# GaryGky/IDEAL-NeRF

Measured on AMD Instinct MI355X. Metric: ray-samples/sec (64+128 pts, 512x512), whole job, higher is better.
Workload: dtype f32

## Files before the change

ideal-nerf_amd/_lib.py:

```python
import ctypes as C
import os

HERE = os.path.dirname(os.path.abspath(__file__))
LIB_PATH = os.environ.get("IDN_LIB") or os.path.join(HERE, "libidealnerf.so")

IDN_PREC_F32, IDN_PREC_BF16X3, IDN_PREC_BF16, IDN_PREC_FP16X3, IDN_PREC_BF16X6 = 0, 1, 2, 3, 4
RAY_FLOATS = 11
MAX_MULTIRES, MAX_MULTIRES_VIEWS = 10, 4
SAMPLE_MAX_REGION = 4096
SCORE_TILE = 32
PROF_KINDS = ("mlp_fwd", "mlp_fwd_save", "delta_chain", "dw_gemm", "dw_gemm_x6", "mlp_fwd_save_x6", "delta_chain_x6")

fp = C.c_void_p


class FaceNerfParams(C.Structure):
    _fields_ = [("pts_w", fp * 8), ("pts_b", fp * 8), ("views_w", fp * 3), ("views_b", fp * 3),
                ("alpha_w", fp), ("alpha_b", fp), ("rgb_w", fp), ("rgb_b", fp),
                ("dim_aud", C.c_int), ("dim_expr", C.c_int), ("dim_latent", C.c_int),
                ("multires_plus1", C.c_int), ("multires_views_plus1", C.c_int)]


class FaceNerfGrads(C.Structure):
    _fields_ = [("pts_w", fp * 8), ("pts_b", fp * 8), ("views_w", fp * 3), ("views_b", fp * 3),
                ("alpha_w", fp), ("alpha_b", fp), ("rgb_w", fp), ("rgb_b", fp)]


class PassBwdExtra(C.Structure):
    _fields_ = [("d_expr", fp), ("d_rays", fp), ("d_views0_bias", fp)]


class CompositeOut(C.Structure):
    _fields_ = [(n, fp) for n in ("rgb_map", "disp_map", "acc_map", "depth_map", "weights", "rgb_fg", "last_weight")]


class RenderArgs(C.Structure):
    _fields_ = [("rays", fp), ("bc_rgb", fp), ("n_rays", C.c_int64), ("n_samples", C.c_int),
                ("n_importance", C.c_int), ("precision", C.c_int),
                ("packed_coarse", fp), ("folded_coarse", fp), ("packed_fine", fp), ("folded_fine", fp),
                ("t_vals", fp), ("t_rand", fp), ("u", fp), ("u_per_ray", C.c_int)] + \
               [(n, fp) for n in ("rgb_map", "disp_map", "acc_map", "depth_map", "last_weight", "rgb_fg",
                                  "rgb0", "disp0", "acc0", "z_std", "last_weight0", "rgb_fg0",
                                  "tap_z_coarse", "tap_raw_coarse", "tap_weights_coarse", "tap_cdf", "tap_inds",
                                  "tap_z_samples", "tap_z_fine", "tap_raw_fine", "tap_weights_fine")] + \
               [("workspace", fp), ("workspace_bytes", C.c_size_t), ("precision_fine_plus1", C.c_int),
                ("lindisp", C.c_int), ("white_bkgd", C.c_int), ("noise_coarse", fp), ("noise_fine", fp), ("fused_march", C.c_int),
                ("rng_mode", C.c_int), ("rng_seed", C.c_uint64), ("rng_ray0", C.c_int64)]


class AudioNetParams(C.Structure):
    _fields_ = [("conv_w", fp * 4), ("conv_b", fp * 4), ("fc_w", fp * 2), ("fc_b", fp * 2), ("dim_aud", C.c_int)]


class AudioNetGrads(C.Structure):
    _fields_ = [("conv_w", fp * 4), ("conv_b", fp * 4), ("fc_w", fp * 2), ("fc_b", fp * 2)]


class Frame(C.Structure):
    _fields_ = [("c2w", C.c_float * 12), ("H", C.c_int), ("W", C.c_int), ("focal", C.c_float), ("cx", C.c_float), ("cy", C.c_float),
                ("near_", C.c_float), ("far_", C.c_float), ("row0", C.c_int), ("nrows", C.c_int), ("rays_out", fp)]


class RenderOpts(C.Structure):
    _fields_ = [("colour_gate", C.c_int), ("gate_counters", fp)]


class CullGridStruct(C.Structure):
    _fields_ = [("bits", fp), ("G", C.c_int), ("lo", C.c_float * 3), ("cell", C.c_float)]


CULL_MAX_OUTPUTS = 12


class CullOutput(C.Structure):
    _fields_ = [("dense", fp), ("live", fp), ("channels", C.c_int), ("fill_background", C.c_int), ("value", C.c_float)]


DW_MAX_PRODUCTS, DW_MAX_TAKES, DW_MAX_COLSUM_TAKES = 16, 4, 2


class DwTake(C.Structure):
    _fields_ = [("row0", C.c_int), ("col0", C.c_int), ("rows", C.c_int), ("cols", C.c_int), ("out", fp), ("ldo", C.c_int)]
# ... 17 lines not shown
    "idealnerf_last_error": (C.c_char_p, []),
    "idealnerf_packed_weight_floats": (C.c_size_t, [C.c_int]),
    "idealnerf_folded_bias_floats": (C.c_size_t, []),
    "idealnerf_pack_weights": (C.c_int, [C.POINTER(FaceNerfParams), C.c_int, fp, fp]),
    "idealnerf_fold_conditioning": (C.c_int, [C.POINTER(FaceNerfParams), fp, fp, fp, fp, fp]),
    "idealnerf_facenerf_fwd": (C.c_int, [fp, fp, C.c_int, fp, C.c_int64, fp, fp]),
    "idealnerf_facenerf_fwd_ch": (C.c_int, [fp, fp, C.c_int, fp, C.c_int, C.c_int, C.c_int64, fp, fp]),
    "idealnerf_params_pts_ch": (C.c_int, [C.POINTER(FaceNerfParams)]),
    "idealnerf_params_views_ch": (C.c_int, [C.POINTER(FaceNerfParams)]),
    "idealnerf_query_rays_fwd": (C.c_int, [fp, fp, C.c_int, fp, fp, C.c_int64, C.c_int, fp, fp]),
    "idealnerf_query_points_fwd": (C.c_int, [fp, fp, C.c_int, fp, fp, C.c_int64, C.c_int, fp, fp]),
    "idealnerf_frame_rays": (C.c_int, [C.POINTER(C.c_float), C.c_int, C.c_int, C.c_float, C.c_float, C.c_float,
                                       C.c_float, C.c_float, C.c_int, C.c_int, fp, fp]),
    "idealnerf_to8b": (C.c_int, [fp, C.c_int64, C.c_int, fp, fp, fp]),
    "idealnerf_compose_to8b": (C.c_int, [fp, fp, fp, C.c_int64, C.c_int, fp, fp, fp, fp]),
    "idealnerf_philox_uniform": (C.c_int, [C.c_uint64, C.c_int, C.c_int64, C.c_int64, C.c_int, fp, fp]),
    "idealnerf_sample_pixels_workspace_bytes": (C.c_size_t, []),
    "idealnerf_sample_pixels": (C.c_int, [fp, C.c_int, C.c_int, C.c_int, C.c_int, C.c_int, C.c_int, C.c_uint64, C.c_uint64,
                                          fp, C.c_size_t, fp, fp]),
    "idealnerf_gather_rays": (C.c_int, [fp, C.c_int64, C.POINTER(C.c_float), C.c_int, C.c_int, C.c_float, C.c_float, C.c_float,
                                        fp, fp, fp, fp, fp, fp, fp, fp]),
    "idealnerf_gather_ray_pairs": (C.c_int, [fp, C.c_int64, C.POINTER(C.c_float), C.POINTER(C.c_float), C.c_int, C.c_int, C.c_float,
                                             C.c_float, C.c_float, fp, fp, fp, fp, fp, fp, fp, fp, fp]),
    "idealnerf_frame_scores_workspace_bytes": (C.c_size_t, [C.c_int, C.c_int]),
    "idealnerf_frame_scores": (C.c_int, [fp, fp, fp, C.c_int, C.c_int, fp, fp, C.c_size_t, fp]),
    "idealnerf_coarse_depths": (C.c_int, [fp, fp, fp, C.c_int, C.c_int64, C.c_int, fp, fp]),
    "idealnerf_composite_fwd": (C.c_int, [fp, fp, fp, fp, fp, C.c_int, C.c_int64, C.c_int, C.POINTER(CompositeOut), fp]),
    "idealnerf_sample_pdf_fwd": (C.c_int, [fp, fp, fp, C.c_int, C.c_int64, C.c_int, C.c_int, fp, fp, fp, fp, fp, fp]),
    "idealnerf_march_fwd": (C.c_int, [fp, fp, fp, fp, fp, C.c_int, fp, C.c_int, C.c_int64, C.c_int, C.c_int,
                                      C.POINTER(CompositeOut), fp, fp, fp, fp, fp, fp]),
    "idealnerf_sample_pdf_bins_fwd": (C.c_int, [fp, fp, fp, C.c_int, C.c_int64, C.c_int, C.c_int, fp, fp, fp, fp]),
    "idealnerf_invert_cdf": (C.c_int, [fp, fp, fp, C.c_int, C.c_int64, C.c_int, C.c_int, fp, fp, fp]),
    "idealnerf_render_workspace_bytes": (C.c_size_t, [C.c_int64, C.c_int, C.c_int]),
    "idealnerf_render_rays_fwd": (C.c_int, [C.POINTER(RenderArgs), fp]),
    "idealnerf_render_frame_workspace_bytes": (C.c_size_t, [C.c_int64, C.c_int, C.c_int]),
    "idealnerf_render_frame_fwd": (C.c_int, [C.POINTER(RenderArgs), C.POINTER(Frame), fp]),
    "idealnerf_render_rays_fwd_opts": (C.c_int, [C.POINTER(RenderArgs), C.POINTER(RenderOpts), fp]),
    "idealnerf_render_frame_fwd_opts": (C.c_int, [C.POINTER(RenderArgs), C.POINTER(Frame), C.POINTER(RenderOpts), fp]),
    "idealnerf_colour_gate_max_dist": (C.c_float, []),
    "idealnerf_audio_net_saved_floats": (C.c_size_t, [C.c_int]),
    "idealnerf_audio_net_fwd": (C.c_int, [C.POINTER(AudioNetParams), fp, C.c_int, fp, fp, fp]),
    "idealnerf_audio_net_bwd": (C.c_int, [C.POINTER(AudioNetParams), C.POINTER(AudioNetGrads), fp, fp, fp, C.c_int, fp]),
    "idealnerf_train_acts_floats": (C.c_size_t, [C.c_int64]),
    "idealnerf_query_rays_train_fwd": (C.c_int, [fp, fp, C.c_int, fp, fp, C.c_int64, C.c_int, fp, fp, fp]),
    "idealnerf_pass_bwd_workspace_bytes": (C.c_size_t, [C.c_int64, C.c_int]),
    "idealnerf_pass_bwd": (C.c_int, [C.POINTER(FaceNerfParams), C.POINTER(FaceNerfGrads), fp, fp, fp, fp, fp, fp, fp,
                                     fp, C.c_int64, C.c_int, fp, fp, fp, fp, fp, fp, fp, C.c_size_t, fp]),
    "idealnerf_pass_bwd_rays": (C.c_int, [C.POINTER(FaceNerfParams), C.POINTER(FaceNerfGrads), fp, fp, fp, fp, fp, fp, fp,
                                          fp, C.c_int64, C.c_int, fp, fp, fp, fp, fp, fp, fp, fp, C.c_size_t, fp]),
    "idealnerf_pass_bwd_cond": (C.c_int, [C.POINTER(FaceNerfParams), fp, fp, fp, fp, fp, fp, fp, fp, C.c_int64, C.c_int, fp, fp, fp,
                                          fp, fp, fp, fp, C.c_size_t, fp]),
    "idealnerf_pass_bwd_ex": (C.c_int, [C.POINTER(FaceNerfParams), C.POINTER(FaceNerfGrads), fp, fp, fp, fp, fp, fp, fp,
                                        fp, C.c_int64, C.c_int, fp, fp, fp, fp, fp, fp, C.POINTER(PassBwdExtra), fp, C.c_size_t, fp]),
    "idealnerf_facenerf_train_fwd": (C.c_int, [fp, fp, C.c_int, fp, C.c_int64, fp, fp, fp]),
    "idealnerf_facenerf_train_fwd_ch": (C.c_int, [fp, fp, C.c_int, fp, C.c_int, C.c_int, C.c_int64, fp, fp, fp]),
    "idealnerf_facenerf_bwd_workspace_bytes": (C.c_size_t, [C.c_int64]),
    "idealnerf_facenerf_bwd": (C.c_int, [C.POINTER(FaceNerfParams), C.POINTER(FaceNerfGrads), fp, fp, fp, fp, C.c_int64, fp,
                                         fp, fp, fp, fp, fp, C.c_size_t, fp]),
    "idealnerf_dw_gemm_workspace_bytes": (C.c_size_t, []),
    "idealnerf_dw_gemm": (C.c_int, [fp, C.c_int, fp, C.c_int, C.c_int64, fp, fp, C.c_int, fp, C.c_size_t, fp]),
    "idealnerf_dw_products_workspace_bytes": (C.c_size_t, []),
    "idealnerf_dw_products": (C.c_int, [C.c_int64, C.c_int, C.c_int, C.POINTER(DwProduct), C.c_int, fp, C.c_size_t, fp]),
    "idealnerf_delta_chain_workspace_bytes": (C.c_size_t, []),
    "idealnerf_delta_chain": (C.c_int, [C.POINTER(FaceNerfParams), C.c_int, fp, C.c_int64, fp, fp, fp, fp, C.c_int,
                                        C.POINTER(C.c_int), fp, C.c_size_t, fp]),
    "idealnerf_composite_bwd": (C.c_int, [fp, fp, fp, fp, C.c_int64, C.c_int, fp, fp, fp, fp, fp, C.c_int, fp, C.c_int, fp, C.c_int, fp]),
    "idealnerf_cull_mark": (C.c_int, [fp, C.c_int64, C.c_float, fp, fp]),
    "idealnerf_cull_cells": (C.c_int, [fp, C.c_int, C.c_int, fp, fp]),
    "idealnerf_cull_classify_workspace_bytes": (C.c_size_t, [C.c_int64]),
    "idealnerf_cull_classify": (C.c_int, [C.POINTER(CullGridStruct), C.POINTER(Frame), C.c_float, C.c_int, fp, fp, fp, C.c_size_t, fp]),
    "idealnerf_cull_gather": (C.c_int, [fp, C.c_int64, C.POINTER(Frame), fp, fp, fp, fp]),
    "idealnerf_cull_scatter": (C.c_int, [fp, C.c_int64, C.c_int64, fp, C.POINTER(CullOutput), C.c_int, fp]),
    "idealnerf_profile_begin": (None, []),
    "idealnerf_profile_end": (C.c_int, [C.POINTER(C.c_double), C.POINTER(C.c_int64), C.POINTER(C.c_int64)]),
    "idealnerf_profile_end_kinds": (C.c_int, [C.POINTER(C.c_double), C.POINTER(C.c_int64), C.POINTER(C.c_int64)]),
}

_lib = None


class IdealNerfError(RuntimeError):
    pass


def load():
    global _lib
    if _lib is not None:
        return _lib
    if not os.path.exists(LIB_PATH):
        raise IdealNerfError(
            f"{LIB_PATH} is missing: build the HIP extension first "
            "(python ideal-nerf_amd/build.py, or __graft_entry__.build()). There is no fallback path.")
    lib = C.CDLL(LIB_PATH)
    for name, (res, args) in PROTOTYPES.items():
        fn = getattr(lib, name)
        fn.restype = res
        fn.argtypes = args
    if lib.idealnerf_version() != ABI_VERSION:
        raise IdealNerfError(f"{LIB_PATH} has ABI version {lib.idealnerf_version()}, this package binds version {ABI_VERSION}: rebuild it")
    _lib = lib
    return lib


def check(rc):
    if rc != 0:
        msg = load().idealnerf_last_error()
        raise IdealNerfError(f"libidealnerf error {rc}: {msg.decode() if msg else '?'}")
```

ideal-nerf_amd/csrc/capi.hip:

```cpp
#include "idn_internal.h"
#include <cstdarg>
#include <cstdio>

namespace idn {

static thread_local char g_err[512] = "";

int fail(int code, const char* fmt, ...) {
    va_list ap;
    va_start(ap, fmt);
    vsnprintf(g_err, sizeof(g_err), fmt, ap);
    va_end(ap);
    return code;
}

static int check_precision(int precision) {
    if (precision == IDN_PREC_F32 || precision == IDN_PREC_BF16X3 || precision == IDN_PREC_BF16 || precision == IDN_PREC_FP16X3 ||
        precision == IDN_PREC_BF16X6)
        return IDN_OK;
    return fail(IDN_EUNSUPPORTED, "precision %d is unknown (IDN_PREC_F32, IDN_PREC_BF16X3, IDN_PREC_BF16, IDN_PREC_FP16X3, IDN_PREC_BF16X6)", precision);
}
static int check_precision_train(int precision) {
    if (precision == IDN_PREC_F32 || precision == IDN_PREC_BF16X6) return IDN_OK;
    return fail(IDN_EUNSUPPORTED, "the training path runs fp32-grade arithmetic only: IDN_PREC_F32 or IDN_PREC_BF16X6 (got %d)", precision);
// ... 310 lines not shown
    if (!packed || !folded || !rays || !z || !raw || !acts) return fail(IDN_EINVAL, "NULL pointer");
    const int64_t p_pad = (n_rays * n_samples + 127) / 128 * 128;
    return launch_mlp(precision, mlp_saving(mlp_rays(packed, folded, rays, z, n_rays, n_samples, raw), acts, p_pad), (hipStream_t)stream,
                      MlpGate{});
}

size_t idealnerf_pass_bwd_workspace_bytes(int64_t n_rays, int n_samples) {
    if (n_rays <= 0 || n_samples <= 0) return 0;
    return bwd_workspace_bytes(n_rays * n_samples);
}

static int check_grads(const idn_facenerf_grads* grads) {
    if (!grads) return fail(IDN_EINVAL, "grads is NULL");
    for (int i = 0; i < 8; ++i)
        if (!grads->pts_w[i] || !grads->pts_b[i]) return fail(IDN_EINVAL, "grad pts_linears.%d is NULL", i);
    for (int i = 0; i < 3; ++i)
        if (!grads->views_w[i] || !grads->views_b[i]) return fail(IDN_EINVAL, "grad views_linears.%d is NULL", i);
    if (!grads->alpha_w || !grads->alpha_b || !grads->rgb_w || !grads->rgb_b) return fail(IDN_EINVAL, "grad head is NULL");
    return IDN_OK;
}

static int pass_bwd_any(const PassBwd& b, void* stream) {
    const idn_facenerf_params* p = b.p;
    const BwdCond& c = b.cond;
    const bool frozen = !b.grads;
    if (int e = check_params(p)) return e;
    if (!frozen)
        if (int e = check_grads(b.grads)) return e;
    if ((p->dim_aud > 0) != (c.aud != nullptr) || (p->dim_expr > 0) != (c.expr != nullptr) ||
        (p->dim_latent > 0) != (c.latent != nullptr))
        return fail(IDN_EINVAL, "conditioning pointers do not match the widths");
    if (c.d_expr && (p->dim_expr == 0 || !c.expr)) return fail(IDN_EINVAL, "d_expr for a network without an expression");
    if (frozen && b.d_rays) return fail(IDN_EUNSUPPORTED, "the conditioning-only backward (grads NULL) returns no ray gradient");
    if (!frozen && c.d_vb) return fail(IDN_EINVAL, "d_views0_bias is the frozen plan's: with grads it is grads->views_b[0]");
    const bool want_cond = c.d_aud || c.d_latent || c.d_expr;
    if (frozen && c.d_vb && !want_cond) return fail(IDN_EINVAL, "d_views0_bias needs d_aud, d_latent or d_expr (with none the pass is not run)");
    if (b.n_rays < 0) return fail(IDN_EINVAL, "n_rays < 0");
    if (b.n_rays == 0 || (frozen && !want_cond)) return IDN_OK;
    if (!b.acts || !b.raw || !b.z || !b.rays || !b.bc) return fail(IDN_EINVAL, "NULL pointer");
    return launch_pass_bwd(b, (hipStream_t)stream);
}
static int pass_bwd_trained(const PassBwd& b, void* stream) {
    if (int e = check_params(b.p)) return e;
    if (!b.grads) return check_grads(b.grads);
    return pass_bwd_any(b, stream);
}

int idealnerf_pass_bwd(const idn_facenerf_params* p, const idn_facenerf_grads* grads, const float* aud,
                       const float* expr, const float* latent, const float* acts, const float* raw, const float* z,
                       const float* rays, const float* bc_rgb, int64_t n_rays, int n_samples, const float* g_rgb_map,
                       const float* g_rgb_fg, const float* g_last_weight, const float* g_acc, float* d_aud,
                       float* d_latent, void* workspace, size_t workspace_bytes, void* stream) {
    PassBwd b = {};
    b.p = p; b.grads = grads;
    b.cond.aud = aud; b.cond.expr = expr; b.cond.latent = latent; b.cond.d_aud = d_aud; b.cond.d_latent = d_latent;
    b.acts = acts; b.raw = raw; b.z = z; b.rays = rays; b.bc = bc_rgb; b.n_rays = n_rays; b.S = n_samples;
    b.g_rgb = g_rgb_map; b.g_fg = g_rgb_fg; b.g_lw = g_last_weight; b.g_acc = g_acc; b.ws = workspace; b.ws_bytes = workspace_bytes;
    return pass_bwd_trained(b, stream);
}

int idealnerf_pass_bwd_rays(const idn_facenerf_params* p, const idn_facenerf_grads* grads, const float* aud,
                            const float* expr, const float* latent, const float* acts, const float* raw, const float* z,
                            const float* rays, const float* bc_rgb, int64_t n_rays, int n_samples, const float* g_rgb_map,
                            const float* g_rgb_fg, const float* g_last_weight, const float* g_acc, float* d_aud,
                            float* d_latent, float* d_rays, void* workspace, size_t workspace_bytes, void* stream) {
    PassBwd b = {};
    b.p = p; b.grads = grads;
    b.cond.aud = aud; b.cond.expr = expr; b.cond.latent = latent; b.cond.d_aud = d_aud; b.cond.d_latent = d_latent;
    b.acts = acts; b.raw = raw; b.z = z; b.rays = rays; b.bc = bc_rgb; b.n_rays = n_rays; b.S = n_samples;
    b.g_rgb = g_rgb_map; b.g_fg = g_rgb_fg; b.g_lw = g_last_weight; b.g_acc = g_acc; b.ws = workspace; b.ws_bytes = workspace_bytes;
    b.d_rays = d_rays;
    return pass_bwd_trained(b, stream);
}

int idealnerf_pass_bwd_cond(const idn_facenerf_params* p, const float* aud, const float* expr, const float* latent,
                            const float* acts, const float* raw, const float* z, const float* rays, const float* bc_rgb,
                            int64_t n_rays, int n_samples, const float* g_rgb_map, const float* g_rgb_fg,
                            const float* g_last_weight, const float* g_acc, float* d_aud, float* d_latent, void* workspace,
                            size_t workspace_bytes, void* stream) {
    PassBwd b = {};
    b.p = p;
    b.cond.aud = aud; b.cond.expr = expr; b.cond.latent = latent; b.cond.d_aud = d_aud; b.cond.d_latent = d_latent;
    b.acts = acts; b.raw = raw; b.z = z; b.rays = rays; b.bc = bc_rgb; b.n_rays = n_rays; b.S = n_samples;
    b.g_rgb = g_rgb_map; b.g_fg = g_rgb_fg; b.g_lw = g_last_weight; b.g_acc = g_acc; b.ws = workspace; b.ws_bytes = workspace_bytes;
    return pass_bwd_any(b, stream);
}

int idealnerf_pass_bwd_ex(const idn_facenerf_params* p, const idn_facenerf_grads* grads, const float* aud,
                          const float* expr, const float* latent, const float* acts, const float* raw, const float* z,
                          const float* rays, const float* bc_rgb, int64_t n_rays, int n_samples, const float* g_rgb_map,
                          const float* g_rgb_fg, const float* g_last_weight, const float* g_acc, float* d_aud,
                          float* d_latent, const idn_pass_bwd_extra* extra, void* workspace, size_t workspace_bytes,
                          void* stream) {
    PassBwd b = {};
    b.p = p; b.grads = grads;
    b.cond.aud = aud; b.cond.expr = expr; b.cond.latent = latent; b.cond.d_aud = d_aud; b.cond.d_latent = d_latent;
    if (extra) b.cond.d_expr = extra->d_expr, b.cond.d_vb = extra->d_views0_bias, b.d_rays = extra->d_rays;
    b.acts = acts; b.raw = raw; b.z = z; b.rays = rays; b.bc = bc_rgb; b.n_rays = n_rays; b.S = n_samples;
    b.g_rgb = g_rgb_map; b.g_fg = g_rgb_fg; b.g_lw = g_last_weight; b.g_acc = g_acc; b.ws = workspace; b.ws_bytes = workspace_bytes;
    return pass_bwd_any(b, stream);
}

int idealnerf_facenerf_train_fwd(const float* packed, const float* folded, int precision, const float* x, int64_t n,
                                 float* out, float* acts, void* stream) {
    return idealnerf_facenerf_train_fwd_ch(packed, folded, precision, x, IDN_PTS_CH, IDN_VIEWS_CH, n, out, acts, stream);
}
int idealnerf_facenerf_train_fwd_ch(const float* packed, const float* folded, int precision, const float* x, int pts_ch,
                                    int views_ch, int64_t n, float* out, float* acts, void* stream) {
    if (int e = check_precision_train(precision)) return e;
    if (int e = check_widths(pts_ch, views_ch)) return e;
    if (n < 0) return fail(IDN_EINVAL, "n < 0");
    if (n == 0) return IDN_OK;
    if (!packed || !folded || !x || !out || !acts) return fail(IDN_EINVAL, "NULL pointer");
    if (n > 0x7fffffffLL) return fail(IDN_EUNSUPPORTED, "n %lld exceeds 2^31-1 per launch", (long long)n);
    const int64_t p_pad = (n + 127) / 128 * 128;
    return launch_mlp(precision, mlp_saving(mlp_rows(packed, folded, x, pts_ch, views_ch, n, out), acts, p_pad), (hipStream_t)stream,
                      MlpGate{});
}

size_t idealnerf_facenerf_bwd_workspace_bytes(int64_t n) {
    if (n <= 0) return 0;
    return bwd_workspace_bytes(n);
}

int idealnerf_facenerf_bwd(const idn_facenerf_params* p, const idn_facenerf_grads* grads, const float* aud, const float* expr,
                           const float* latent, const float* acts, int64_t n, const float* g_out, float* d_x, float* d_aud,
                           float* d_expr, float* d_latent, void* workspace, size_t workspace_bytes, void* stream) {
    if (int e = check_params(p)) return e;
    if (int e = check_grads(grads)) return e;
    if ((p->dim_aud > 0) != (aud != nullptr) || (p->dim_expr > 0) != (expr != nullptr) ||
        (p->dim_latent > 0) != (latent != nullptr))
        return fail(IDN_EINVAL, "conditioning pointers do not match the widths");
    if (n < 0) return fail(IDN_EINVAL, "n < 0");
    if (n == 0) return IDN_OK;
    if (!acts || !g_out) return fail(IDN_EINVAL, "NULL pointer");
    const BwdCond cond = {aud, expr, latent, d_aud, d_expr, d_latent, nullptr};
    return launch_facenerf_bwd(*p, *grads, cond, acts, n, g_out, d_x, workspace, workspace_bytes, (hipStream_t)stream);
}

size_t idealnerf_dw_gemm_workspace_bytes(void) { return dw_gemm_workspace_bytes(); }

int idealnerf_dw_gemm(const float* delta, int ld_delta, const float* acts, int ld_acts, int64_t rows, float* dW, float* db,
                      int pipe, void* workspace, size_t workspace_bytes, void* stream) {
    if (!delta || !acts || !dW) return fail(IDN_EINVAL, "NULL pointer");
    return launch_dw_gemm(delta, ld_delta, acts, ld_acts, rows, dW, db, pipe, workspace, workspace_bytes, (hipStream_t)stream);
}

size_t idealnerf_dw_products_workspace_bytes(void) { return dw_products_workspace_bytes(); }

int idealnerf_dw_products(int64_t rows, int pipe, int x6_items, idn_dw_product* products, int n, void* workspace,
                          size_t workspace_bytes, void* stream) {
    return launch_dw_products(rows, pipe, x6_items, products, n, workspace, workspace_bytes, (hipStream_t)stream);
}

size_t idealnerf_delta_chain_workspace_bytes(void) { return delta_chain_workspace_bytes(); }

int idealnerf_delta_chain(const idn_facenerf_params* p, int pipe, const float* acts, int64_t p_pad, const float* d_rgb,
                          float* dv0, float* dv21, float* da, int max_blocks, int* blocks_out, void* workspace,
                          size_t workspace_bytes, void* stream) {
    if (int e = check_params(p)) return e;
    return launch_delta_chain_alone(*p, pipe, acts, p_pad, d_rgb, dv0, dv21, da, max_blocks, blocks_out, workspace,
                                    workspace_bytes, (hipStream_t)stream);
}

int idealnerf_composite_bwd(const float* raw, const float* z, const float* rays, const float* bc_rgb, int64_t n_rays,
                            int n_samples, const float* g_rgb_map, const float* g_rgb_fg, const float* g_last_weight,
                            const float* g_acc, float* d_rgb, int ld_rgb, float* d_sig, int ld_sig, float* d_norm, int ld_norm,
                            void* stream) {
    if (n_rays < 0) return fail(IDN_EINVAL, "composite_bwd: n_rays < 0");
    if (n_rays == 0) return IDN_OK;
    if (!raw || !z || !rays || !bc_rgb || !d_rgb || !d_sig) return fail(IDN_EINVAL, "composite_bwd: NULL pointer");
    if ((uintptr_t)raw & 15) return fail(IDN_EINVAL, "composite_bwd: raw is not 16-byte aligned");
    if (ld_rgb < 3 || ld_sig < 1 || (d_norm && ld_norm < 1))
        return fail(IDN_EINVAL, "composite_bwd: row pitch %d / %d / %d below 3 / 1 / 1", ld_rgb, ld_sig, ld_norm);
    if (n_rays > 0x7fffffffLL) return fail(IDN_EUNSUPPORTED, "composite_bwd: n_rays %lld exceeds 2^31-1 per launch", (long long)n_rays);
    const CompBwdArgs a{reinterpret_cast<const float4*>(raw), z, rays, bc_rgb, g_rgb_map, g_rgb_fg, g_last_weight, g_acc,
                        d_rgb, ld_rgb, d_sig, ld_sig, (long)n_rays, n_samples, d_norm, ld_norm};
    return launch_composite_bwd(a, (hipStream_t)stream);
}

void idealnerf_profile_begin(void) {
    g_prof_n = 0;
    g_prof_on = true;
}

int idealnerf_profile_end_kinds(double* total_ms, int64_t* launches, int64_t* points) {
    g_prof_on = false;
    double ms[IDN_PROF_KINDS] = {0};
    int64_t n[IDN_PROF_KINDS] = {0}, pts[IDN_PROF_KINDS] = {0};
    for (int i = 0; i < g_prof_n; ++i) {
        IDN_HIP_CHECK(hipEventSynchronize(g_prof_ev[i][1]));
        float t = 0;
        IDN_HIP_CHECK(hipEventElapsedTime(&t, g_prof_ev[i][0], g_prof_ev[i][1]));
        const int k = g_prof_kind[i];
        ms[k] += t;
        n[k] += 1;
        pts[k] += g_prof_points[i];
    }
    for (int k = 0; k < IDN_PROF_KINDS; ++k) {
        if (total_ms) total_ms[k] = ms[k];
        if (launches) launches[k] = n[k];
        if (points) points[k] = pts[k];
    }
    return IDN_OK;
}
// ... 256 lines not shown
```

ideal-nerf_amd/csrc/dw_gemm.h:

```cpp
#pragma once
#include "mlp_common.h"

namespace idn {

__device__ __forceinline__ f32x16 mfma32(float a, float b, f32x16 c) { return __builtin_amdgcn_mfma_f32_32x32x2f32(a, b, c, 0, 0, 0); }
__device__ __forceinline__ int d_row(int r, int hh) { return (r & 3) + 8 * (r >> 2) + 4 * hh; }

struct TNArgs {
    const float* A; int lda;
    const float* B; int ldb;
    float* part;
    int N, K;
    long P;
    int chunks_per_split;
    float* cpart;
    int b_split, b_off0, b_off1;
};
constexpr int kMaxTnBatch = 12;
struct TNBatch {
    TNArgs it[kMaxTnBatch];
    int n, splits;
};
constexpr int kMaxReduceItems = 32;
struct ReduceItem {
    const float* part;
    float* out;
    int splits, N, K, ldo, rows, cols;
    int block_end;
};
struct ReduceBatch {
    ReduceItem it[kMaxReduceItems];
    int n;
};

inline size_t al256(size_t x) { return (x + 255) & ~(size_t)255; }
enum { kPipeX6 = IDN_DW_PIPE_BF16X6, kPipeF32 = IDN_DW_PIPE_F32 };

struct DwPassProduct { int N, K; bool colsum; int pipes; };
constexpr int kOnX6 = 1 << kPipeX6, kOnF32 = 1 << kPipeF32, kOnBoth = kOnX6 | kOnF32;
constexpr DwPassProduct kTrunk = {256, 256, true, kOnBoth};
constexpr DwPassProduct kPassProducts[] = {
    {64, 128, true, kOnBoth},
    {256, 256, true, kOnX6}, {128, 128, true, kOnF32}, {128, 128, true, kOnF32},
    kTrunk, {128, 64, false, kOnBoth},
    kTrunk, kTrunk, kTrunk, {256, 64, false, kOnBoth}, kTrunk, kTrunk, kTrunk, kTrunk,
    {256, 64, true, kOnBoth},
};
constexpr size_t pass_sum(int pipe, int what) {
    size_t n = 0;
    for (const DwPassProduct& t : kPassProducts)
        if (t.pipes >> pipe & 1) n += what == 0 ? (t.N == 256 && t.K == 256) : what == 1 ? (size_t)t.N * t.K : t.colsum ? t.N : 0;
    return n;
}
constexpr int kX6ItemsPerPass = (int)pass_sum(kPipeX6, 0);
static_assert(kX6ItemsPerPass == 9 && kX6ItemsPerPass <= kMaxTnBatch, "one x6 batch per pass");

constexpr int kMaxSplits = 256;
constexpr int kColsumBlocks = 256;
constexpr int kGemmsPerPass = 16;
constexpr size_t kPartFloatsPerSplit = 9 * 65536 + 6 * 16384 + 4 * 8192;
constexpr size_t kPartPoolFloats = (size_t)kMaxSplits * kPartFloatsPerSplit, kCpartPoolFloats = (size_t)kColsumBlocks * 256 * kGemmsPerPass;
static_assert(pass_sum(kPipeX6, 1) <= kPartFloatsPerSplit && pass_sum(kPipeF32, 1) <= kPartFloatsPerSplit, "a pass's partial blocks fit");
static_assert(kMaxSplits * pass_sum(kPipeX6, 2) <= kCpartPoolFloats && kMaxSplits * pass_sum(kPipeF32, 2) <= kCpartPoolFloats, "a pass's column sums fit");

struct DwProduct { const float *part, *cpart; int splits, N, K, chunks_per_split; };

struct DwPass {
    DwPass(float* part, size_t part_floats, float* cpart, size_t cpart_floats, int64_t P, int pipe, int x6_items, hipStream_t s)
        : part_next(part), part_left(part_floats), cpart_next(cpart), cpart_left(cpart_floats), P(P), pipe(pipe), x6_items(x6_items), s(s) {}
    int product(const float* A, int lda, int N, const float* B, int ldb, int K, bool want_colsum, DwProduct* h, const float* B2 = nullptr);
    int take(const DwProduct& h, int row0, int col0, int rows, int cols, float* out, int ldo);
    int take_colsum(const DwProduct& h, int col0, int cols, float* out);
    int finish();

private:
    float* part_next; size_t part_left;
    float* cpart_next; size_t cpart_left;
    int64_t P;
    int pipe, x6_items;
    hipStream_t s;
    TNBatch x6{{}, 0, 0};
    ReduceBatch red{{}, 0};
    int red_blocks = 0;
};

}
```

ideal-nerf_amd/csrc/dw_gemm.hip:

```cpp
#include "dw_gemm.h"
#include "mlp_x6.h"

namespace idn {

template <int N>
struct LdsVec;
template <>
struct LdsVec<4> {
    f32x4 v;
    template <int OFF>
    __device__ __forceinline__ void issue(uint32_t addr) { asm volatile("ds_read_b128 %0, %1 offset:%2" : "=v"(v) : "v"(addr), "n"(OFF) : "memory"); }
    __device__ __forceinline__ float get(int j) const { return v[j]; }
};
template <>
struct LdsVec<2> {
    typedef float f32x2 __attribute__((ext_vector_type(2)));
    f32x2 v;
    template <int OFF>
    __device__ __forceinline__ void issue(uint32_t addr) { asm volatile("ds_read_b64 %0, %1 offset:%2" : "=v"(v) : "v"(addr), "n"(OFF) : "memory"); }
    __device__ __forceinline__ float get(int j) const { return v[j]; }
};
template <>
struct LdsVec<1> {
    float v;
    template <int OFF>
    __device__ __forceinline__ void issue(uint32_t addr) { asm volatile("ds_read_b32 %0, %1 offset:%2" : "=v"(v) : "v"(addr), "n"(OFF) : "memory"); }
    __device__ __forceinline__ float get(int) const { return v; }
};
template <int OFF>
__device__ __forceinline__ void lds_read_f32(float& dst, uint32_t addr) {
    asm volatile("ds_read_b32 %0, %1 offset:%2" : "=v"(dst) : "v"(addr), "n"(OFF) : "memory");
}
__device__ __forceinline__ float landed(float& v) {
    asm volatile("" : "+v"(v));
    return v;
}
template <int NEWER, class VA, class VB>
__device__ __forceinline__ void lds_retire(VA& a, VB& b) {
    if constexpr (NEWER == 0) asm volatile("s_waitcnt lgkmcnt(0)" : "+v"(a.v), "+v"(b.v)::"memory");
    else asm volatile("s_waitcnt lgkmcnt(2)" : "+v"(a.v), "+v"(b.v)::"memory");
}

constexpr int kTnRows = 16, kTnBufs = 3;
constexpr int kTnNarrowBufs = 3;
constexpr int kTnRows4x1 = 32, kTnRowsThin = 64;
constexpr int kTnNarrowSplits = 256;

template <int NTW, int KTW, int NB = kTnBufs, int R = kTnRows>
__global__ __launch_bounds__(256) void gemm_tn_kernel(TNArgs g) {
    static_assert(R % 16 == 0, "chunks are multiples of 16 points");
    constexpr int NPA = NTW * R / 16, NPB = KTW * R / 16;
    static_assert(NB >= 3 && (NB - 2) * (NPA + NPB) <= 63, "vmcnt is a 6-bit field");
    constexpr int BN = 64 * NTW, BK = 64 * KTW;
    constexpr int kTileFloats = R * (BN + BK);
    constexpr int kSteps = R / 2;
    constexpr int NP = NPA + NPB;
    static_assert(NP <= kSteps, "at most one piece per step");
    extern __shared__ __attribute__((aligned(16))) float tn_smem[];
    const int tid = threadIdx.x, lane = tid & 63;
    const int w = __builtin_amdgcn_readfirstlane(tid >> 6);
    const int i = lane & 31, hh = lane >> 5;
    const int wr = w >> 1, wc = w & 1;
    const int n0 = blockIdx.x * BN, k0 = blockIdx.y * BK;
    const int split = blockIdx.z;
    f32x16 acc[NTW][KTW];
#pragma unroll
    for (int a = 0; a < NTW; ++a)
#pragma unroll
        for (int b = 0; b < KTW; ++b)
            for (int r = 0; r < 16; ++r) acc[a][b][r] = 0.f;

    const long c_begin = (long)split * g.chunks_per_split;
    long c_end = c_begin + g.chunks_per_split;
    const long c_total = g.P / R;
    if (c_end > c_total) c_end = c_total;
    const bool colsum_block = g.cpart != nullptr && blockIdx.y == 0;
    const bool do_colsum = colsum_block && tid < BN;
    const int ccol = tid < BN ? tid : 0;
    float csum = 0.0f;

    constexpr int kRowsPerPieceA = 256 / BN > 0 ? 256 / BN : 1, kRowsPerPieceB = 256 / BK > 0 ? 256 / BK : 1;
    const __amdgpu_buffer_rsrc_t rsrcA = __builtin_amdgcn_make_buffer_rsrc(const_cast<float*>(g.A + n0 + c_begin * R * (long)g.lda), 0, 0xfffffffc, 0x00020000);
    const __amdgpu_buffer_rsrc_t rsrcB = __builtin_amdgcn_make_buffer_rsrc(const_cast<float*>(g.B + k0 + c_begin * R * (long)g.ldb), 0, 0xfffffffc, 0x00020000);
    const uint32_t voffA = ((lane / (BN / 4)) * g.lda + (lane % (BN / 4)) * 4) * 4;
    const uint32_t voffB = ((lane / (BK / 4)) * g.ldb + (lane % (BK / 4)) * 4) * 4;
    const uint32_t rowA = g.lda * 4, rowB = g.ldb * 4;
    auto piece_a = [&](long c, int buf, int ja) {
        const int pc = NPA * w + ja;
        __builtin_amdgcn_raw_ptr_buffer_load_lds(rsrcA, (__attribute__((address_space(3))) void*)(tn_smem + buf * kTileFloats + pc * 256), 16, voffA,
                                                 (uint32_t)(((c - c_begin) * R + pc * kRowsPerPieceA) * rowA), 0, 0);
    };
    auto piece_b = [&](long c, int buf, int jb) {
        const int pc = NPB * w + jb;
        __builtin_amdgcn_raw_ptr_buffer_load_lds(rsrcB, (__attribute__((address_space(3))) void*)(tn_smem + buf * kTileFloats + R * BN + pc * 256), 16, voffB,
                                                 (uint32_t)(((c - c_begin) * R + pc * kRowsPerPieceB) * rowB), 0, 0);
    };
    auto piece = [&](long c, int buf, int j) {
        if (j < NPA) piece_a(c, buf, j);
        else if (j < NP) piece_b(c, buf, j - NPA);
    };
    const uint32_t smem0 = (uint32_t)(uintptr_t)(__attribute__((address_space(3))) float*)tn_smem;
    const uint32_t a_addr0 = smem0 + (hh * BN + NTW * (32 * wr + i)) * 4;
    const uint32_t b_addr0 = smem0 + (R * BN + hh * BK + KTW * (32 * wc + i)) * 4;
    for (int ahead = 0; ahead < NB - 1; ++ahead)
        for (int j = 0; j < NP; ++j) piece(c_begin + ahead < c_end ? c_begin + ahead : c_end - 1, ahead, j);
    int buf = 0;
    for (long c = c_begin; c < c_end; ++c) {
        asm volatile("s_waitcnt vmcnt(%0)" ::"n"((NB - 2) * NP) : "memory");
        __builtin_amdgcn_s_barrier();
        asm volatile("" ::: "memory");
        const int buf2 = buf >= 1 ? buf - 1 : NB - 1;
        const long cnext = c + NB - 1 < c_end ? c + NB - 1 : c_end - 1;
        float cs[16];
        auto cs_issue = [&](int batch) {
            const uint32_t caddr = smem0 + buf * (kTileFloats * 4) + ccol * 4 + batch * (16 * BN * 4);
            static_for<16>([&](auto Row) {
                lds_read_f32<decltype(Row)::value * BN * 4>(cs[decltype(Row)::value], caddr);
            });
        };
        static_assert(R / 16 <= kSteps / 4, "one batch of column reads per iteration of the first half loop");
        if (colsum_block) cs_issue(0);
        LdsVec<NTW> a0v, a1v;
        LdsVec<KTW> b0v, b1v;
        constexpr int kStepA = 2 * BN * 4, kStepB = 2 * BK * 4;
        uint32_t pa = a_addr0 + buf * (kTileFloats * 4), pb = b_addr0 + buf * (kTileFloats * 4);
        a0v.template issue<0>(pa);
        b0v.template issue<0>(pb);
        static_assert(NPA <= kSteps / 2 && NPB <= kSteps / 2, "pieces of one matrix fit one half of a chunk");
        constexpr int M = NTW * KTW;
        if constexpr (M >= 4) {
            auto step = [&](LdsVec<NTW>& ca, LdsVec<KTW>& cb, auto&& side0, auto&& side1, auto&& side2) {
                lds_retire<0>(ca, cb);
                static_for<M>([&](auto M_) {
                    constexpr int m = decltype(M_)::value, x = m / KTW, y = m % KTW;
                    acc[x][y] = mfma32(ca.get(x), cb.get(y), acc[x][y]);
                    if constexpr (m < 3) {
                        __builtin_amdgcn_sched_barrier(0);
                        if constexpr (m == 0) side0();
                        if constexpr (m == 1) side1();
                        if constexpr (m == 2) side2();
                        __builtin_amdgcn_sched_barrier(0);
                    }
                });
            };
#pragma unroll 1
            for (int it = 0; it < kSteps / 4; ++it) {
                step(a0v, b0v,
                     [&]() { a1v.template issue<kStepA>(pa); b1v.template issue<kStepB>(pb); },
                     [&]() { if (2 * it < NPA) piece_a(cnext, buf2, 2 * it); },
                     [&]() {
                         if (colsum_block && it < R / 16) {
                             static_for<16>([&](auto Row) { csum += landed(cs[decltype(Row)::value]); });
                         }
                         pa += 2 * kStepA;
                         pb += 2 * kStepB;
                     });
                step(a1v, b1v,
                     [&]() { a0v.template issue<0>(pa); b0v.template issue<0>(pb); },
                     [&]() { if (2 * it + 1 < NPA) piece_a(cnext, buf2, 2 * it + 1); },
                     [&]() { if (colsum_block && it + 1 < R / 16) cs_issue(it + 1); });
// ... 19 lines not shown
            LdsVec<KTW> b2v, b3v;
            a1v.template issue<kStepA>(pa);
            b1v.template issue<kStepB>(pb);
            auto quad = [&](LdsVec<NTW>& c0a, LdsVec<KTW>& c0b, LdsVec<NTW>& c1a, LdsVec<KTW>& c1b, LdsVec<NTW>& n0a, LdsVec<KTW>& n0b,
                            LdsVec<NTW>& n1a, LdsVec<KTW>& n1b, bool last, auto&& side_c, auto&& side_d) {
                lds_retire<0>(c0a, c0b);
                lds_retire<0>(c1a, c1b);
                const uint32_t na = last ? pa : pa + 2 * kStepA, nb = last ? pb : pb + 2 * kStepB;
                auto mf = [&](LdsVec<NTW>& ca, LdsVec<KTW>& cb, auto M_) {
                    constexpr int m = decltype(M_)::value, x = m / KTW, y = m % KTW;
                    acc[x][y] = mfma32(ca.get(x), cb.get(y), acc[x][y]);
                    __builtin_amdgcn_sched_barrier(0);
                };
                mf(c0a, c0b, ic<0>{});
                n0a.template issue<0>(na);
                n0b.template issue<0>(nb);
                __builtin_amdgcn_sched_barrier(0);
                mf(c0a, c0b, ic<1>{});
                n1a.template issue<kStepA>(na);
                n1b.template issue<kStepB>(nb);
                __builtin_amdgcn_sched_barrier(0);
                mf(c1a, c1b, ic<0>{});
                side_c();
                __builtin_amdgcn_sched_barrier(0);
                mf(c1a, c1b, ic<1>{});
                side_d();
                pa = na;
                pb = nb;
                __builtin_amdgcn_sched_barrier(0);
            };
#pragma unroll 1
            for (int it = 0; it < kSteps / 8; ++it) {
                quad(a0v, b0v, a1v, b1v, a2v, b2v, a3v, b3v, false,
                     [&]() { if (2 * it < NPA) piece_a(cnext, buf2, 2 * it); },
                     [&]() {
                         if (colsum_block && it < R / 16) {
                             static_for<16>([&](auto Row) { csum += landed(cs[decltype(Row)::value]); });
                         }
                     });
                quad(a2v, b2v, a3v, b3v, a0v, b0v, a1v, b1v, false,
                     [&]() { if (2 * it + 1 < NPA) piece_a(cnext, buf2, 2 * it + 1); },
                     [&]() { if (colsum_block && it + 1 < R / 16) cs_issue(it + 1); });
            }
#pragma unroll 1
            for (int it = 0; it < kSteps / 8; ++it) {
                quad(a0v, b0v, a1v, b1v, a2v, b2v, a3v, b3v, false,
                     [&]() { if (2 * it < NPB) piece_b(cnext, buf2, 2 * it); }, [&]() {});
                quad(a2v, b2v, a3v, b3v, a0v, b0v, a1v, b1v, it == kSteps / 8 - 1,
                     [&]() { if (2 * it + 1 < NPB) piece_b(cnext, buf2, 2 * it + 1); }, [&]() {});
            }
            lds_retire<0>(a1v, b1v);
        }
        lds_retire<0>(a0v, b0v);
        buf = buf + 1 == NB ? 0 : buf + 1;
    }
    asm volatile("s_waitcnt vmcnt(0)" ::: "memory");
    if (do_colsum) g.cpart[(long)split * g.N + n0 + tid] = csum;
    float* out = g.part + (long)split * g.N * g.K;
#pragma unroll
    for (int x = 0; x < NTW; ++x)
#pragma unroll
        for (int r = 0; r < 16; ++r) {
            const int n = n0 + NTW * (32 * wr + d_row(r, hh)) + x;
            float* dst = out + (long)n * g.K + k0 + KTW * (32 * wc + i);
            if constexpr (KTW == 4) {
                *reinterpret_cast<f32x4*>(dst) = f32x4{acc[x][0][r], acc[x][1][r], acc[x][2][r], acc[x][3][r]};
            } else {
#pragma unroll
                for (int y = 0; y < KTW; ++y) dst[y] = acc[x][y][r];
            }
        }
}

typedef unsigned tn_u32x4 __attribute__((ext_vector_type(4)));
typedef int tn_i32x4 __attribute__((ext_vector_type(4)));
__device__ __forceinline__ void split3(float x0, float x1, unsigned& p1, unsigned& p2, unsigned& p3) {
    float w1, w2, w3;
    x6::split3(x0, x1, w1, w2, w3);
    p1 = __float_as_uint(w1), p2 = __float_as_uint(w2), p3 = __float_as_uint(w3);
}
constexpr int kX6BufBytes = 2 * 8 * 3 * kFragBytes;
constexpr int kX6Lds = 2 * kX6BufBytes;

struct X6Frag {
    f32x4 v;
    template <int OFF>
    __device__ __forceinline__ void issue(uint32_t addr) { asm volatile("ds_read_b128 %0, %1 offset:%2" : "=v"(v) : "v"(addr), "n"(OFF) : "memory"); }
};
template <int N>
__device__ __forceinline__ void x6_retire(X6Frag (&f)[3]) {
    static_assert(N <= 15, "lgkmcnt is a 4-bit field");
    asm volatile("s_waitcnt lgkmcnt(%3)" : "+v"(f[0].v), "+v"(f[1].v), "+v"(f[2].v) : "n"(N) : "memory");
}

__device__ __forceinline__ void gemm_tn_x6_item(const TNArgs& g, const int split, char* x6_smem) {
    const int tid = threadIdx.x, lane = tid & 63;
    const int w = __builtin_amdgcn_readfirstlane(tid >> 6);
    const int i = lane & 31, hh = lane >> 5;
    const int wr = w >> 1, wc = w & 1;
    f32x16 acc[4][4];
#pragma unroll
    for (int a = 0; a < 4; ++a)
#pragma unroll
        for (int b = 0; b < 4; ++b)
            for (int r = 0; r < 16; ++r) acc[a][b][r] = 0.f;

    const long c_begin = (long)split * g.chunks_per_split;
    long c_end = c_begin + g.chunks_per_split;
    const long c_total = g.P / kTnRows;
    if (c_end > c_total) c_end = c_total;
    const int n_chunks = (int)(c_end - c_begin);
    auto make_rsrc = [](const float* ptr) {
        const uint64_t a64 = (uint64_t)(uintptr_t)ptr;
        return tn_i32x4{(int)(uint32_t)a64, (int)((uint32_t)(a64 >> 32) & 0xffffu), (int)0xfffffffcu, 0x00020000};
    };
    const tn_i32x4 rsrcA = make_rsrc(g.A + c_begin * kTnRows * (long)g.lda);
    const tn_i32x4 rsrcB = make_rsrc(g.B + c_begin * kTnRows * (long)g.ldb);
    const int voff = tid * 4;
    const int voffB = g.b_split ? (tid < 128 ? g.b_off0 : g.b_off1) + (tid & 127) * 4 : voff;
    const int rowA = g.lda * 4, rowB = g.ldb * 4;
    float ra[kTnRows], rb[kTnRows];
#pragma unroll
    for (int p = 0; p < kTnRows; ++p) ra[p] = rb[p] = 0.f;
    auto load_row_at = [&](float& dst, const tn_i32x4& rsrc, int soff, int vo) {
        asm volatile("buffer_load_dword %0, %1, %2, %3 offen" : "+v"(dst) : "v"(vo), "s"(rsrc), "s"(soff) : "memory");
    };
    auto load_row = [&](float& dst, const tn_i32x4& rsrc, int soff) { load_row_at(dst, rsrc, soff, voff); };
    auto load_chunk = [&](int rc) {
        const int base = (rc < n_chunks ? rc : n_chunks - 1) * kTnRows;
#pragma unroll
        for (int p = 0; p < kTnRows; ++p) load_row(ra[p], rsrcA, (base + p) * rowA);
#pragma unroll
        for (int p = 0; p < kTnRows; ++p) load_row_at(rb[p], rsrcB, (base + p) * rowB, voffB);
    };
    char* const my_slot = x6_smem + (tid >> 5) * (3 * kFragBytes) + (tid & 31) * 16;
    auto split_store = [&](int buf, int X, const float (&r)[kTnRows]) {
        unsigned pw[3][8];
#pragma unroll
        for (int j = 0; j < 8; ++j) split3(r[2 * j], r[2 * j + 1], pw[0][j], pw[1][j], pw[2][j]);
        char* dst = my_slot + buf * kX6BufBytes + X * (8 * 3 * kFragBytes);
#pragma unroll
        for (int q = 0; q < 3; ++q)
#pragma unroll
            for (int h2 = 0; h2 < 2; ++h2)
                *reinterpret_cast<tn_u32x4*>(dst + q * kFragBytes + h2 * 512) =
                    tn_u32x4{pw[q][4 * h2], pw[q][4 * h2 + 1], pw[q][4 * h2 + 2], pw[q][4 * h2 + 3]};
    };
    const bool do_colsum = g.cpart != nullptr;
    float csum = 0.0f, csum1 = 0.0f;
    auto colsum = [&]() {
        float s0 = (ra[0] + ra[1]) + (ra[2] + ra[3]), s1 = (ra[4] + ra[5]) + (ra[6] + ra[7]);
        float s2 = (ra[8] + ra[9]) + (ra[10] + ra[11]), s3 = (ra[12] + ra[13]) + (ra[14] + ra[15]);
        csum += (s0 + s1) + (s2 + s3);
    };
    const uint32_t smem0 = (uint32_t)(uintptr_t)(__attribute__((address_space(3))) char*)x6_smem;
    const uint32_t a_base = smem0 + (4 * wr) * (3 * kFragBytes) + lane * 16;
    const uint32_t b_base = smem0 + (8 + 4 * wc) * (3 * kFragBytes) + lane * 16;

    load_chunk(0);
#pragma unroll
    for (int p = 0; p < kTnRows; ++p) asm volatile("s_waitcnt vmcnt(0)" : "+v"(ra[p]), "+v"(rb[p])::"memory");
    colsum();
    split_store(0, 0, ra);
    split_store(0, 1, rb);
    load_chunk(1);
    asm volatile("s_waitcnt lgkmcnt(0)" ::: "memory");
    __builtin_amdgcn_s_barrier();
    asm volatile("" ::: "memory");

    X6Frag fa[4][3], fb[4][3];
    auto issue_first_row = [&](uint32_t pa, uint32_t pb) {
        static_for<3>([&](auto Q) { fa[0][decltype(Q)::value].template issue<decltype(Q)::value * kFragBytes>(pa); });
        static_for<2>([&](auto Y) {
            static_for<3>([&](auto Q) {
                fb[decltype(Y)::value][decltype(Q)::value].template issue<(decltype(Y)::value * 3 + decltype(Q)::value) * kFragBytes>(pb);
            });
        });
    };
    issue_first_row(a_base, b_base);
#pragma unroll 1
    for (int rc = 0; rc < n_chunks; ++rc) {
        const int buf = rc & 1;
        const uint32_t pa = a_base + buf * kX6BufBytes, pb = b_base + buf * kX6BufBytes;
        static_for<2>([&](auto Y) {
            static_for<3>([&](auto Q) {
                fb[decltype(Y)::value + 2][decltype(Q)::value].template issue<((decltype(Y)::value + 2) * 3 + decltype(Q)::value) * kFragBytes>(pb);
            });
        });
        static_for<3>([&](auto X) {
            static_for<3>([&](auto Q) {
                fa[decltype(X)::value + 1][decltype(Q)::value].template issue<((decltype(X)::value + 1) * 3 + decltype(Q)::value) * kFragBytes>(pa);
            });
        });
        auto mm2 = [&](int x, int y0, int y1) {
#define X6_TERM(QA, QB)                                                   \
    acc[x][y0] = x6::mfma_bf(fa[x][QA].v, fb[y0][QB].v, acc[x][y0]);        \
    acc[x][y1] = x6::mfma_bf(fa[x][QA].v, fb[y1][QB].v, acc[x][y1]);
            X6_TERM(0, 0) X6_TERM(0, 1) X6_TERM(1, 0) X6_TERM(1, 1) X6_TERM(0, 2) X6_TERM(2, 0)
#undef X6_TERM
        };
        x6_retire<15>(fa[0]);
        x6_retire<15>(fb[0]);
        x6_retire<15>(fb[1]);
        mm2(0, 0, 1);
        x6_retire<9>(fb[2]);
        x6_retire<9>(fb[3]);
        mm2(0, 2, 3);
        x6_retire<0>(fa[1]);
        x6_retire<0>(fa[2]);
        x6_retire<0>(fa[3]);
        const unsigned live_mask = rc + 1 < n_chunks ? 0xffffffffu : 0u;
        const int nbase = (rc + 2 < n_chunks ? rc + 2 : n_chunks - 1) * kTnRows;
        char* const dst = my_slot + (buf ^ 1) * kX6BufBytes;
        unsigned pw[2][3][8];
        float t0 = 0.f, t1 = 0.f;
        auto slice = [&](auto X_, auto S_) {
            constexpr int X = decltype(X_)::value, sl = decltype(S_)::value;
            float (&r)[kTnRows] = *(X ? &rb : &ra);
            auto store = [&](auto Q_, auto H_) {
                constexpr int q = decltype(Q_)::value, h2 = decltype(H_)::value;
                *reinterpret_cast<tn_u32x4*>(dst + X * (8 * 3 * kFragBytes) + q * kFragBytes + h2 * 512) =
                    tn_u32x4{pw[X][q][4 * h2], pw[X][q][4 * h2 + 1], pw[X][q][4 * h2 + 2], pw[X][q][4 * h2 + 3]};
            };
            if constexpr (sl < 24) {
                constexpr int j = sl / 3, ph = sl % 3;
                if constexpr (ph == 0) {
                    asm volatile("s_waitcnt vmcnt(30)" : "+v"(r[2 * j]), "+v"(r[2 * j + 1])::"memory");
                    const unsigned p1 = x6::cvt_pk_bf16(r[2 * j], r[2 * j + 1]);
                    pw[X][0][j] = p1;
                    t0 = r[2 * j] - __uint_as_float(p1 << 16);
                    t1 = r[2 * j + 1] - __uint_as_float(p1 & 0xffff0000u);
                    if constexpr (X == 0) {
                        csum += __uint_as_float(__float_as_uint(r[2 * j]) & live_mask);
                        csum1 += __uint_as_float(__float_as_uint(r[2 * j + 1]) & live_mask);
                        asm volatile("" : "+v"(csum), "+v"(csum1));
                    }
                } else if constexpr (ph == 1) {
                    const unsigned p2 = x6::cvt_pk_bf16(t0, t1);
                    pw[X][1][j] = p2;
                    t0 = t0 - __uint_as_float(p2 << 16);
                    t1 = t1 - __uint_as_float(p2 & 0xffff0000u);
                    pw[X][2][j] = x6::cvt_pk_bf16(t0, t1);
                } else {
                    load_row_at(r[2 * j], X ? rsrcB : rsrcA, (nbase + 2 * j) * (X ? rowB : rowA), X ? voffB : voff);
                    load_row_at(r[2 * j + 1], X ? rsrcB : rsrcA, (nbase + 2 * j + 1) * (X ? rowB : rowA), X ? voffB : voff);
                    if constexpr (j >= 3 && j < 6) store(ic<j - 3>{}, ic<0>{});
                    if constexpr (j == 7) store(ic<0>{}, ic<1>{});
                }
            } else if constexpr (sl == 24) {
                store(ic<1>{}, ic<1>{});
            } else if constexpr (sl == 25) {
                store(ic<2>{}, ic<1>{});
            }
        };
        __builtin_amdgcn_sched_barrier(0);
        static_for<72>([&](auto K_) {
            constexpr int k = decltype(K_)::value;
            constexpr int x = 1 + k / 24, kk = k % 24, y = 2 * (kk / 12) + (kk % 2), t = (kk % 12) / 2;
            constexpr int qa = t == 2 || t == 3 ? 1 : (t == 5 ? 2 : 0);
            constexpr int qb = t == 1 || t == 3 ? 1 : (t == 4 ? 2 : 0);
            acc[x][y] = x6::mfma_bf(fa[x][qa].v, fb[y][qb].v, acc[x][y]);
            constexpr int kX1 = 26;
            if constexpr (k < kX1) slice(ic<0>{}, ic<k>{});
            else slice(ic<1>{}, ic<k - kX1>{});
            if constexpr (k == 59) {
                asm volatile("s_waitcnt lgkmcnt(0)" ::: "memory");
                __builtin_amdgcn_s_barrier();
                asm volatile("" ::: "memory");
                issue_first_row(a_base + (buf ^ 1) * kX6BufBytes, b_base + (buf ^ 1) * kX6BufBytes);
            }
            __builtin_amdgcn_sched_barrier(0);
        });
    }
    x6_retire<0>(fa[0]);
    x6_retire<0>(fb[0]);
    x6_retire<0>(fb[1]);
#pragma unroll
    for (int p = 0; p < kTnRows; ++p) asm volatile("s_waitcnt vmcnt(0)" : "+v"(ra[p]), "+v"(rb[p])::"memory");
    if (do_colsum) g.cpart[(long)split * g.N + tid] = csum + csum1;
    float* out = g.part + (long)split * g.N * g.K;
#pragma unroll
    for (int x = 0; x < 4; ++x)
#pragma unroll
        for (int y = 0; y < 4; ++y)
#pragma unroll
            for (int r = 0; r < 16; ++r)
                out[(long)(32 * (4 * wr + x) + d_row(r, hh)) * g.K + 32 * (4 * wc + y) + i] = acc[x][y][r];
}
__global__ __launch_bounds__(256) void gemm_tn_x6_kernel(TNBatch b) {
    extern __shared__ __attribute__((aligned(16))) char x6_smem[];
    const int item = __builtin_amdgcn_readfirstlane((int)blockIdx.z / b.splits);
    const int split = __builtin_amdgcn_readfirstlane((int)blockIdx.z - item * b.splits);
    gemm_tn_x6_item(b.it[item], split, x6_smem);
}

__global__ __launch_bounds__(256) void reduce_batch_kernel(ReduceBatch b) {
    __shared__ double red[4][64];
    int i = 0;
    while (i + 1 < b.n && (int)blockIdx.x >= b.it[i].block_end) ++i;
    const ReduceItem& t = b.it[i];
    const int block0 = i ? b.it[i - 1].block_end : 0;
    const int o = threadIdx.x & 63, q = threadIdx.x >> 6;
    const int idx = ((int)blockIdx.x - block0) * 64 + o;
    const bool live = idx < t.rows * t.cols;
    const int n = live ? idx / t.cols : 0, k = live ? idx % t.cols : 0;
    double s = 0.0;
    if (live) {
        const float* src = t.part + (long)n * t.K + k;
        const long stride = (long)t.N * t.K;
#pragma unroll 8
        for (int sp = q; sp < t.splits; sp += 4) s += (double)src[sp * stride];
    }
    red[q][o] = s;
    __syncthreads();
    if (q == 0 && live) t.out[(long)n * t.ldo + k] = (float)(((red[0][o] + red[1][o]) + red[2][o]) + red[3][o]);
}

template <int NTW, int KTW, int NB, int R = kTnRows>
static int launch_tn(const TNArgs& g, int splits, hipStream_t s) {
    constexpr size_t lds = (size_t)NB * R * (size_t)(64 * NTW + 64 * KTW) * 4;
    static_assert(lds <= 160 * 1024, "the chunk ring must fit a CU's LDS");
    static LaunchSetup setup;
    int num_cu = 0;
    if (int e = setup.get([]() -> int {
            IDN_HIP_CHECK(hipFuncSetAttribute(reinterpret_cast<const void*>(&gemm_tn_kernel<NTW, KTW, NB, R>),
                                              hipFuncAttributeMaxDynamicSharedMemorySize, (int)lds));
            return IDN_OK;
        }, &num_cu))
        return e;
    hipLaunchKernelGGL((gemm_tn_kernel<NTW, KTW, NB, R>), dim3(g.N / (64 * NTW), g.K / (64 * KTW), splits), dim3(256), lds, s, g);
    IDN_HIP_CHECK(hipGetLastError());
    return IDN_OK;
}
struct DwShape { int N, K, rows_per_chunk, max_splits; int (*launch)(const TNArgs&, int, hipStream_t); };
constexpr DwShape kX6Shape = {256, 256, kTnRows, kMaxSplits, nullptr};
constexpr DwShape kF32Shapes[] = {
    {256, 256, kTnRows, kMaxSplits, &launch_tn<4, 4, kTnBufs>},
    {256, 64, kTnRows4x1, kTnNarrowSplits, &launch_tn<4, 1, kTnNarrowBufs, kTnRows4x1>},
    {128, 256, kTnRows, kMaxSplits, &launch_tn<2, 4, kTnBufs>},
    {128, 64, kTnRowsThin, kTnNarrowSplits, &launch_tn<2, 1, kTnNarrowBufs, kTnRowsThin>},
    {128, 128, kTnRows, kMaxSplits, &launch_tn<2, 2, kTnBufs>},
    {64, 128, kTnRowsThin, kTnNarrowSplits, &launch_tn<1, 2, kTnNarrowBufs, kTnRowsThin>},
};
static_assert(kTnNarrowSplits <= kMaxSplits, "the pools hold kMaxSplits splits of every product of a pass (dw_gemm.h)");

static int x6_setup(int* cus) {
    static LaunchSetup st;
    return st.get([]() -> int {
        IDN_HIP_CHECK(hipFuncSetAttribute(reinterpret_cast<const void*>(&gemm_tn_x6_kernel), hipFuncAttributeMaxDynamicSharedMemorySize, kX6Lds));
        return IDN_OK;
    }, cus);
}

int DwPass::product(const float* A, int lda, int N, const float* B, int ldb, int K, bool want_colsum, DwProduct* h, const float* B2) {
    const DwShape* sh = nullptr;
    if (N == 256 && K == 256 && pipe == kPipeX6) sh = &kX6Shape;
    else
        for (const DwShape& t : kF32Shapes)
            if (t.N == N && t.K == K) sh = &t;
    if (!sh) return fail(IDN_EUNSUPPORTED, "gemm_tn: no instantiation for %d x %d", N, K);
    const bool queued = sh->launch == nullptr;
    if (B2 && !queued) return fail(IDN_EINVAL, "gemm_tn: a split B needs the 256 x 256 bf16-piece kernel");
    if (P % sh->rows_per_chunk) return fail(IDN_EINVAL, "gemm_tn: %lld rows are not a multiple of the %d-row chunk", (long long)P, sh->rows_per_chunk);
    const long chunks = P / sh->rows_per_chunk;
    int splits = sh->max_splits;
    if (queued) {
        if (x6.n >= x6_items || x6.n >= kMaxTnBatch) return fail(IDN_EINVAL, "gemm_tn: more 256 x 256 products than the pass declared (%d)", x6_items);
        int cus = 0;
        if (int e = x6_setup(&cus)) return e;
        splits = 2 * cus / x6_items;
        if (splits > kMaxSplits) splits = kMaxSplits;
    }
    if (splits > chunks) splits = (int)chunks;
    if (splits < 1) splits = 1;
    const int cps = (int)((chunks + splits - 1) / splits);
    splits = (int)((chunks + cps - 1) / cps);
    const size_t part_floats = (size_t)splits * N * K, cpart_floats = want_colsum ? (size_t)splits * N : 0;
    if (part_floats > part_left || cpart_floats > cpart_left)
        return fail(IDN_EWORKSPACE, "gemm_tn: the partial blocks of %d x %d in %d splits do not fit the pool", N, K, splits);
    TNArgs g{A, lda, B, ldb, part_next, N, K, (long)P, cps, want_colsum ? cpart_next : nullptr, 0, 0, 0};
    if (B2) {
        const float* base = B < B2 ? B : B2;
        const int64_t o0 = (int64_t)(B - base) * 4, o1 = (int64_t)(B2 - base) * 4;
        if (o0 >= (int64_t)1 << 31 || o1 >= (int64_t)1 << 31) return fail(IDN_EUNSUPPORTED, "gemm_tn: split B matrices more than 2 GiB apart");
        g.B = base, g.b_split = 1;
        g.b_off0 = (int)o0, g.b_off1 = (int)o1;
    }
    if (queued) {
        x6.splits = splits;
        x6.it[x6.n++] = g;
    } else {
        ProfScope prof(s, P, IDN_PROF_DW_GEMM);
        if (int e = sh->launch(g, splits, s)) return e;
    }
    *h = DwProduct{g.part, g.cpart, splits, N, K, cps};
    part_next += part_floats, part_left -= part_floats;
    cpart_next += cpart_floats, cpart_left -= cpart_floats;
    return IDN_OK;
}

int DwPass::take(const DwProduct& h, int row0, int col0, int rows, int cols, float* out, int ldo) {
    if (red.n >= kMaxReduceItems) return fail(IDN_EUNSUPPORTED, "reduce queue full");
    red_blocks += (rows * cols + 63) / 64;
    red.it[red.n++] = ReduceItem{h.part + (size_t)row0 * h.K + col0, out, h.splits, h.N, h.K, ldo, rows, cols, red_blocks};
    return IDN_OK;
}
int DwPass::take_colsum(const DwProduct& h, int col0, int cols, float* out) {
    if (!h.cpart) return fail(IDN_EINVAL, "gemm_tn: the product kept no column sums");
    return take(DwProduct{h.cpart, nullptr, h.splits, 1, h.N, h.chunks_per_split}, 0, col0, 1, cols, out, cols);
}

int DwPass::finish() {
    if (x6.n) {
        ProfScope prof(s, P * x6.n, IDN_PROF_DW_GEMM_X6);
        hipLaunchKernelGGL(gemm_tn_x6_kernel, dim3(1, 1, x6.splits * x6.n), dim3(256), kX6Lds, s, x6);
    }
    IDN_HIP_CHECK(hipGetLastError());
    if (red.n) hipLaunchKernelGGL(reduce_batch_kernel, dim3(red_blocks), dim3(256), 0, s, red);
    IDN_HIP_CHECK(hipGetLastError());
    return IDN_OK;
}

size_t dw_gemm_workspace_bytes() { return al256((size_t)kMaxSplits * 65536 * 4) + al256((size_t)kColsumBlocks * 256 * 4); }
int launch_dw_gemm(const float* delta, int ld_delta, const float* acts, int ld_acts, int64_t rows, float* dW, float* db, int pipe,
                   void* ws, size_t ws_bytes, hipStream_t s) {
    if (rows <= 0 || rows % 128) return fail(IDN_EINVAL, "dw_gemm: rows %lld is not a positive multiple of 128", (long long)rows);
    if (ld_delta < 256 || ld_acts < 256) return fail(IDN_EINVAL, "dw_gemm: row pitch < 256");
    const int x6_items = pipe == IDN_DW_PIPE_BF16X6_PASS ? kX6ItemsPerPass : 1;
    if (pipe == IDN_DW_PIPE_BF16X6_PASS) pipe = IDN_DW_PIPE_BF16X6;
    if (pipe != IDN_DW_PIPE_BF16X6 && pipe != IDN_DW_PIPE_F32) return fail(IDN_EINVAL, "dw_gemm: pipe %d", pipe);
    if (!ws || ws_bytes < dw_gemm_workspace_bytes()) return fail(IDN_EWORKSPACE, "dw_gemm workspace %zu < %zu", ws_bytes, dw_gemm_workspace_bytes());
    float* part = reinterpret_cast<float*>(ws);
    float* cpart = reinterpret_cast<float*>(reinterpret_cast<char*>(ws) + al256((size_t)kMaxSplits * 65536 * 4));
    DwPass q(part, (size_t)kMaxSplits * 65536, cpart, (size_t)kColsumBlocks * 256, rows, pipe, x6_items, s);
    DwProduct h;
    if (int e = q.product(delta, ld_delta, 256, acts, ld_acts, 256, db != nullptr, &h)) return e;
    int e = db ? q.take_colsum(h, 0, 256, db) : IDN_OK;
    if (!e) e = q.take(h, 0, 0, 256, 256, dW, 256);
    return e ? e : q.finish();
}

size_t dw_products_workspace_bytes() { return al256(kPartPoolFloats * 4) + al256(kCpartPoolFloats * 4); }
int launch_dw_products(int64_t rows, int pipe, int x6_items, idn_dw_product* pr, int n, void* ws, size_t ws_bytes, hipStream_t s) {
    if (!pr) return fail(IDN_EINVAL, "dw_products: NULL pointer");
    if (n < 1 || n > IDN_DW_MAX_PRODUCTS) return fail(IDN_EINVAL, "dw_products: %d products outside [1, %d]", n, IDN_DW_MAX_PRODUCTS);
    if (pipe != kPipeX6 && pipe != kPipeF32) return fail(IDN_EINVAL, "dw_products: pipe %d", pipe);
    if (rows <= 0 || rows % 128) return fail(IDN_EINVAL, "dw_products: rows %lld is not a positive multiple of 128", (long long)rows);
    if (rows > (int64_t)1 << 24) return fail(IDN_EUNSUPPORTED, "dw_products: rows %lld exceed 2^24", (long long)rows);
    if (pipe == kPipeX6 && (x6_items < 1 || x6_items > kMaxTnBatch))
        return fail(IDN_EINVAL, "dw_products: x6_items %d outside [1, %d]", x6_items, kMaxTnBatch);
    int n_x6 = 0, n_red = 0;
    size_t part_per_split = 0, cpart_per_split = 0;
    for (int i = 0; i < n; ++i) {
        const idn_dw_product& t = pr[i];
        if (!t.delta || !t.acts) return fail(IDN_EINVAL, "dw_products: product %d: NULL pointer", i);
        const bool x6 = t.N == 256 && t.K == 256 && pipe == kPipeX6;
        bool known = x6;
        for (const DwShape& sh : kF32Shapes) known = known || (sh.N == t.N && sh.K == t.K);
        if (!known) return fail(IDN_EUNSUPPORTED, "dw_products: product %d: no instantiation for %d x %d", i, t.N, t.K);
        const int b_cols = t.acts2 ? 128 : t.K;
        if (t.ld_delta < t.N || t.ld_acts < b_cols) return fail(IDN_EINVAL, "dw_products: product %d: row pitch %d / %d < %d / %d", i, t.ld_delta, t.ld_acts, t.N, b_cols);
        if (t.ld_delta % 4 || t.ld_acts % 4 || ((uintptr_t)t.delta | (uintptr_t)t.acts | (uintptr_t)t.acts2) % 16)
            return fail(IDN_EINVAL, "dw_products: product %d: operands are not 16-byte aligned row by row", i);
        if (t.acts2 && !x6) return fail(IDN_EINVAL, "dw_products: product %d: a split B needs the 256 x 256 bf16-piece kernel", i);
        if (t.acts2) {
            const uintptr_t lo = (uintptr_t)(t.acts < t.acts2 ? t.acts : t.acts2), hi = (uintptr_t)(t.acts < t.acts2 ? t.acts2 : t.acts);
            if (hi - lo >= (uintptr_t)1 << 31) return fail(IDN_EUNSUPPORTED, "dw_products: product %d: split B matrices more than 2 GiB apart", i);
        }
        if (x6 && ++n_x6 > x6_items) return fail(IDN_EINVAL, "dw_products: more 256 x 256 products than x6_items (%d)", x6_items);
        if (t.n_takes < 0 || t.n_takes > IDN_DW_MAX_TAKES || t.n_colsum_takes < 0 || t.n_colsum_takes > IDN_DW_MAX_COLSUM_TAKES)
            return fail(IDN_EINVAL, "dw_products: product %d: %d takes / %d column-sum takes", i, t.n_takes, t.n_colsum_takes);
        if (t.n_colsum_takes && !t.want_colsum) return fail(IDN_EINVAL, "dw_products: product %d kept no column sums", i);
        if ((n_red += t.n_takes + t.n_colsum_takes) > kMaxReduceItems)
            return fail(IDN_EINVAL, "dw_products: more than %d takes in one pass", kMaxReduceItems);
        for (int j = 0; j < t.n_takes; ++j) {
            const idn_dw_take& k = t.takes[j];
            if (!k.out) return fail(IDN_EINVAL, "dw_products: product %d take %d: NULL pointer", i, j);
            if (k.row0 < 0 || k.col0 < 0 || k.rows < 1 || k.cols < 1 || k.row0 + k.rows > t.N || k.col0 + k.cols > t.K || k.ldo < k.cols)
                return fail(IDN_EINVAL, "dw_products: product %d take %d leaves the %d x %d block (or its pitch is short)", i, j, t.N, t.K);
        }
        for (int j = 0; j < t.n_colsum_takes; ++j) {
            const idn_dw_colsum_take& k = t.colsum_takes[j];
            if (!k.out) return fail(IDN_EINVAL, "dw_products: product %d column-sum take %d: NULL pointer", i, j);
            if (k.col0 < 0 || k.cols < 1 || k.col0 + k.cols > t.N)
                return fail(IDN_EINVAL, "dw_products: product %d column-sum take %d leaves the %d columns", i, j, t.N);
        }
        part_per_split += (size_t)t.N * t.K;
        cpart_per_split += t.want_colsum ? t.N : 0;
    }
    if (part_per_split > kPartFloatsPerSplit || cpart_per_split * kMaxSplits > kCpartPoolFloats)
        return fail(IDN_EWORKSPACE, "dw_products: the list's partial blocks do not fit the pools of a pass");
    if (!ws || ws_bytes < dw_products_workspace_bytes())
        return fail(IDN_EWORKSPACE, "dw_products workspace %zu < %zu", ws_bytes, dw_products_workspace_bytes());
    float* part = reinterpret_cast<float*>(ws);
    float* cpart = reinterpret_cast<float*>(reinterpret_cast<char*>(ws) + al256(kPartPoolFloats * 4));
    DwPass q(part, kPartPoolFloats, cpart, kCpartPoolFloats, rows, pipe, x6_items, s);
    for (int i = 0; i < n; ++i) {
        idn_dw_product& t = pr[i];
        DwProduct h;
        if (int e = q.product(t.delta, t.ld_delta, t.N, t.acts, t.ld_acts, t.K, t.want_colsum != 0, &h, t.acts2)) return e;
        for (int j = 0; j < t.n_colsum_takes; ++j)
            if (int e = q.take_colsum(h, t.colsum_takes[j].col0, t.colsum_takes[j].cols, t.colsum_takes[j].out)) return e;
        for (int j = 0; j < t.n_takes; ++j) {
            const idn_dw_take& k = t.takes[j];
            if (int e = q.take(h, k.row0, k.col0, k.rows, k.cols, k.out, k.ldo)) return e;
        }
        t.splits = h.splits, t.chunks_per_split = h.chunks_per_split;
    }
    return q.finish();
}

}
```

ideal-nerf_amd/csrc/idn_internal.h:

```cpp
#pragma once
#include <hip/hip_runtime.h>
#include <mutex>
#include <type_traits>
#include <stdint.h>
#include <stddef.h>
#include "../../include/idealnerf.h"

namespace idn {

__host__ __device__ inline int pts_ch_of(const idn_facenerf_params& p) {
    return p.multires_plus1 ? 6 * p.multires_plus1 - 3 : IDN_PTS_CH;
}
__host__ __device__ inline int views_ch_of(const idn_facenerf_params& p) {
    return p.multires_views_plus1 ? 6 * p.multires_views_plus1 - 3 : IDN_VIEWS_CH;
}
inline bool widths_ok(int pts_ch, int views_ch) {
    return pts_ch >= 3 && pts_ch <= IDN_PTS_CH && pts_ch % 6 == 3 && views_ch >= 3 && views_ch <= IDN_VIEWS_CH && views_ch % 6 == 3;
}

constexpr int kFragBytes = 1024;
constexpr int kFragFloats = 256;
constexpr int kSliceFrags = 64;
constexpr int kRingSlots = 2;
constexpr int kRingFrags = kRingSlots * kSliceFrags;
// ... 185 lines not shown
                       float cx, float cy, const unsigned char* image, const unsigned char* background, const float* target_table,
                       const float* background_table, float* batch_rays, float* batch_rays2, float* target_s, float* bc_rgb,
                       hipStream_t s);
int launch_cull_mark(const float* raw, int64_t n, float sigma_min, unsigned char* corners, hipStream_t s);
int launch_cull_cells(const unsigned char* corners, int G, int dilate, unsigned* bits, hipStream_t s);
size_t cull_classify_workspace_bytes(int64_t npix);
int launch_cull_classify(const idn_cull_grid& grid, const idn_frame& frame, float dz, int K, long long* sel, int* n_live, void* ws,
                         hipStream_t s);
int launch_cull_gather(const long long* sel, int64_t n, const idn_frame& frame, const float* bc, float* rays, float* bc_live,
                       hipStream_t s);
int launch_cull_scatter(const long long* sel, int64_t n_live, int64_t npix, const float* bc, const idn_cull_output* outs, int n_outs,
                        hipStream_t s);
size_t frame_scores_workspace_bytes(int H, int W);
int launch_frame_scores(const float* pred, const unsigned char* truth, const unsigned char* regions, int H, int W, double* out,
                        double* partial, hipStream_t s);
int launch_coarse_depths(const float* rays, const float* t_vals, const float* t_rand, int64_t n_rays, int S,
                         int lindisp, float* z, hipStream_t s, Draws draws = Draws{0, 0, 0});
int launch_composite(const float* raw, const float* z, const float* rays, const float* bc, int64_t n_rays, int S,
                     const float* noise, int white_bkgd, const idn_composite_out& out, hipStream_t s);
int launch_march(const float* raw, const float* z, const float* rays, const float* bc, const float* noise, int white_bkgd,
                 const idn_composite_out& out, const float* u, int u_per_ray, int64_t n_rays, int S, int Ni,
                 float* z_samples, int64_t* inds, float* cdf_out, float* z_fine, float* z_std, hipStream_t s,
                 Draws draws = Draws{0, 0, 0});
int launch_render_fused(int arrangement, const float* packed_c, const float* folded_c, const float* packed_f, const float* folded_f,
                        const float* rays, const float* bc, const float* z_c, float* z_f, const float* u, int u_per_ray, int64_t n_rays,
                        int white_bkgd, const idn_composite_out& co, const idn_composite_out& fo, float* z_std, float* tap_raw_c,
                        float* tap_raw_f, float* tap_z_fine, int64_t* tap_inds, float* tap_z_samples, float* tap_cdf, hipStream_t s,
                        Draws draws = Draws{0, 0, 0});
int launch_sample_pdf(const float* z, const float* weights, const float* cdf_in, const float* bins_in,
                      const float* u, int u_per_ray, int64_t n_rays, int S, int Ni, float* z_samples,
                      int64_t* inds, float* cdf_out, float* z_fine, float* z_std, hipStream_t s);

constexpr int kBwdStages = 11;
constexpr int kBwdNT[kBwdStages] = {4, 4, 4, 8, 8, 8, 8, 8, 8, 8, 8};
constexpr int kBwdKG[kBwdStages] = {2, 16, 16, 18, 32, 32, 32, 32, 32, 32, 32};
constexpr int kBwdHeadFrags = 280, kBwdTrunk0 = 384;
constexpr int bwd_f0(int s) {
    if (s >= 4) return kBwdTrunk0 + 256 * (s - 4);
    int f = 0;
    for (int i = 0; i < s; ++i) f += kBwdNT[i] * kBwdKG[i];
    return f;
}
static_assert(bwd_f0(3) + kBwdNT[3] * kBwdKG[3] == kBwdHeadFrags, "head stages");
constexpr int kBwdStreamFrags = kBwdTrunk0 + 7 * 256;
static_assert(kBwdStreamFrags % kSliceFrags == 0 && kBwdTrunk0 % kRingFrags == 0, "ring phase of the trunk stages");
constexpr int kBwdNumSlices = kBwdStreamFrags / kSliceFrags;

int launch_pack_f32_bwd(const idn_facenerf_params& p, float* packed_bwd, hipStream_t s);
int launch_delta_chain(const float* packed_bwd, const float* acts, int64_t p_pad, const float* d_rgb, float* dv0,
                       float* dv2, float* dv1, float* const da[8], hipStream_t s, int max_grid = 0,
                       int* grid_out = nullptr);
size_t bwd_stream_floats_x6();
int launch_pack_bf16x6_bwd(const idn_facenerf_params& p, float* packed_bwd, hipStream_t s);
int launch_delta_chain_x6(const float* packed_bwd, const float* acts, int64_t p_pad, const float* d_rgb, float* dv0,
                          float* dv2, float* dv1, float* const da[8], hipStream_t s, int max_grid = 0,
                          int* grid_out = nullptr);
size_t delta_chain_workspace_bytes();
int launch_delta_chain_alone(const idn_facenerf_params& p, int pipe, const float* acts, int64_t p_pad, const float* d_rgb,
                             float* dv0, float* dv21, float* da, int max_blocks, int* blocks_out, void* ws, size_t ws_bytes,
                             hipStream_t s);

size_t dw_gemm_workspace_bytes();
int launch_dw_gemm(const float* delta, int ld_delta, const float* acts, int ld_acts, int64_t rows, float* dW, float* db, int pipe,
                   void* ws, size_t ws_bytes, hipStream_t s);
size_t dw_products_workspace_bytes();
int launch_dw_products(int64_t rows, int pipe, int x6_items, idn_dw_product* products, int n, void* ws, size_t ws_bytes, hipStream_t s);

size_t bwd_workspace_bytes(int64_t n_points);
struct BwdCond {
    const float *aud, *expr, *latent;
    float *d_aud, *d_expr, *d_latent;
    float* d_vb;
};
struct PassBwd {
    const idn_facenerf_params* p;
    const idn_facenerf_grads* grads;
    BwdCond cond;
    const float *acts, *raw, *z, *rays, *bc;
    int64_t n_rays;
    int S;
    const float *g_rgb, *g_fg, *g_lw, *g_acc;
    float* d_rays;
    void* ws;
    size_t ws_bytes;
};
int launch_pass_bwd(const PassBwd& b, hipStream_t s);
struct CompBwdArgs {
    const float4* raw; const float* z; const float* rays; const float* bc;
    const float* g_rgb;
    const float* g_fg;
    const float* g_lw;
    const float* g_acc;
    float* d_rgb; int ld_rgb;
    float* d_sig; int ld_sig;
    long n_rays; int S;
    float* d_norm; int ld_norm;
};
int launch_composite_bwd(const CompBwdArgs& a, hipStream_t s);
int launch_ray_grad(const float* d_x, int pts_ch, int views_ch, const float* rays, const float* z, int64_t n_rays, int S,
                    float* d_rays, hipStream_t s);
int launch_facenerf_bwd(const idn_facenerf_params& p, const idn_facenerf_grads& gr, const BwdCond& cond, const float* acts,
                        int64_t n, const float* g_out, float* d_x, void* ws, size_t ws_bytes, hipStream_t s);

}
```

ideal-nerf_amd/csrc/mlp_f32_bwd.hip:

```cpp
#include "mlp_x6.h"

namespace idn {

__device__ __forceinline__ f32x16 mfma_b(float a, float b, f32x16 c) {
    return __builtin_amdgcn_mfma_f32_32x32x2f32(a, b, c, 0, 0, 0);
}

struct BwdPackStage {
    const float* w;
    const float* extra;
    int ld, col0, rows, cols, extra_at;
};
struct BwdPackDesc {
    BwdPackStage st[kBwdStages];
};
__global__ void pack_f32_bwd_kernel(BwdPackDesc d, float4* out) {
    const int gid = blockIdx.x * blockDim.x + threadIdx.x;
    if (gid >= kBwdStreamFrags * 64) return;
    const int f = gid >> 6, lane = gid & 63;
    float v[4] = {0.f, 0.f, 0.f, 0.f};
    int s = -1;
    for (int i = 0; i < kBwdStages; ++i)
        if (f >= bwd_f0(i) && f < bwd_f0(i) + kBwdNT[i] * kBwdKG[i]) s = i;
    if (s >= 0) {
// ... 367 lines not shown
        }
        a[0] = n[0];
        a[1] = n[1];
        a[2] = n[2];
    });
    if constexpr (!LAST && (F0 + kX6KFrags * NP) % kX6SliceFrags != 0) retire3<0>(a);
    pref[0] = a[0];
    pref[1] = a[1];
    pref[2] = a[2];
}

template <int KS>
struct MaskStoreSide {
    f32x16* O;
    const uint32_t* mk;
    float* row;
    template <int T>
    __device__ __forceinline__ void apply(ic<T>) const {
        const uint32_t w = mk[T >> 1];
        static_for<16>([&](auto R) {
            constexpr int r = decltype(R)::value, i = 16 * (T & 1) + r;
            const int off = (int)(w << i) >> 31;
            O[T][r] = __uint_as_float(__float_as_uint(O[T][r]) & ~(uint32_t)off);
        });
    }
    template <int T, int Q0>
    __device__ __forceinline__ void store2(ic<T>, ic<Q0>) const {
        static_for<2>([&](auto I) {
            constexpr int q = Q0 + decltype(I)::value;
            *reinterpret_cast<f32x4*>(row + 32 * T + 8 * q) = f32x4{O[T][4 * q], O[T][4 * q + 1], O[T][4 * q + 2], O[T][4 * q + 3]};
        });
    }
    template <int T>
    __device__ __forceinline__ void whole(ic<T>) const {
        apply(ic<T>{});
        store2(ic<T>{}, ic<0>{});
        store2(ic<T>{}, ic<2>{});
    }
    template <int T, int Q>
    __device__ __forceinline__ void store1(ic<T>, ic<Q>) const {
        *reinterpret_cast<f32x4*>(row + 32 * T + 8 * Q) = f32x4{O[T][4 * Q], O[T][4 * Q + 1], O[T][4 * Q + 2], O[T][4 * Q + 3]};
    }
    template <int T, int S>
    __device__ __forceinline__ void operator()(ic<T>, ic<S>) const {
        if constexpr (KS == 16 && T > 0) {
            if constexpr (S == 7) apply(ic<T - 1>{});
            if constexpr (S >= 8 && S < 16 && (S & 1) == 0) store1(ic<T - 1>{}, ic<(S - 8) / 2>{});
        }
    }
};

constexpr int kDelta6Lds = kX6RingFrags * kFragBytes;

__global__ __launch_bounds__(256, 1) void delta_chain_x6_kernel(DeltaArgs a) {
    extern __shared__ __attribute__((aligned(16))) char smem[];
    char* ring = smem;
    const int tid = threadIdx.x, lane = tid & 63;
    const int wave = __builtin_amdgcn_readfirstlane(tid >> 6);
    const int m = lane & 31, h = lane >> 5;

    WStream6 ws;
    ws.init(a.wstream, kBwd6NumSlices, ring, tid, wave);
    FragReader fr;
    fr.addr0 = (uint32_t)(uintptr_t)(__attribute__((address_space(3))) char*)ring + lane * 16;
    fr.addr1 = fr.addr0 + 64 * kFragBytes;
    const long ntiles = a.p_pad >> 7;
    f32x4 pref[3] = {{0.f, 0.f, 0.f, 0.f}, {0.f, 0.f, 0.f, 0.f}, {0.f, 0.f, 0.f, 0.f}};

    for (long tile = blockIdx.x; tile < ntiles; tile += gridDim.x) {
        const long P = tile * 128 + wave * 32 + m;
        const f32x4 drgb = *reinterpret_cast<const f32x4*>(a.d_rgb + P * 64);
        const float dsig = a.dv0[P * 256 + kSigmaChannel];
        f32x4 in_rgb[3], in_sig[3];
        {
            const f32x4 z4 = {0.f, 0.f, 0.f, 0.f};
            float r[3][2], g[3];
            split3(h ? 0.0f : drgb[0], h ? 0.0f : drgb[1], r[0][0], r[1][0], r[2][0]);
            split3(h ? 0.0f : drgb[2], 0.0f, r[0][1], r[1][1], r[2][1]);
            float unused0, unused1, unused2;
            (void)unused0; (void)unused1; (void)unused2;
            split3(h ? 0.0f : dsig, 0.0f, g[0], g[1], g[2]);
            static_for<3>([&](auto Q) {
                constexpr int q = decltype(Q)::value;
                in_rgb[q] = z4;
                in_rgb[q][0] = r[q][0];
                in_rgb[q][1] = r[q][1];
                in_sig[q] = z4;
                in_sig[q][0] = g[q];
            });
        }

        settle(in_rgb);
        settle(in_sig);
        PTile6 Pt[8];
        f32x16 O[8];
        typedef uint32_t u32x4 __attribute__((ext_vector_type(4)));
        const u32x4* mbase = reinterpret_cast<const u32x4*>(a.acts + (size_t)kActCols * a.p_pad);
        auto mask_load = [&](int id) { return mbase[mask_index(id, a.p_pad, tile * 4 + wave, lane)]; };
        u32x4 mask_nxt = mask_load(10);
        auto tiles = [&](auto Q, auto S_) {
            constexpr int q = decltype(Q)::value, s = decltype(S_)::value;
            return Pt[s >> 1].p[q][s & 1];
        };
        auto stage_run = [&](auto F0c, auto NTc, auto KSc, auto LASTc, auto LDc, auto YOUNGERc, auto&& bget, int next_id, float* dst) __attribute__((always_inline)) {
            constexpr int NT = decltype(NTc)::value, LD = decltype(LDc)::value;
            const u32x4 mv = mask_nxt;
            const uint32_t mk[4] = {mv.x, mv.y, mv.z, mv.w};
            if (next_id >= 0) mask_nxt = mask_load(next_id);
            const MaskStoreSide<decltype(KSc)::value> side{O, mk, dst + P * LD + 4 * h};
            constexpr bool trunk = decltype(F0c)::value >= bwd6_f0(4);
            run_stage6<decltype(F0c)::value, NT, decltype(KSc)::value, decltype(LASTc)::value != 0, decltype(YOUNGERc)::value, (trunk ? 4 : 0)>(O, bget, ws, fr, pref, side);
            if constexpr (trunk) side.whole(ic<NT - 1>{});
            else static_for<NT>([&](auto T) { side.whole(T); });
            static_for<NT>([&](auto T) { convert_tile<false>(O[decltype(T)::value], Pt[decltype(T)::value]); });
        };
        stage_run(ic<bwd6_f0(0)>{}, ic<4>{}, ic<1>{}, ic<0>{}, ic<256>{}, ic<0>{}, [&](auto Q, auto) { return in_rgb[decltype(Q)::value]; }, 9, a.dv2);
        stage_run(ic<bwd6_f0(1)>{}, ic<4>{}, ic<8>{}, ic<0>{}, ic<256>{}, ic<0>{}, tiles, 8, a.dv1);
        stage_run(ic<bwd6_f0(2)>{}, ic<4>{}, ic<8>{}, ic<0>{}, ic<256>{}, ic<0>{}, tiles, 7, a.dv0);
        stage_run(ic<bwd6_f0(3)>{}, ic<8>{}, ic<9>{}, ic<1>{}, ic<256>{}, ic<0>{},
                  [&](auto Q, auto S_) {
                      constexpr int q = decltype(Q)::value, s = decltype(S_)::value;
                      if constexpr (s < 8) return Pt[s >> 1].p[q][s & 1];
                      else return in_sig[q];
                  },
                  6, a.da[7]);
        finish_pass6<kX6KFrags * (kBwdHeadFrags / 2), bwd6_f0(4)>(ws);
        stage_run(ic<bwd6_f0(4)>{}, ic<8>{}, ic<16>{}, ic<0>{}, ic<256>{}, ic<0>{}, tiles, 5, a.da[6]);
#pragma unroll 1
        for (int L = 6; L >= 2; --L)
            stage_run(ic<bwd6_f0(5)>{}, ic<8>{}, ic<16>{}, ic<0>{}, ic<256>{}, ic<8>{}, tiles, L - 2, a.da[L - 1]);
        stage_run(ic<bwd6_f0(10)>{}, ic<8>{}, ic<16>{}, ic<1>{}, ic<256>{}, ic<8>{}, tiles, -1, a.da[0]);
    }
    __builtin_amdgcn_s_waitcnt(0);
    __syncthreads();
}

}

int launch_delta_chain_x6(const float* packed_bwd, const float* acts, int64_t p_pad, const float* d_rgb, float* dv0,
                          float* dv2, float* dv1, float* const da[8], hipStream_t s, int max_grid, int* grid_out) {
    if (p_pad <= 0) return IDN_OK;
    if (p_pad % 128) return fail(IDN_EINVAL, "delta chain: p_pad %lld is not a multiple of 128", (long long)p_pad);
    static LaunchSetup setup;
    int num_cu = 0;
    if (int e = setup.get([]() -> int {
            IDN_HIP_CHECK(hipFuncSetAttribute(reinterpret_cast<const void*>(&x6::delta_chain_x6_kernel),
                                              hipFuncAttributeMaxDynamicSharedMemorySize, x6::kDelta6Lds));
            return IDN_OK;
        }, &num_cu))
        return e;
    const int64_t ntiles = p_pad / 128;
    const int grid = chain_grid(ntiles, num_cu, max_grid);
    DeltaArgs a{packed_bwd, acts, (long)p_pad, d_rgb, dv0, dv2, dv1, {}};
    for (int l = 0; l < 8; ++l) a.da[l] = da[l];
    ProfScope prof(s, p_pad, IDN_PROF_DELTA_CHAIN_X6);
    hipLaunchKernelGGL(x6::delta_chain_x6_kernel, dim3(grid), dim3(256), x6::kDelta6Lds, s, a);
    IDN_HIP_CHECK(hipGetLastError());
    if (grid_out) *grid_out = grid;
    return IDN_OK;
}

size_t delta_chain_workspace_bytes() { return bwd_stream_floats_x6() * sizeof(float); }

int launch_delta_chain_alone(const idn_facenerf_params& p, int pipe, const float* acts, int64_t p_pad, const float* d_rgb,
                             float* dv0, float* dv21, float* da, int max_blocks, int* blocks_out, void* ws, size_t ws_bytes,
                             hipStream_t s) {
    if (!acts || !d_rgb || !dv0 || !dv21 || !da) return fail(IDN_EINVAL, "delta_chain: NULL pointer");
    if (p_pad <= 0 || p_pad % 128) return fail(IDN_EINVAL, "delta_chain: p_pad %lld is not a positive multiple of 128", (long long)p_pad);
    if (p_pad > (int64_t)1 << 24) return fail(IDN_EUNSUPPORTED, "delta_chain: p_pad %lld exceeds 2^24", (long long)p_pad);
    if (pipe != IDN_DW_PIPE_BF16X6 && pipe != IDN_DW_PIPE_F32) return fail(IDN_EINVAL, "delta_chain: pipe %d", pipe);
    if (max_blocks < 0) return fail(IDN_EINVAL, "delta_chain: max_blocks %d < 0", max_blocks);
    for (const void* q : {(const void*)acts, (const void*)d_rgb, (const void*)dv0, (const void*)dv21, (const void*)da, (const void*)ws})
        if ((uintptr_t)q & 15) return fail(IDN_EINVAL, "delta_chain: operands are not 16-byte aligned");
    if (!ws || ws_bytes < delta_chain_workspace_bytes())
        return fail(IDN_EWORKSPACE, "delta_chain workspace %zu < %zu", ws_bytes, delta_chain_workspace_bytes());
    float* wbwd = static_cast<float*>(ws);
    float* dal[8];
    for (int l = 0; l < 8; ++l) dal[l] = da + (size_t)l * (size_t)p_pad * 256;
    int grid = 0;
    if (pipe == IDN_DW_PIPE_BF16X6) {
        if (int e = launch_pack_bf16x6_bwd(p, wbwd, s)) return e;
        if (int e = launch_delta_chain_x6(wbwd, acts, p_pad, d_rgb, dv0, dv21, dv21 + 128, dal, s, max_blocks, &grid)) return e;
    } else {
        if (int e = launch_pack_f32_bwd(p, wbwd, s)) return e;
        if (int e = launch_delta_chain(wbwd, acts, p_pad, d_rgb, dv0, dv21, dv21 + 128, dal, s, max_blocks, &grid)) return e;
    }
    if (blocks_out) *blocks_out = grid;
    return IDN_OK;
}

}
```

ideal-nerf_amd/csrc/train.hip:

```cpp
#include "dw_gemm.h"
#include "march.h"
#include <cstdlib>

namespace idn {

__device__ __forceinline__ double shfl_up_dd(double v, int delta) {
    int lo = __double2loint(v), hi = __double2hiint(v);
    lo = __shfl_up(lo, delta, 64);
    hi = __shfl_up(hi, delta, 64);
    return __hiloint2double(hi, lo);
}
__device__ __forceinline__ double shfl_down_dd(double v, int delta) {
    int lo = __double2loint(v), hi = __double2hiint(v);
    lo = __shfl_down(lo, delta, 64);
    hi = __shfl_down(hi, delta, 64);
    return __hiloint2double(hi, lo);
}
__device__ __forceinline__ double shfl_xor_dd(double v, int mask) {
    int lo = __double2loint(v), hi = __double2hiint(v);
    lo = __shfl_xor(lo, mask, 64);
    hi = __shfl_xor(hi, mask, 64);
    return __hiloint2double(hi, lo);
}

// ... 147 lines not shown
        const int c = rel >> 6, lane = rel & 63;
        if (c >= C) return;
        double s = 0.0;
        for (int n = lane; n < IDN_W; n += 64)
            s += (double)d.p.pts_w[0][(long)n * ld0 + PC + c] * (double)d.db0[n] +
                 (double)d.p.pts_w[5][(long)n * ld5 + PC + c] * (double)d.db5[n];
#pragma unroll
        for (int m = 32; m >= 1; m >>= 1) s += shfl_xor_dd(s, m);
        const int e = c - d.p.dim_aud;
        const bool want_expr = d.d_expr != nullptr && e >= 0 && e < d.p.dim_expr;
        double sv = 0.0;
        if (want_expr) {
            for (int n = lane; n < IDN_W / 2; n += 64)
                sv += (double)d.p.views_w[0][(long)n * ldv + IDN_W + VC + e] * (double)d.dbv[n];
#pragma unroll
            for (int m = 32; m >= 1; m >>= 1) sv += shfl_xor_dd(sv, m);
        }
        if (lane != 0) return;
        if (c < d.p.dim_aud) {
            if (d.d_aud) d.d_aud[c] += (float)s;
        } else if (c >= d.p.dim_aud + d.p.dim_expr) {
            if (d.d_latent) d.d_latent[c - d.p.dim_aud - d.p.dim_expr] += (float)s;
        } else if (want_expr) {
            d.d_expr[e] += (float)((s + sv) / 3.0);
        }
    }
}

__global__ __launch_bounds__(256) void colsum_rows_kernel(const float* m0, const float* m1, long rows, long rows_per_block, double* part) {
    const float* m = blockIdx.y ? m1 : m0;
    const long r0 = (long)blockIdx.x * rows_per_block;
    const long r1 = r0 + rows_per_block < rows ? r0 + rows_per_block : rows;
    const float* col = m + threadIdx.x;
    double acc = 0.0;
    long r = r0;
    for (; r + 8 <= r1; r += 8) {
        float v[8];
#pragma unroll
        for (int i = 0; i < 8; ++i) v[i] = col[(r + i) * 256];
#pragma unroll
        for (int i = 0; i < 8; ++i) acc += (double)v[i];
    }
    for (; r < r1; ++r) acc += (double)col[r * 256];
    part[((long)blockIdx.x * 2 + blockIdx.y) * 256 + threadIdx.x] = acc;
}
__global__ __launch_bounds__(256) void colsum_finish_kernel(const double* part, int blocks, float* out) {
    double acc = 0.0;
    for (int b = 0; b < blocks; ++b) acc += part[((long)b * 2 + blockIdx.x) * 256 + threadIdx.x];
    out[blockIdx.x * 256 + threadIdx.x] = (float)acc;
}
constexpr int kCondColsumBlocks = 512;
static_assert(512 + (size_t)kCondColsumBlocks * 512 * 2 <= kCpartPoolFloats, "the conditioning-only column sums fit the cpart pool");

struct BwdWs {
    float *dA[8], *dV[2], *dV0, *dRGB, *part, *cpart, *wbwd;
    size_t bytes;
};
static BwdWs carve_bwd(char* base, int64_t p_pad) {
    BwdWs w;
    size_t off = 0;
    auto take = [&](size_t floats) {
        float* p = reinterpret_cast<float*>(base + off);
        off += al256(floats * 4);
        return p;
    };
    for (int l = 0; l < 8; ++l) w.dA[l] = take((size_t)p_pad * 256);
    w.dV[0] = take((size_t)p_pad * 256);
    w.dV[1] = w.dV[0] + 128;
    w.dV0 = take((size_t)p_pad * 256);
    w.dRGB = take((size_t)p_pad * 64);
    w.part = take(kPartPoolFloats);
    w.cpart = take(kCpartPoolFloats);
    w.wbwd = take(bwd_stream_floats_x6());
    w.bytes = off;
    return w;
}

size_t bwd_workspace_bytes(int64_t n_points) {
    const int64_t p_pad = (n_points + 127) / 128 * 128;
    return carve_bwd(nullptr, p_pad).bytes;
}

static int backward_pipe() {
    static const int v = [] {
        const char* e = getenv("IDN_BACKWARD_PIPE");
        return (e && e[0] == 'f' && e[1] == '3' && e[2] == '2' && e[3] == 0) ? kPipeF32 : kPipeX6;
    }();
    return v;
}

static int bwd_tail(const idn_facenerf_params& p, const idn_facenerf_grads* grads, const BwdCond& cond, const float* acts, int64_t P,
                    int64_t Pp, const BwdWs& w, hipStream_t s) {
    const int C = p.dim_aud + p.dim_expr + p.dim_latent;
    const int PC = pts_ch_of(p), VC = views_ch_of(p);
    const int ld0 = PC + C, ld5 = PC + C + IDN_W, ldv = IDN_W + VC + p.dim_expr;
    auto act = [&](int i) { return acts + (size_t)act_off(i) * Pp; };
    auto a_l = [&](int l) { return act(kActA1 + l - 1); };
    auto v_l = [&](int l) { return act(kActV1 + l - 1); };
#define TRY(x) do { if (int e_ = (x)) return e_; } while (0)
    const int pipe = backward_pipe();
    if (pipe == kPipeX6) {
        TRY(launch_pack_bf16x6_bwd(p, w.wbwd, s));
        TRY(launch_delta_chain_x6(w.wbwd, acts, Pp, w.dRGB, w.dV0, w.dV[0], w.dV[1], w.dA, s));
    } else {
        TRY(launch_pack_f32_bwd(p, w.wbwd, s));
        TRY(launch_delta_chain(w.wbwd, acts, Pp, w.dRGB, w.dV0, w.dV[0], w.dV[1], w.dA, s));
    }
    if (!grads) {
        const bool want_dbv = cond.d_expr != nullptr || cond.d_vb != nullptr;
        if (C == 0 && !want_dbv) return IDN_OK;
        float* db = w.cpart;
        double* part = reinterpret_cast<double*>(w.cpart + 512);
        const int64_t chunks = Pp / 128;
        const int64_t rows_per_block = (chunks + kCondColsumBlocks - 1) / kCondColsumBlocks * 128;
        if (C > 0) {
            const int blocks = (int)((Pp + rows_per_block - 1) / rows_per_block);
            hipLaunchKernelGGL(colsum_rows_kernel, dim3(blocks, 2), dim3(256), 0, s, (const float*)w.dA[0], (const float*)w.dA[5], (long)Pp,
                               (long)rows_per_block, part);
            IDN_HIP_CHECK(hipGetLastError());
            hipLaunchKernelGGL(colsum_finish_kernel, dim3(2), dim3(256), 0, s, (const double*)part, blocks, db);
            IDN_HIP_CHECK(hipGetLastError());
        }
        float* dbv = cond.d_vb ? cond.d_vb : w.part;
        if (want_dbv) {
            const int blocks = (int)((P + rows_per_block - 1) / rows_per_block);
            hipLaunchKernelGGL(colsum_rows_kernel, dim3(blocks, 1), dim3(128), 0, s, (const float*)w.dV0, (const float*)w.dV0, (long)P,
                               (long)rows_per_block, part);
            IDN_HIP_CHECK(hipGetLastError());
            hipLaunchKernelGGL(colsum_finish_kernel, dim3(1), dim3(128), 0, s, (const double*)part, blocks, dbv);
            IDN_HIP_CHECK(hipGetLastError());
        }
        if (C == 0) return IDN_OK;
        FoldBwdArgs f{p, cond.aud, cond.expr, cond.latent, db, db + 256, dbv, nullptr, nullptr, nullptr, cond.d_aud, cond.d_latent, cond.d_expr};
        hipLaunchKernelGGL(fold_bwd_kernel<true>, dim3((C * 64 + 255) / 256), dim3(256), 0, s, f);
        IDN_HIP_CHECK(hipGetLastError());
        return IDN_OK;
    }
    const idn_facenerf_grads& gr = *grads;
    DwPass q(w.part, kPartPoolFloats, w.cpart, kCpartPoolFloats, Pp, pipe, kX6ItemsPerPass, s);
    DwProduct h;
    TRY(q.product(w.dRGB, 64, 64, v_l(3), 128, 128, true, &h));
    TRY(q.take_colsum(h, 0, 3, gr.rgb_b));
    TRY(q.take(h, 0, 0, 3, 128, gr.rgb_w, 128));
    if (pipe == kPipeX6) {
        TRY(q.product(w.dV[0], 256, 256, v_l(2), 128, 256, true, &h, v_l(1)));
        TRY(q.take_colsum(h, 0, 128, gr.views_b[2]));
        TRY(q.take_colsum(h, 128, 128, gr.views_b[1]));
        TRY(q.take(h, 0, 0, 128, 128, gr.views_w[2], 128));
        TRY(q.take(h, 128, 128, 128, 128, gr.views_w[1], 128));
    } else {
        for (int l = 2; l >= 1; --l) {
            TRY(q.product(w.dV[2 - l], 256, 128, v_l(l), 128, 128, true, &h));
            TRY(q.take_colsum(h, 0, 128, gr.views_b[l]));
            TRY(q.take(h, 0, 0, 128, 128, gr.views_w[l], 128));
        }
    }
    TRY(q.product(w.dV0, 256, 256, a_l(8), 256, 256, true, &h));
    TRY(q.take_colsum(h, 0, 128, gr.views_b[0]));
    TRY(q.take_colsum(h, kSigmaChannel, 1, gr.alpha_b));
    TRY(q.take(h, 0, 0, 128, 256, gr.views_w[0], ldv));
    TRY(q.take(h, kSigmaChannel, 0, 1, 256, gr.alpha_w, 256));
    TRY(q.product(w.dV0, 256, 128, act(kActDir), 64, 64, false, &h));
    TRY(q.take(h, 0, 0, 128, VC, gr.views_w[0] + IDN_W, ldv));
    for (int l = 7; l >= 1; --l) {
        TRY(q.product(w.dA[l], 256, 256, a_l(l), 256, 256, true, &h));
        TRY(q.take_colsum(h, 0, 256, gr.pts_b[l]));
        TRY(q.take(h, 0, 0, 256, 256, l == 5 ? gr.pts_w[5] + PC + C : gr.pts_w[l], l == 5 ? ld5 : 256));
        if (l == 5) {
            TRY(q.product(w.dA[5], 256, 256, act(kActX0), 64, 64, false, &h));
            TRY(q.take(h, 0, 0, 256, PC, gr.pts_w[5], ld5));
        }
    }
    TRY(q.product(w.dA[0], 256, 256, act(kActX0), 64, 64, true, &h));
    TRY(q.take_colsum(h, 0, 256, gr.pts_b[0]));
    TRY(q.take(h, 0, 0, 256, PC, gr.pts_w[0], ld0));
    TRY(q.finish());
#undef TRY
    {
        FoldBwdArgs f{p, cond.aud, cond.expr, cond.latent, gr.pts_b[0], gr.pts_b[5], gr.views_b[0], gr.pts_w[0], gr.pts_w[5],
                      gr.views_w[0], cond.d_aud, cond.d_latent, cond.d_expr};
        const int total = IDN_W * C + (IDN_W / 2) * p.dim_expr + C * 64;
        if (total > 0) {
            hipLaunchKernelGGL(fold_bwd_kernel<false>, dim3((total + 255) / 256), dim3(256), 0, s, f);
            IDN_HIP_CHECK(hipGetLastError());
        }
    }
    return IDN_OK;
}

static int launch_dx(const idn_facenerf_params& p, const BwdWs& w, int64_t n, int64_t Pp, float* d_x, hipStream_t s);

template <bool kNorm>
static void launch_composite_bwd_spl(const CompBwdArgs& a, hipStream_t s) {
    const dim3 grid((unsigned)((a.n_rays + 3) / 4)), block(256);
    switch ((a.S + 63) / 64) {
        case 1: hipLaunchKernelGGL((composite_bwd_kernel<1, kNorm>), grid, block, 0, s, a); break;
        case 2: hipLaunchKernelGGL((composite_bwd_kernel<2, kNorm>), grid, block, 0, s, a); break;
        case 3: hipLaunchKernelGGL((composite_bwd_kernel<3, kNorm>), grid, block, 0, s, a); break;
        case 4: hipLaunchKernelGGL((composite_bwd_kernel<4, kNorm>), grid, block, 0, s, a); break;
        case 5: hipLaunchKernelGGL((composite_bwd_kernel<5, kNorm>), grid, block, 0, s, a); break;
        case 6: hipLaunchKernelGGL((composite_bwd_kernel<6, kNorm>), grid, block, 0, s, a); break;
        case 7: hipLaunchKernelGGL((composite_bwd_kernel<7, kNorm>), grid, block, 0, s, a); break;
        default: hipLaunchKernelGGL((composite_bwd_kernel<8, kNorm>), grid, block, 0, s, a); break;
    }
}

int launch_composite_bwd(const CompBwdArgs& a, hipStream_t s) {
    if (a.S < 2 || a.S > 64 * kMaxSpl) return fail(IDN_EUNSUPPORTED, "composite_bwd: n_samples %d outside [2, %d]", a.S, 64 * kMaxSpl);
    if (a.d_norm) launch_composite_bwd_spl<true>(a, s);
    else launch_composite_bwd_spl<false>(a, s);
    IDN_HIP_CHECK(hipGetLastError());
    return IDN_OK;
}

int launch_pass_bwd(const PassBwd& b, hipStream_t s) {
    const idn_facenerf_params& p = *b.p;
    const int64_t n_rays = b.n_rays; const int S = b.S;
    float* const d_rays = b.d_rays;
    const int64_t P = n_rays * S;
    const int64_t Pp = (P + 127) / 128 * 128;
    if (S < 2 || S > 64 * kMaxSpl) return fail(IDN_EUNSUPPORTED, "pass_bwd: n_samples %d outside [2, %d]", S, 64 * kMaxSpl);
    const BwdWs w = carve_bwd(reinterpret_cast<char*>(b.ws), Pp);
    if (!b.ws || b.ws_bytes < w.bytes) return fail(IDN_EWORKSPACE, "backward workspace %zu < %zu", b.ws_bytes, w.bytes);

    IDN_HIP_CHECK(hipMemsetAsync(w.dRGB, 0, (size_t)Pp * 64 * 4, s));
    if (Pp > P) IDN_HIP_CHECK(hipMemsetAsync(w.dV0 + (size_t)P * 256, 0, (size_t)(Pp - P) * 256 * 4, s));
    {
        CompBwdArgs a{reinterpret_cast<const float4*>(b.raw), b.z, b.rays, b.bc, b.g_rgb, b.g_fg, b.g_lw, b.g_acc,
                      w.dRGB, 64, w.dV0 + kSigmaChannel, 256, (long)n_rays, S, d_rays ? d_rays + 6 : nullptr, IDN_RAY_FLOATS};
        if (int e = launch_composite_bwd(a, s)) return e;
    }
    if (int e = bwd_tail(p, b.grads, b.cond, b.acts, P, Pp, w, s)) return e;
    if (d_rays) {
        float* d_x = w.dA[1];
        static_assert(IDN_PTS_CH + IDN_VIEWS_CH <= 256, "the input-row gradient fits a delta matrix");
        if (int e = launch_dx(p, w, P, Pp, d_x, s)) return e;
        return launch_ray_grad(d_x, pts_ch_of(p), views_ch_of(p), b.rays, b.z, n_rays, S, d_rays, s);
    }
    return IDN_OK;
}

__global__ __launch_bounds__(256) void head_seed_kernel(const float* g_out, long n, long p_pad, float* d_rgb, float* dv0) {
    const long idx = (long)blockIdx.x * 256 + threadIdx.x;
    const long p = idx >> 4;
    const int q = (int)(idx & 15);
    if (p >= p_pad) return;
    f32x4 v = {0.f, 0.f, 0.f, 0.f};
    if (q == 0 && p < n) v = f32x4{g_out[p * 4 + 0], g_out[p * 4 + 1], g_out[p * 4 + 2], 0.f};
    *reinterpret_cast<f32x4*>(d_rgb + p * 64 + 4 * q) = v;
    if (q == 0) dv0[p * 256 + kSigmaChannel] = p < n ? g_out[p * 4 + 3] : 0.f;
}

constexpr int kDxFrags = 2 * 64 + 16;
constexpr int kDxLds = kDxFrags * kFragBytes;
constexpr int kDxWaves = 16;
static_assert(kDxLds <= 160 * 1024, "the fragments must fit a CU's LDS");
struct DxArgs {
    const float* w0; int ld0;
    const float* w5; int ld5;
    const float* wv; int ldv;
    const float* dA0; const float* dA5; const float* dV0;
    long n, p_pad;
    float* d_x;
    int pts_ch, views_ch;
};
__global__ __launch_bounds__(64 * kDxWaves, 1) void dx_kernel(DxArgs a) {
    extern __shared__ __attribute__((aligned(16))) f32x4 dx_frag[];
    const int tid = threadIdx.x, lane = tid & 63;
    const int wave = __builtin_amdgcn_readfirstlane(tid >> 6);
    const int j = lane & 31, hh = lane >> 5;
    for (int e = tid; e < kDxFrags * 64; e += 64 * kDxWaves) {
        const int f = e >> 6, i = e & 31, h = (e >> 5) & 1;
        float v[4];
        for (int t = 0; t < 4; ++t) {
            if (f < 128) {
                const int g = f >> 1, col = 32 * (f & 1) + i, k = 8 * g + 4 * h + t;
                const float* row = k < IDN_W ? a.w0 + (long)k * a.ld0 : a.w5 + (long)(k - IDN_W) * a.ld5;
                v[t] = col < a.pts_ch ? row[col] : 0.f;
            } else {
                const int k = 8 * (f - 128) + 4 * h + t;
                v[t] = i < a.views_ch ? a.wv[(long)k * a.ldv + IDN_W + i] : 0.f;
            }
        }
        dx_frag[e] = f32x4{v[0], v[1], v[2], v[3]};
    }
// ... 86 lines not shown
```

ideal-nerf_amd/ops.py:

```python
import contextlib
import ctypes as C
import os
from typing import Dict, Optional

import torch

from . import _lib
from ._lib import IDN_PREC_F32, RAY_FLOATS, IdealNerfError, check

PTS_CH, VIEWS_CH, W_HID = 63, 27, 256


def embed_channels(multires: int, views: bool = False) -> int:
    limit = _lib.MAX_MULTIRES_VIEWS if views else _lib.MAX_MULTIRES
    name = "multires_views" if views else "multires"
    if not 0 <= int(multires) <= limit:
        raise NotImplementedError(f"{name}={multires}: libidealnerf is compiled for {name} in 0..{limit} "
                                  f"({3 + 6 * limit} input channels at the most)")
    return 3 + 6 * int(multires)


def check_input_channels(input_ch: int, input_ch_views: int):
    for ch, name, flag, limit in ((input_ch, "input_ch", "multires", _lib.MAX_MULTIRES),
                                  (input_ch_views, "input_ch_views", "multires_views", _lib.MAX_MULTIRES_VIEWS)):
# ... 146 lines not shown
        out = torch.empty((n, 4), dtype=torch.float32, device=x.device)
        acts = torch.empty(lib.idealnerf_train_acts_floats(n), dtype=torch.float32, device=x.device)
        check(lib.idealnerf_facenerf_train_fwd_ch(_ptr(packed, "packed"), _ptr(folded, "folded"), precision, _ptr(x, "x"),
                                                  pts_ch, views_ch, n, out.data_ptr(), acts.data_ptr(), L.stream))
    return out, acts


def grads_struct(grads: Dict[str, torch.Tensor]):
    g = _lib.FaceNerfGrads()
    for i in range(8):
        g.pts_w[i] = grads[f"pts_linears.{i}.weight"].data_ptr()
        g.pts_b[i] = grads[f"pts_linears.{i}.bias"].data_ptr()
    for i in range(3):
        g.views_w[i] = grads[f"views_linears.{i}.weight"].data_ptr()
        g.views_b[i] = grads[f"views_linears.{i}.bias"].data_ptr()
    g.alpha_w, g.alpha_b = grads["alpha_linear.weight"].data_ptr(), grads["alpha_linear.bias"].data_ptr()
    g.rgb_w, g.rgb_b = grads["rgb_linear.weight"].data_ptr(), grads["rgb_linear.bias"].data_ptr()
    return g


def facenerf_bwd(p, grads, aud, expr, latent, acts, g_out, d_x=None, d_aud=None, d_expr=None, d_latent=None):
    lib = _lib.load()
    _shape(g_out, "g_out", None, 4)
    n = g_out.shape[0]
    _shape(acts, "acts", lib.idealnerf_train_acts_floats(n))
    _shape(d_x, "d_x", n, sum(widths(p)))
    for t, name, dim in ((aud, "aud", p.dim_aud), (expr, "expr", p.dim_expr), (latent, "latent", p.dim_latent),
                         (d_aud, "d_aud", p.dim_aud), (d_expr, "d_expr", p.dim_expr), (d_latent, "d_latent", p.dim_latent)):
        _shape(t, name, dim)
    for k, t in grads.items():
        _ptr(t, f"grad {k}")
    with _Launch(aud, expr, latent, acts, g_out, d_x, d_aud, d_expr, d_latent, *grads.values()) as L:
        ptrs = [_ptr(t, name) for t, name in ((aud, "aud"), (expr, "expr"), (latent, "latent"), (acts, "acts"))]
        ptrs += [n, _ptr(g_out, "g_out")]
        ptrs += [_ptr(t, name) for t, name in ((d_x, "d_x"), (d_aud, "d_aud"), (d_expr, "d_expr"), (d_latent, "d_latent"))]
        ws = _workspace(lib.idealnerf_facenerf_bwd_workspace_bytes(n), g_out.device, L.stream)
        check(lib.idealnerf_facenerf_bwd(C.byref(p), C.byref(grads_struct(grads)), *ptrs, ws.data_ptr(), ws.numel(), L.stream))
    return grads


def query_rays_train_fwd(packed, folded, rays, z, precision=_lib.IDN_PREC_BF16X6):
    lib = _lib.load()
    _shape(z, "z", None, None)
    n, S = z.shape
    _shape(rays, "rays", n, RAY_FLOATS)
    with _Launch(packed, folded, rays, z) as L:
        raw = torch.empty((n, S, 4), dtype=torch.float32, device=z.device)
        acts = torch.empty(lib.idealnerf_train_acts_floats(n * S), dtype=torch.float32, device=z.device)
        check(lib.idealnerf_query_rays_train_fwd(_ptr(packed, "packed"), _ptr(folded, "folded"), precision, _ptr(rays, "rays"),
                                                 _ptr(z, "z"), n, S, raw.data_ptr(), acts.data_ptr(), L.stream))
    return raw, acts


def _pass_bwd(p, grads, aud, expr, latent, acts, raw, z, rays, bc, g_rgb, g_fg, g_lw, g_acc, d_aud, d_latent, d_views0_bias=None,
              d_rays=None, with_rays=False, d_expr=None, ex=False):
    lib = _lib.load()
    if grads is None:
        grads = {}
    n, S = z.shape
    for t, name, shape in ((raw, "raw", (n, S, 4)), (rays, "rays", (n, RAY_FLOATS)), (bc, "bc_rgb", (n, 3)),
                           (g_rgb, "g_rgb_map", (n, 3)), (g_fg, "g_rgb_fg", (n, 3)), (g_lw, "g_last_weight", (n,)),
                           (g_acc, "g_acc", (n,)), (d_rays, "d_rays", (n, RAY_FLOATS)), (d_expr, "d_expr", (p.dim_expr,))):
        _shape(t, name, *shape)
    tensors = (aud, expr, latent, acts, raw, z, rays, bc, g_rgb, g_fg, g_lw, g_acc, d_aud, d_latent)
    with _Launch(*tensors, d_rays, d_expr, d_views0_bias if ex else None, *grads.values()) as L:
        ws = _workspace(lib.idealnerf_pass_bwd_workspace_bytes(n, S), z.device, L.stream)
        ptrs = [_ptr(t) for t in tensors]
        if ex:
            _shape(d_views0_bias, "d_views0_bias", W_HID // 2)
            extra = _lib.PassBwdExtra(_ptr(d_expr, "d_expr"), _ptr(d_rays, "d_rays"), _ptr(d_views0_bias, "d_views0_bias"))
            check(lib.idealnerf_pass_bwd_ex(C.byref(p), C.byref(grads_struct(grads)) if grads else None, *ptrs[:8], n, S, *ptrs[8:],
                                            C.byref(extra), ws.data_ptr(), ws.numel(), L.stream))
        elif with_rays:
            check(lib.idealnerf_pass_bwd_rays(C.byref(p), C.byref(grads_struct(grads)), *ptrs[:8], n, S, *ptrs[8:], _ptr(d_rays, "d_rays"),
                                              ws.data_ptr(), ws.numel(), L.stream))
        elif grads:
            check(lib.idealnerf_pass_bwd(C.byref(p), C.byref(grads_struct(grads)), *ptrs[:8], n, S, *ptrs[8:], ws.data_ptr(), ws.numel(), L.stream))
        else:
            check(lib.idealnerf_pass_bwd_cond(C.byref(p), *ptrs[:8], n, S, *ptrs[8:], ws.data_ptr(), ws.numel(), L.stream))
    return grads


def pass_bwd(p, grads, aud, expr, latent, acts, raw, z, rays, bc, g_rgb, g_fg, g_lw, g_acc, d_aud, d_latent):
    return _pass_bwd(p, grads, aud, expr, latent, acts, raw, z, rays, bc, g_rgb, g_fg, g_lw, g_acc, d_aud, d_latent)


def pass_bwd_rays(p, grads, aud, expr, latent, acts, raw, z, rays, bc, g_rgb, g_fg, g_lw, g_acc, d_aud, d_latent, d_rays):
    return _pass_bwd(p, grads, aud, expr, latent, acts, raw, z, rays, bc, g_rgb, g_fg, g_lw, g_acc, d_aud, d_latent,
                     d_rays=d_rays, with_rays=True)


def pass_bwd_cond(p, aud, expr, latent, acts, raw, z, rays, bc, g_rgb, g_fg, g_lw, g_acc, d_aud, d_latent, d_views0_bias=None):
    if d_views0_bias is not None and d_aud is None and d_latent is None:
        raise IdealNerfError("pass_bwd_cond: d_views0_bias needs d_aud or d_latent (with neither the pass is not run)")
    _pass_bwd(p, None, aud, expr, latent, acts, raw, z, rays, bc, g_rgb, g_fg, g_lw, g_acc, d_aud, d_latent, d_views0_bias,
              ex=d_views0_bias is not None)


def pass_bwd_ex(p, grads, aud, expr, latent, acts, raw, z, rays, bc, g_rgb, g_fg, g_lw, g_acc, d_aud, d_latent, d_expr=None,
                d_rays=None, d_views0_bias=None):
    return _pass_bwd(p, grads, aud, expr, latent, acts, raw, z, rays, bc, g_rgb, g_fg, g_lw, g_acc, d_aud, d_latent,
                     d_views0_bias=d_views0_bias, d_rays=d_rays, d_expr=d_expr, ex=True)


def query_rays_fwd(packed, folded, rays, z, precision=IDN_PREC_F32) -> torch.Tensor:
    lib = _lib.load()
    _shape(z, "z", None, None)
    n, S = z.shape
    _shape(rays, "rays", n, RAY_FLOATS)
    _net_buffers(lib, packed, folded, precision)
    with _Launch(packed, folded, rays, z) as L:
        raw = torch.empty((n, S, 4), dtype=torch.float32, device=z.device)
        check(lib.idealnerf_query_rays_fwd(_ptr(packed, "packed"), _ptr(folded, "folded"), precision, _ptr(rays, "rays"),
                                           _ptr(z, "z"), n, S, raw.data_ptr(), L.stream))
    return raw


def query_points_fwd(packed, folded, pts, viewdirs, precision=IDN_PREC_F32) -> torch.Tensor:
    lib = _lib.load()
    _shape(pts, "pts", None, None, 3)
    n, S, _ = pts.shape
    _shape(viewdirs, "viewdirs", n, 3)
    _net_buffers(lib, packed, folded, precision)
    with _Launch(packed, folded, pts, viewdirs) as L:
        raw = torch.empty((n, S, 4), dtype=torch.float32, device=pts.device)
        check(lib.idealnerf_query_points_fwd(_ptr(packed, "packed"), _ptr(folded, "folded"), precision, _ptr(pts, "pts"),
                                             _ptr(viewdirs, "viewdirs"), n, S, raw.data_ptr(), L.stream))
    return raw


def frame_rays(c2w, H, W, focal, near, far, row0=0, nrows=None, cx=None, cy=None, device="cuda") -> torch.Tensor:
    lib = _lib.load()
    nrows = H - row0 if nrows is None else nrows
    if not (0 <= row0 and 0 <= nrows and row0 + nrows <= H and W > 0):
        raise IdealNerfError(f"rows [{row0}, {row0 + nrows}) are outside a {H}x{W} frame")
    if tuple(c2w.shape[-2:]) not in ((3, 4), (4, 4)) or c2w.dim() != 2:
        raise IdealNerfError(f"c2w must be [3, 4] or [4, 4], got {list(c2w.shape)}")
# ... 135 lines not shown
    _shape(bins, "bins", None, None)
    n, nb = bins.shape
    _shape(weights, "weights", n, nb - 1)
    per_ray = _u_shape(u, n)
    ni = u.shape[-1]
    dev = bins.device
    with _Launch(bins, weights, u) as L:
        o = dict(z_samples=torch.empty((n, ni), dtype=torch.float32, device=dev),
                 inds=torch.empty((n, ni), dtype=torch.int64, device=dev),
                 cdf=torch.empty((n, nb), dtype=torch.float32, device=dev))
        check(lib.idealnerf_sample_pdf_bins_fwd(_ptr(bins, "bins"), _ptr(weights, "weights"), _ptr(u, "u"), per_ray, n,
                                                nb, ni, o["z_samples"].data_ptr(), o["inds"].data_ptr(),
                                                o["cdf"].data_ptr(), L.stream))
    return o


def invert_cdf(cdf, bins, u):
    lib = _lib.load()
    _shape(cdf, "cdf", None, None)
    n, nb = cdf.shape
    _shape(bins, "bins", n, nb)
    per_ray = _u_shape(u, n)
    ni = u.shape[-1]
    with _Launch(cdf, bins, u) as L:
        zs = torch.empty((n, ni), dtype=torch.float32, device=cdf.device)
        inds = torch.empty((n, ni), dtype=torch.int64, device=cdf.device)
        check(lib.idealnerf_invert_cdf(_ptr(cdf, "cdf"), _ptr(bins, "bins"), _ptr(u, "u"), per_ray, n, nb, ni,
                                       zs.data_ptr(), inds.data_ptr(), L.stream))
    return zs, inds


def dw_gemm(delta, acts, pipe=0, with_bias=True):
    lib = _lib.load()
    _shape(delta, "delta", None, None)
    rows = delta.shape[0]
    _shape(acts, "acts", rows, None)
    with _Launch(delta, acts) as L:
        dW = torch.empty((256, 256), dtype=torch.float32, device=delta.device)
        db = torch.empty(256, dtype=torch.float32, device=delta.device) if with_bias else None
        nbytes = lib.idealnerf_dw_gemm_workspace_bytes()
        ws = _workspace(nbytes, delta.device, L.stream)
        check(lib.idealnerf_dw_gemm(_ptr(delta, "delta"), delta.shape[1], _ptr(acts, "acts"), acts.shape[1], rows, dW.data_ptr(),
                                    None if db is None else db.data_ptr(), int(pipe), ws.data_ptr(), ws.numel(), L.stream))
    return dW, db


DW_SHAPES = ((256, 256), (256, 64), (128, 256), (128, 64), (128, 128), (64, 128))
DW_MAX_X6_ITEMS, DW_MAX_REDUCE_ITEMS = 12, 32


_dw_products_ws = {}


def dw_products(rows, products, pipe=0, x6_items=1):
    lib = _lib.load()
    E = IdealNerfError
    if not 1 <= len(products) <= _lib.DW_MAX_PRODUCTS:
        raise E(f"dw_products: {len(products)} products outside [1, {_lib.DW_MAX_PRODUCTS}]")
    if pipe not in (0, 1):
        raise E(f"dw_products: pipe {pipe}")
    if rows <= 0 or rows % 128:
        raise E(f"dw_products: rows {rows} is not a positive multiple of 128")
    if pipe == 0 and not 1 <= x6_items <= DW_MAX_X6_ITEMS:
        raise E(f"dw_products: x6_items {x6_items} outside [1, {DW_MAX_X6_ITEMS}]")
    n_x6 = n_red = 0
    tensors = []
    for i, t in enumerate(products):
        N, K = int(t["N"]), int(t["K"])
        if (N, K) not in DW_SHAPES:
            raise E(f"dw_products: product {i}: no instantiation for {N} x {K}")
        _shape(t["delta"], f"product {i}: delta", rows, None)
        _shape(t["acts"], f"product {i}: acts", rows, None)
        b_cols = K if t.get("acts2") is None else 128
        if t["delta"].shape[1] < N or t["acts"].shape[1] < b_cols:
            raise E(f"dw_products: product {i}: row pitch {t['delta'].shape[1]} / {t['acts'].shape[1]} < {N} / {b_cols}")
        d0 = int(t.get("delta_col0", 0))
        if d0 < 0 or d0 % 4 or d0 + N > t["delta"].shape[1]:
            raise E(f"dw_products: product {i}: delta columns {d0} .. {d0 + N} of {t['delta'].shape[1]}")
        x6 = pipe == 0 and (N, K) == (256, 256)
        if t.get("acts2") is not None:
            if not x6:
                raise E(f"dw_products: product {i}: a split B needs the 256 x 256 bf16-piece kernel")
            _shape(t["acts2"], f"product {i}: acts2", rows, t["acts"].shape[1])
        n_x6 += x6
        if n_x6 > x6_items:
            raise E(f"dw_products: more 256 x 256 products than x6_items ({x6_items})")
        takes, ctakes = t.get("takes", ()), t.get("colsum_takes", ())
        if len(takes) > _lib.DW_MAX_TAKES or len(ctakes) > _lib.DW_MAX_COLSUM_TAKES:
            raise E(f"dw_products: product {i}: {len(takes)} takes / {len(ctakes)} column-sum takes")
        if ctakes and not t.get("colsum"):
            raise E(f"dw_products: product {i} kept no column sums")
        n_red += len(takes) + len(ctakes)
        if n_red > DW_MAX_REDUCE_ITEMS:
            raise E(f"dw_products: more than {DW_MAX_REDUCE_ITEMS} takes in one pass")
        for j, (row0, col0, nr, nc, out, o_r, o_c) in enumerate(takes):
            if min(row0, col0) < 0 or min(nr, nc) < 1 or row0 + nr > N or col0 + nc > K:
                raise E(f"dw_products: product {i} take {j} leaves the {N} x {K} block")
            _shape(out, f"product {i} take {j}: out", None, None)
            if min(o_r, o_c) < 0 or o_r + nr > out.shape[0] or o_c + nc > out.shape[1]:
                raise E(f"dw_products: product {i} take {j} does not fit out {list(out.shape)}")
            tensors.append(out)
        for j, (col0, nc, out, o0) in enumerate(ctakes):
            if col0 < 0 or nc < 1 or col0 + nc > N:
                raise E(f"dw_products: product {i} column-sum take {j} leaves the {N} columns")
            _shape(out, f"product {i} column-sum take {j}: out", None)
            if o0 < 0 or o0 + nc > out.shape[0]:
                raise E(f"dw_products: product {i} column-sum take {j} does not fit out {list(out.shape)}")
            tensors.append(out)
        tensors += [t["delta"], t["acts"], t.get("acts2")]
    with _Launch(*tensors) as L:
        recs = (_lib.DwProduct * len(products))()
        for r, t in zip(recs, products):
            r.delta, r.ld_delta, r.N = _ptr(t["delta"], "delta") + 4 * int(t.get("delta_col0", 0)), t["delta"].shape[1], int(t["N"])
            r.acts, r.ld_acts, r.K = _ptr(t["acts"], "acts"), t["acts"].shape[1], int(t["K"])
            r.acts2, r.want_colsum = _ptr(t.get("acts2"), "acts2"), int(bool(t.get("colsum")))
            takes, ctakes = t.get("takes", ()), t.get("colsum_takes", ())
            r.n_takes, r.n_colsum_takes = len(takes), len(ctakes)
            for k, (row0, col0, nr, nc, out, o_r, o_c) in zip(r.takes, takes):
                k.row0, k.col0, k.rows, k.cols, k.ldo = row0, col0, nr, nc, out.shape[1]
                k.out = _ptr(out, "out") + 4 * (o_r * out.shape[1] + o_c)
            for k, (col0, nc, out, o0) in zip(r.colsum_takes, ctakes):
                k.col0, k.cols, k.out = col0, nc, _ptr(out, "out") + 4 * o0
        nbytes = lib.idealnerf_dw_products_workspace_bytes()
        key = (str(L.device), int(L.stream))
        ws = _dw_products_ws.get(key)
        if ws is None:
            ws = _dw_products_ws[key] = torch.zeros(nbytes, dtype=torch.uint8, device=L.device)
        check(lib.idealnerf_dw_products(rows, int(pipe), int(x6_items), recs, len(products), ws.data_ptr(), ws.numel(), L.stream))
        return [(r.splits, r.chunks_per_split) for r in recs]


_delta_chain_ws = {}


def delta_chain(p, pipe, acts, d_rgb, dv0, max_blocks=0, dv21=None, da=None):
    lib = _lib.load()
    E = IdealNerfError
    if not isinstance(p, _lib.FaceNerfParams):
        raise E("delta_chain: p must be a params_struct")
    if pipe not in (0, 1):
        raise E(f"delta_chain: pipe {pipe}")
    if isinstance(max_blocks, bool) or not isinstance(max_blocks, int) or max_blocks < 0:
        raise E(f"delta_chain: max_blocks {max_blocks} < 0")
    _shape(dv0, "dv0", None, 256)
    p_pad = dv0.shape[0]
    if p_pad <= 0 or p_pad % 128 or p_pad > 1 << 24:
        raise E(f"delta_chain: p_pad {p_pad} is not a positive multiple of 128 up to 2^24")
    _shape(acts, "acts", lib.idealnerf_train_acts_floats(p_pad))
    _shape(d_rgb, "d_rgb", p_pad, 64)
    _shape(dv21, "dv21", p_pad, 256)
    _shape(da, "da", 8, p_pad, 256)
    for t, name in ((acts, "acts"), (d_rgb, "d_rgb"), (dv0, "dv0"), (dv21, "dv21"), (da, "da")):
        if t is not None and t.dtype != torch.float32:
            raise E(f"{name} must be {torch.float32} (got {t.dtype})")
    with _Launch(acts, d_rgb, dv0, dv21, da) as L:
        ptrs = [_ptr(t, name) for t, name in ((acts, "acts"), (d_rgb, "d_rgb"), (dv0, "dv0"))]
        if dv21 is None:
            dv21 = torch.empty((p_pad, 256), dtype=torch.float32, device=L.device)
        if da is None:
            da = torch.empty((8, p_pad, 256), dtype=torch.float32, device=L.device)
        ptrs += [_ptr(dv21, "dv21"), _ptr(da, "da")]
        if any(q % 16 for q in ptrs):
            raise E("delta_chain: operands are not 16-byte aligned")
        key = str(L.device)
        ws = _delta_chain_ws.get(key)
        if ws is None:
            ws = _delta_chain_ws[key] = torch.zeros(lib.idealnerf_delta_chain_workspace_bytes(), dtype=torch.uint8, device=L.device)
        blocks = C.c_int(0)
        check(lib.idealnerf_delta_chain(C.byref(p), int(pipe), ptrs[0], p_pad, ptrs[1], ptrs[2], ptrs[3], ptrs[4], int(max_blocks),
                                        C.byref(blocks), ws.data_ptr(), ws.numel(), L.stream))
    return dv21, da, blocks.value


def composite_bwd(raw, z, rays, bc, g_rgb=None, g_fg=None, g_lw=None, g_acc=None, d_rgb=None, d_sig=None, sig_col=0, d_norm=None,
                  norm_col=0):
    lib = _lib.load()
    E = IdealNerfError
    if z is None:
        raise E("composite_bwd: z is None")
    _shape(z, "z", None, None)
    n, S = z.shape
# ... 453 lines not shown
```

include/idealnerf.h:

```cpp
#ifndef IDEALNERF_H
#define IDEALNERF_H

#include <stddef.h>
#include <stdint.h>

#ifdef __cplusplus
extern "C" {
#endif

#define IDN_OK 0
#define IDN_EINVAL (-1)
#define IDN_EUNSUPPORTED (-2)
#define IDN_EHIP (-3)
#define IDN_EWORKSPACE (-4)

#define IDN_W 256
#define IDN_D 8
#define IDN_PTS_CH 63
#define IDN_VIEWS_CH 27
#define IDN_MAX_MULTIRES 10
#define IDN_MAX_MULTIRES_VIEWS 4
#define IDN_RAY_FLOATS 11

#define IDN_PREC_F32 0
// ... 159 lines not shown
float idealnerf_colour_gate_max_dist(void);


size_t idealnerf_train_acts_floats(int64_t n_points);

int idealnerf_query_rays_train_fwd(const float* packed, const float* folded, int precision, const float* rays,
                                   const float* z, int64_t n_rays, int n_samples, float* raw, float* acts,
                                   void* stream);

typedef struct idn_facenerf_grads {
    float* pts_w[8];
    float* pts_b[8];
    float* views_w[3];
    float* views_b[3];
    float* alpha_w;
    float* alpha_b;
    float* rgb_w;
    float* rgb_b;
} idn_facenerf_grads;

size_t idealnerf_pass_bwd_workspace_bytes(int64_t n_rays, int n_samples);

int idealnerf_pass_bwd(const idn_facenerf_params* p, const idn_facenerf_grads* grads, const float* aud,
                       const float* expr, const float* latent, const float* acts, const float* raw, const float* z,
                       const float* rays, const float* bc_rgb, int64_t n_rays, int n_samples, const float* g_rgb_map,
                       const float* g_rgb_fg, const float* g_last_weight, const float* g_acc, float* d_aud,
                       float* d_latent, void* workspace, size_t workspace_bytes, void* stream);

int idealnerf_pass_bwd_rays(const idn_facenerf_params* p, const idn_facenerf_grads* grads, const float* aud,
                            const float* expr, const float* latent, const float* acts, const float* raw, const float* z,
                            const float* rays, const float* bc_rgb, int64_t n_rays, int n_samples, const float* g_rgb_map,
                            const float* g_rgb_fg, const float* g_last_weight, const float* g_acc, float* d_aud,
                            float* d_latent, float* d_rays, void* workspace, size_t workspace_bytes, void* stream);

int idealnerf_pass_bwd_cond(const idn_facenerf_params* p, const float* aud, const float* expr, const float* latent,
                            const float* acts, const float* raw, const float* z, const float* rays, const float* bc_rgb,
                            int64_t n_rays, int n_samples, const float* g_rgb_map, const float* g_rgb_fg,
                            const float* g_last_weight, const float* g_acc, float* d_aud, float* d_latent, void* workspace,
                            size_t workspace_bytes, void* stream);

typedef struct idn_pass_bwd_extra {
    float* d_expr;
    float* d_rays;
    float* d_views0_bias;
} idn_pass_bwd_extra;

int idealnerf_pass_bwd_ex(const idn_facenerf_params* p, const idn_facenerf_grads* grads, const float* aud,
                          const float* expr, const float* latent, const float* acts, const float* raw, const float* z,
                          const float* rays, const float* bc_rgb, int64_t n_rays, int n_samples, const float* g_rgb_map,
                          const float* g_rgb_fg, const float* g_last_weight, const float* g_acc, float* d_aud,
                          float* d_latent, const idn_pass_bwd_extra* extra, void* workspace, size_t workspace_bytes,
                          void* stream);

int idealnerf_facenerf_train_fwd(const float* packed, const float* folded, int precision, const float* x, int64_t n,
                                 float* out, float* acts, void* stream);
int idealnerf_facenerf_train_fwd_ch(const float* packed, const float* folded, int precision, const float* x, int pts_ch,
                                    int views_ch, int64_t n, float* out, float* acts, void* stream);

size_t idealnerf_facenerf_bwd_workspace_bytes(int64_t n);

int idealnerf_facenerf_bwd(const idn_facenerf_params* p, const idn_facenerf_grads* grads, const float* aud, const float* expr,
                           const float* latent, const float* acts, int64_t n, const float* g_out, float* d_x, float* d_aud,
                           float* d_expr, float* d_latent, void* workspace, size_t workspace_bytes, void* stream);

#define IDN_DW_PIPE_BF16X6 0
#define IDN_DW_PIPE_F32 1
#define IDN_DW_PIPE_BF16X6_PASS 2
size_t idealnerf_dw_gemm_workspace_bytes(void);
int idealnerf_dw_gemm(const float* delta, int ld_delta, const float* acts, int ld_acts, int64_t rows, float* dW, float* db,
                      int pipe, void* workspace, size_t workspace_bytes, void* stream);

#define IDN_DW_MAX_PRODUCTS 16
#define IDN_DW_MAX_TAKES 4
#define IDN_DW_MAX_COLSUM_TAKES 2
typedef struct idn_dw_take {
    int row0, col0, rows, cols;
    float* out;
    int ldo;
} idn_dw_take;
typedef struct idn_dw_colsum_take {
    int col0, cols;
    float* out;
} idn_dw_colsum_take;
typedef struct idn_dw_product {
    const float* delta;
    int ld_delta, N;
    const float* acts;
    int ld_acts, K;
    const float* acts2;
    int want_colsum;
    int n_takes;
    idn_dw_take takes[IDN_DW_MAX_TAKES];
    int n_colsum_takes;
    idn_dw_colsum_take colsum_takes[IDN_DW_MAX_COLSUM_TAKES];
    int splits, chunks_per_split;
} idn_dw_product;
size_t idealnerf_dw_products_workspace_bytes(void);
int idealnerf_dw_products(int64_t rows, int pipe, int x6_items, idn_dw_product* products, int n, void* workspace,
                          size_t workspace_bytes, void* stream);

size_t idealnerf_delta_chain_workspace_bytes(void);
int idealnerf_delta_chain(const idn_facenerf_params* p, int pipe, const float* acts, int64_t p_pad, const float* d_rgb,
                          float* dv0, float* dv21, float* da, int max_blocks, int* blocks_out, void* workspace,
                          size_t workspace_bytes, void* stream);

int idealnerf_composite_bwd(const float* raw, const float* z, const float* rays, const float* bc_rgb, int64_t n_rays,
                            int n_samples, const float* g_rgb_map, const float* g_rgb_fg, const float* g_last_weight,
                            const float* g_acc, float* d_rgb, int ld_rgb, float* d_sig, int ld_sig, float* d_norm, int ld_norm,
                            void* stream);

typedef struct idn_audio_net_params {
    const float* conv_w[4];
    const float* conv_b[4];
    const float* fc_w[2];
    const float* fc_b[2];
    int dim_aud;
} idn_audio_net_params;
typedef struct idn_audio_net_grads {
    float* conv_w[4];
    float* conv_b[4];
    float* fc_w[2];
    float* fc_b[2];
} idn_audio_net_grads;
size_t idealnerf_audio_net_saved_floats(int n_windows);
int idealnerf_audio_net_fwd(const idn_audio_net_params* p, const float* windows, int n_windows, float* out, float* saved,
                            void* stream);
int idealnerf_audio_net_bwd(const idn_audio_net_params* p, const idn_audio_net_grads* grads, const float* windows,
                            const float* saved, const float* d_out, int n_windows, void* stream);

int idealnerf_to8b(const float* rgb, int64_t n_pixels, int swap_rb, uint8_t* out, int* nonfinite_flag, void* stream);

int idealnerf_compose_to8b(const float* rgb_head, const float* last_weight, const float* rgb_fg, int64_t n_pixels,
                           int swap_rb, uint8_t* out, uint8_t* fg_out, int* nonfinite_flag, void* stream);

int idealnerf_cull_mark(const float* raw, int64_t n, float sigma_min, uint8_t* corners, void* stream);
int idealnerf_cull_cells(const uint8_t* corners, int G, int dilate, uint32_t* bits, void* stream);

typedef struct idn_cull_grid {
    const uint32_t* bits;
    int G;
    float lo[3];
    float cell;
} idn_cull_grid;
size_t idealnerf_cull_classify_workspace_bytes(int64_t n_pixels);
int idealnerf_cull_classify(const idn_cull_grid* grid, const idn_frame* frame, float dz, int K, int64_t* sel, int32_t* n_live,
                            void* workspace, size_t workspace_bytes, void* stream);
int idealnerf_cull_gather(const int64_t* sel, int64_t n, const idn_frame* frame, const float* bc, float* rays, float* bc_live,
                          void* stream);
#define IDN_CULL_MAX_OUTPUTS 12
typedef struct idn_cull_output {
    float* dense;
    const float* live;
// ... 25 lines not shown
```

Before: 132.7 million.

## Skip dead point chunks in backward weight-gradient GEMMs via a live-chunk list

Adds a live-chunk pass that scans the output-colour and first-layer deltas. It builds a compact list of 16-point chunks whose gradients are nonzero. The weight-gradient GEMM kernels (the TN kernel and the x6 variant) gain a gathered mode that walks only the listed chunks, prefetching list entries with scalar loads, and splits that are left empty write zero partials. It is on by default in the pass backward path, with an option to turn it off and to expose chunk counters; the cost is an extra scan kernel and some indirection inside the GEMM loop.

```diff
diff --git a/ideal-nerf_amd/_lib.py b/ideal-nerf_amd/_lib.py
--- a/ideal-nerf_amd/_lib.py
+++ b/ideal-nerf_amd/_lib.py
@@ -28,6 +28,10 @@
 
 class PassBwdExtra(C.Structure):
     _fields_ = [("d_expr", fp), ("d_rays", fp), ("d_views0_bias", fp)]
+
+
+class PassBwdOpts(C.Structure):
+    _fields_ = [("live_chunks", C.c_int), ("chunk_counters", fp)]
 
 
 class CompositeOut(C.Structure):
@@ -151,6 +155,9 @@
                                           fp, fp, fp, fp, C.c_size_t, fp]),
     "idealnerf_pass_bwd_ex": (C.c_int, [C.POINTER(FaceNerfParams), C.POINTER(FaceNerfGrads), fp, fp, fp, fp, fp, fp, fp,
                                         fp, C.c_int64, C.c_int, fp, fp, fp, fp, fp, fp, C.POINTER(PassBwdExtra), fp, C.c_size_t, fp]),
+    "idealnerf_pass_bwd_opts": (C.c_int, [C.POINTER(FaceNerfParams), C.POINTER(FaceNerfGrads), fp, fp, fp, fp, fp, fp, fp,
+                                          fp, C.c_int64, C.c_int, fp, fp, fp, fp, fp, fp, C.POINTER(PassBwdExtra), C.POINTER(PassBwdOpts),
+                                          fp, C.c_size_t, fp]),
     "idealnerf_facenerf_train_fwd": (C.c_int, [fp, fp, C.c_int, fp, C.c_int64, fp, fp, fp]),
     "idealnerf_facenerf_train_fwd_ch": (C.c_int, [fp, fp, C.c_int, fp, C.c_int, C.c_int, C.c_int64, fp, fp, fp]),
     "idealnerf_facenerf_bwd_workspace_bytes": (C.c_size_t, [C.c_int64]),
@@ -160,6 +167,10 @@
     "idealnerf_dw_gemm": (C.c_int, [fp, C.c_int, fp, C.c_int, C.c_int64, fp, fp, C.c_int, fp, C.c_size_t, fp]),
     "idealnerf_dw_products_workspace_bytes": (C.c_size_t, []),
     "idealnerf_dw_products": (C.c_int, [C.c_int64, C.c_int, C.c_int, C.POINTER(DwProduct), C.c_int, fp, C.c_size_t, fp]),
+    "idealnerf_dw_products_live": (C.c_int, [C.c_int64, C.c_int, C.c_int, C.POINTER(DwProduct), C.c_int, fp, fp, C.c_size_t, fp]),
+    "idealnerf_live_list_ints": (C.c_size_t, [C.c_int64]),
+    "idealnerf_live_chunks_workspace_bytes": (C.c_size_t, [C.c_int64]),
+    "idealnerf_live_chunks": (C.c_int, [fp, fp, C.c_int64, fp, fp, C.c_size_t, fp]),
     "idealnerf_delta_chain_workspace_bytes": (C.c_size_t, []),
     "idealnerf_delta_chain": (C.c_int, [C.POINTER(FaceNerfParams), C.c_int, fp, C.c_int64, fp, fp, fp, fp, C.c_int,
                                         C.POINTER(C.c_int), fp, C.c_size_t, fp]),
diff --git a/ideal-nerf_amd/csrc/capi.hip b/ideal-nerf_amd/csrc/capi.hip
--- a/ideal-nerf_amd/csrc/capi.hip
+++ b/ideal-nerf_amd/csrc/capi.hip
@@ -386,6 +386,7 @@
                        const float* g_rgb_fg, const float* g_last_weight, const float* g_acc, float* d_aud,
                        float* d_latent, void* workspace, size_t workspace_bytes, void* stream) {
     PassBwd b = {};
+    b.live_chunks = 1;
     b.p = p; b.grads = grads;
     b.cond.aud = aud; b.cond.expr = expr; b.cond.latent = latent; b.cond.d_aud = d_aud; b.cond.d_latent = d_latent;
     b.acts = acts; b.raw = raw; b.z = z; b.rays = rays; b.bc = bc_rgb; b.n_rays = n_rays; b.S = n_samples;
@@ -399,6 +400,7 @@
                             const float* g_rgb_fg, const float* g_last_weight, const float* g_acc, float* d_aud,
                             float* d_latent, float* d_rays, void* workspace, size_t workspace_bytes, void* stream) {
     PassBwd b = {};
+    b.live_chunks = 1;
     b.p = p; b.grads = grads;
     b.cond.aud = aud; b.cond.expr = expr; b.cond.latent = latent; b.cond.d_aud = d_aud; b.cond.d_latent = d_latent;
     b.acts = acts; b.raw = raw; b.z = z; b.rays = rays; b.bc = bc_rgb; b.n_rays = n_rays; b.S = n_samples;
@@ -427,12 +429,38 @@
                           float* d_latent, const idn_pass_bwd_extra* extra, void* workspace, size_t workspace_bytes,
                           void* stream) {
     PassBwd b = {};
+    b.live_chunks = 1;
     b.p = p; b.grads = grads;
     b.cond.aud = aud; b.cond.expr = expr; b.cond.latent = latent; b.cond.d_aud = d_aud; b.cond.d_latent = d_latent;
     if (extra) b.cond.d_expr = extra->d_expr, b.cond.d_vb = extra->d_views0_bias, b.d_rays = extra->d_rays;
     b.acts = acts; b.raw = raw; b.z = z; b.rays = rays; b.bc = bc_rgb; b.n_rays = n_rays; b.S = n_samples;
     b.g_rgb = g_rgb_map; b.g_fg = g_rgb_fg; b.g_lw = g_last_weight; b.g_acc = g_acc; b.ws = workspace; b.ws_bytes = workspace_bytes;
     return pass_bwd_any(b, stream);
+}
+
+int idealnerf_pass_bwd_opts(const idn_facenerf_params* p, const idn_facenerf_grads* grads, const float* aud,
+                            const float* expr, const float* latent, const float* acts, const float* raw, const float* z,
+                            const float* rays, const float* bc_rgb, int64_t n_rays, int n_samples, const float* g_rgb_map,
+                            const float* g_rgb_fg, const float* g_last_weight, const float* g_acc, float* d_aud,
+                            float* d_latent, const idn_pass_bwd_extra* extra, const idn_pass_bwd_opts* opts, void* workspace,
+                            size_t workspace_bytes, void* stream) {
+    if (opts && opts->live_chunks != 0 && opts->live_chunks != 1) return fail(IDN_EINVAL, "live_chunks %d (1 = on, the default; 0 = off)", opts->live_chunks);
+    PassBwd b = {};
+    b.live_chunks = opts ? opts->live_chunks : 1;
+    b.chunk_counters = opts ? opts->chunk_counters : nullptr;
+    b.p = p; b.grads = grads;
+    b.cond.aud = aud; b.cond.expr = expr; b.cond.latent = latent; b.cond.d_aud = d_aud; b.cond.d_latent = d_latent;
+    if (extra) b.cond.d_expr = extra->d_expr, b.cond.d_vb = extra->d_views0_bias, b.d_rays = extra->d_rays;
+    b.acts = acts; b.raw = raw; b.z = z; b.rays = rays; b.bc = bc_rgb; b.n_rays = n_rays; b.S = n_samples;
+    b.g_rgb = g_rgb_map; b.g_fg = g_rgb_fg; b.g_lw = g_last_weight; b.g_acc = g_acc; b.ws = workspace; b.ws_bytes = workspace_bytes;
+    return pass_bwd_any(b, stream);
+}
+
+size_t idealnerf_live_list_ints(int64_t p_pad) { return p_pad > 0 ? live_list_ints(p_pad) : 0; }
+size_t idealnerf_live_chunks_workspace_bytes(int64_t p_pad) { return p_pad > 0 ? live_chunks_workspace_bytes(p_pad) : 0; }
+int idealnerf_live_chunks(const float* d_rgb, const float* dv0, int64_t p_pad, int* list, void* workspace, size_t workspace_bytes,
+                          void* stream) {
+    return launch_live_chunks_alone(d_rgb, dv0, p_pad, list, workspace, workspace_bytes, (hipStream_t)stream);
 }
 
 int idealnerf_facenerf_train_fwd(const float* packed, const float* folded, int precision, const float* x, int64_t n,
@@ -484,7 +512,11 @@
 
 int idealnerf_dw_products(int64_t rows, int pipe, int x6_items, idn_dw_product* products, int n, void* workspace,
                           size_t workspace_bytes, void* stream) {
-    return launch_dw_products(rows, pipe, x6_items, products, n, workspace, workspace_bytes, (hipStream_t)stream);
+    return launch_dw_products(rows, pipe, x6_items, products, n, nullptr, workspace, workspace_bytes, (hipStream_t)stream);
+}
+int idealnerf_dw_products_live(int64_t rows, int pipe, int x6_items, idn_dw_product* products, int n, const int* live,
+                               void* workspace, size_t workspace_bytes, void* stream) {
+    return launch_dw_products(rows, pipe, x6_items, products, n, live, workspace, workspace_bytes, (hipStream_t)stream);
 }
 
 size_t idealnerf_delta_chain_workspace_bytes(void) { return delta_chain_workspace_bytes(); }
diff --git a/ideal-nerf_amd/csrc/dw_gemm.h b/ideal-nerf_amd/csrc/dw_gemm.h
--- a/ideal-nerf_amd/csrc/dw_gemm.h
+++ b/ideal-nerf_amd/csrc/dw_gemm.h
@@ -20,6 +20,14 @@
 struct TNBatch {
     TNArgs it[kMaxTnBatch];
     int n, splits;
+};
+struct TNArgsG {
+    TNArgs g;
+    const int* live;
+};
+struct TNBatchG {
+    TNBatch b;
+    const int* live;
 };
 constexpr int kMaxReduceItems = 32;
 struct ReduceItem {
@@ -66,8 +74,9 @@
 struct DwProduct { const float *part, *cpart; int splits, N, K, chunks_per_split; };
 
 struct DwPass {
-    DwPass(float* part, size_t part_floats, float* cpart, size_t cpart_floats, int64_t P, int pipe, int x6_items, hipStream_t s)
-        : part_next(part), part_left(part_floats), cpart_next(cpart), cpart_left(cpart_floats), P(P), pipe(pipe), x6_items(x6_items), s(s) {}
+    DwPass(float* part, size_t part_floats, float* cpart, size_t cpart_floats, int64_t P, int pipe, int x6_items, hipStream_t s,
+           const int* live = nullptr)
+        : part_next(part), part_left(part_floats), cpart_next(cpart), cpart_left(cpart_floats), P(P), pipe(pipe), x6_items(x6_items), s(s), live(live) {}
     int product(const float* A, int lda, int N, const float* B, int ldb, int K, bool want_colsum, DwProduct* h, const float* B2 = nullptr);
     int take(const DwProduct& h, int row0, int col0, int rows, int cols, float* out, int ldo);
     int take_colsum(const DwProduct& h, int col0, int cols, float* out);
@@ -79,6 +88,7 @@
     int64_t P;
     int pipe, x6_items;
     hipStream_t s;
+    const int* live;
     TNBatch x6{{}, 0, 0};
     ReduceBatch red{{}, 0};
     int red_blocks = 0;
diff --git a/ideal-nerf_amd/csrc/dw_gemm.hip b/ideal-nerf_amd/csrc/dw_gemm.hip
--- a/ideal-nerf_amd/csrc/dw_gemm.hip
+++ b/ideal-nerf_amd/csrc/dw_gemm.hip
@@ -41,13 +41,19 @@
     else asm volatile("s_waitcnt lgkmcnt(2)" : "+v"(a.v), "+v"(b.v)::"memory");
 }
 
+__device__ __forceinline__ void live_fetch(int& e, const int* entry) { asm volatile("s_load_dword %0, %1, 0x0" : "=s"(e) : "s"(entry) : "memory"); }
+__device__ __forceinline__ void live_landed(int& e) { asm volatile("s_waitcnt lgkmcnt(0)" : "+s"(e)::"memory"); }
+
 constexpr int kTnRows = 16, kTnBufs = 3;
 constexpr int kTnNarrowBufs = 3;
 constexpr int kTnRows4x1 = 32, kTnRowsThin = 64;
 constexpr int kTnNarrowSplits = 256;
 
-template <int NTW, int KTW, int NB = kTnBufs, int R = kTnRows>
-__global__ __launch_bounds__(256) void gemm_tn_kernel(TNArgs g) {
+__device__ __forceinline__ const TNArgs& tn_args(const TNArgs& a) { return a; }
+__device__ __forceinline__ const TNArgs& tn_args(const TNArgsG& a) { return a.g; }
+template <int NTW, int KTW, int NB = kTnBufs, int R = kTnRows, bool G = false>
+__global__ __launch_bounds__(256) void gemm_tn_kernel(std::conditional_t<G, TNArgsG, TNArgs> ga) {
+    const TNArgs& g = tn_args(ga);
     static_assert(R % 16 == 0, "chunks are multiples of 16 points");
     constexpr int NPA = NTW * R / 16, NPB = KTW * R / 16;
     static_assert(NB >= 3 && (NB - 2) * (NPA + NPB) <= 63, "vmcnt is a 6-bit field");
@@ -70,28 +76,52 @@
         for (int b = 0; b < KTW; ++b)
             for (int r = 0; r < 16; ++r) acc[a][b][r] = 0.f;
 
-    const long c_begin = (long)split * g.chunks_per_split;
-    long c_end = c_begin + g.chunks_per_split;
-    const long c_total = g.P / R;
+    static_assert(kLiveListPad * 16 % R == 0, "the list's entries are whole chunks");
+    long live_total = 0;
+    if constexpr (G) live_total = ga.live[1] / (R / 16);
+    const long cps = G ? (live_total + (long)gridDim.z - 1) / (long)gridDim.z : (long)g.chunks_per_split;
+    const long c_begin = (long)split * cps;
+    long c_end = c_begin + cps;
+    const long c_total = G ? live_total : g.P / R;
     if (c_end > c_total) c_end = c_total;
+    if constexpr (G) {
+        if (c_begin >= c_end) {
+            float* out = g.part + (long)split * g.N * g.K;
+            for (int j = tid; j < BN * BK; j += 256) out[(long)(n0 + j / BK) * g.K + k0 + j % BK] = 0.0f;
+            if (g.cpart != nullptr && blockIdx.y == 0 && tid < BN) g.cpart[(long)split * g.N + n0 + tid] = 0.0f;
+            return;
+        }
+    }
     const bool colsum_block = g.cpart != nullptr && blockIdx.y == 0;
     const bool do_colsum = colsum_block && tid < BN;
     const int ccol = tid < BN ? tid : 0;
     float csum = 0.0f;
 
     constexpr int kRowsPerPieceA = 256 / BN > 0 ? 256 / BN : 1, kRowsPerPieceB = 256 / BK > 0 ? 256 / BK : 1;
-    const __amdgpu_buffer_rsrc_t rsrcA = __builtin_amdgcn_make_buffer_rsrc(const_cast<float*>(g.A + n0 + c_begin * R * (long)g.lda), 0, 0xfffffffc, 0x00020000);
-    const __amdgpu_buffer_rsrc_t rsrcB = __builtin_amdgcn_make_buffer_rsrc(const_cast<float*>(g.B + k0 + c_begin * R * (long)g.ldb), 0, 0xfffffffc, 0x00020000);
+    const __amdgpu_buffer_rsrc_t rsrcA = __builtin_amdgcn_make_buffer_rsrc(const_cast<float*>(G ? g.A + n0 : g.A + n0 + c_begin * R * (long)g.lda), 0, 0xfffffffc, 0x00020000);
+    const __amdgpu_buffer_rsrc_t rsrcB = __builtin_amdgcn_make_buffer_rsrc(const_cast<float*>(G ? g.B + k0 : g.B + k0 + c_begin * R * (long)g.ldb), 0, 0xfffffffc, 0x00020000);
     const uint32_t voffA = ((lane / (BN / 4)) * g.lda + (lane % (BN / 4)) * 4) * 4;
     const uint32_t voffB = ((lane / (BK / 4)) * g.ldb + (lane % (BK / 4)) * 4) * 4;
     const uint32_t rowA = g.lda * 4, rowB = g.ldb * 4;
+    const int* entries = nullptr;
+    if constexpr (G) entries = ga.live + kLiveListHeader + w * R / 64;
+    auto entry_of = [&](long c) { return entries + c * (R / 16); };
+    int e_piece = 0;
     auto piece_a = [&](long c, int buf, int ja) {
         const int pc = NPA * w + ja;
+        if constexpr (G)
+            __builtin_amdgcn_raw_ptr_buffer_load_lds(rsrcA, (__attribute__((address_space(3))) void*)(tn_smem + buf * kTileFloats + pc * 256), 16, voffA,
+                                                     (uint32_t)(16 * e_piece + (pc * kRowsPerPieceA) % 16) * rowA, 0, 0);
+        else
         __builtin_amdgcn_raw_ptr_buffer_load_lds(rsrcA, (__attribute__((address_space(3))) void*)(tn_smem + buf * kTileFloats + pc * 256), 16, voffA,
                                                  (uint32_t)(((c - c_begin) * R + pc * kRowsPerPieceA) * rowA), 0, 0);
     };
     auto piece_b = [&](long c, int buf, int jb) {
         const int pc = NPB * w + jb;
+        if constexpr (G)
+            __builtin_amdgcn_raw_ptr_buffer_load_lds(rsrcB, (__attribute__((address_space(3))) void*)(tn_smem + buf * kTileFloats + R * BN + pc * 256), 16, voffB,
+                                                     (uint32_t)(16 * e_piece + (pc * kRowsPerPieceB) % 16) * rowB, 0, 0);
+        else
         __builtin_amdgcn_raw_ptr_buffer_load_lds(rsrcB, (__attribute__((address_space(3))) void*)(tn_smem + buf * kTileFloats + R * BN + pc * 256), 16, voffB,
                                                  (uint32_t)(((c - c_begin) * R + pc * kRowsPerPieceB) * rowB), 0, 0);
     };
@@ -102,10 +132,15 @@
     const uint32_t smem0 = (uint32_t)(uintptr_t)(__attribute__((address_space(3))) float*)tn_smem;
     const uint32_t a_addr0 = smem0 + (hh * BN + NTW * (32 * wr + i)) * 4;
     const uint32_t b_addr0 = smem0 + (R * BN + hh * BK + KTW * (32 * wc + i)) * 4;
-    for (int ahead = 0; ahead < NB - 1; ++ahead)
+    for (int ahead = 0; ahead < NB - 1; ++ahead) {
+        if constexpr (G) e_piece = *entry_of(c_begin + ahead < c_end ? c_begin + ahead : c_end - 1);
         for (int j = 0; j < NP; ++j) piece(c_begin + ahead < c_end ? c_begin + ahead : c_end - 1, ahead, j);
+    }
+    int e_fetch = 0;
+    if constexpr (G) e_piece = *entry_of(c_begin + NB - 1 < c_end ? c_begin + NB - 1 : c_end - 1);
     int buf = 0;
     for (long c = c_begin; c < c_end; ++c) {
+        if constexpr (G) live_fetch(e_fetch, entry_of(c + NB < c_end ? c + NB : c_end - 1));
         asm volatile("s_waitcnt vmcnt(%0)" ::"n"((NB - 2) * NP) : "memory");
         __builtin_amdgcn_s_barrier();
         asm volatile("" ::: "memory");
@@ -231,6 +266,10 @@
             lds_retire<0>(a1v, b1v);
         }
         lds_retire<0>(a0v, b0v);
+        if constexpr (G) {
+            live_landed(e_fetch);
+            e_piece = e_fetch;
+        }
         buf = buf + 1 == NB ? 0 : buf + 1;
     }
     asm volatile("s_waitcnt vmcnt(0)" ::: "memory");
@@ -272,7 +311,8 @@
     asm volatile("s_waitcnt lgkmcnt(%3)" : "+v"(f[0].v), "+v"(f[1].v), "+v"(f[2].v) : "n"(N) : "memory");
 }
 
-__device__ __forceinline__ void gemm_tn_x6_item(const TNArgs& g, const int split, char* x6_smem) {
+template <bool G>
+__device__ __forceinline__ void gemm_tn_x6_item(const TNArgs& g, const int split, char* x6_smem, const int* live = nullptr, const int n_splits = 0) {
     const int tid = threadIdx.x, lane = tid & 63;
     const int w = __builtin_amdgcn_readfirstlane(tid >> 6);
     const int i = lane & 31, hh = lane >> 5;
@@ -284,17 +324,32 @@
         for (int b = 0; b < 4; ++b)
             for (int r = 0; r < 16; ++r) acc[a][b][r] = 0.f;
 
-    const long c_begin = (long)split * g.chunks_per_split;
+    long c_begin = (long)split * g.chunks_per_split;
     long c_end = c_begin + g.chunks_per_split;
-    const long c_total = g.P / kTnRows;
+    long c_total = g.P / kTnRows;
+    if constexpr (G) {
+        c_total = live[1];
+        const long cps = (c_total + n_splits - 1) / n_splits;
+        c_begin = split * cps;
+        c_end = c_begin + cps;
+    }
     if (c_end > c_total) c_end = c_total;
     const int n_chunks = (int)(c_end - c_begin);
+    if constexpr (G) {
+        if (n_chunks <= 0) {
+            float* out = g.part + (long)split * g.N * g.K;
+            for (int j = tid; j < 65536 / 4; j += 256) reinterpret_cast<f32x4*>(out)[j] = f32x4{0.f, 0.f, 0.f, 0.f};
+            if (g.cpart != nullptr) g.cpart[(long)split * g.N + tid] = 0.0f;
+            return;
+        }
+    }
+    const int* const entries = G ? live + kLiveListHeader + c_begin : nullptr;
     auto make_rsrc = [](const float* ptr) {
         const uint64_t a64 = (uint64_t)(uintptr_t)ptr;
         return tn_i32x4{(int)(uint32_t)a64, (int)((uint32_t)(a64 >> 32) & 0xffffu), (int)0xfffffffcu, 0x00020000};
     };
-    const tn_i32x4 rsrcA = make_rsrc(g.A + c_begin * kTnRows * (long)g.lda);
-    const tn_i32x4 rsrcB = make_rsrc(g.B + c_begin * kTnRows * (long)g.ldb);
+    const tn_i32x4 rsrcA = make_rsrc(G ? g.A : g.A + c_begin * kTnRows * (long)g.lda);
+    const tn_i32x4 rsrcB = make_rsrc(G ? g.B : g.B + c_begin * kTnRows * (long)g.ldb);
     const int voff = tid * 4;
     const int voffB = g.b_split ? (tid < 128 ? g.b_off0 : g.b_off1) + (tid & 127) * 4 : voff;
     const int rowA = g.lda * 4, rowB = g.ldb * 4;
@@ -306,7 +361,8 @@
     };
     auto load_row = [&](float& dst, const tn_i32x4& rsrc, int soff) { load_row_at(dst, rsrc, soff, voff); };
     auto load_chunk = [&](int rc) {
-        const int base = (rc < n_chunks ? rc : n_chunks - 1) * kTnRows;
+        int base = (rc < n_chunks ? rc : n_chunks - 1) * kTnRows;
+        if constexpr (G) base = entries[rc < n_chunks ? rc : n_chunks - 1] * kTnRows;
 #pragma unroll
         for (int p = 0; p < kTnRows; ++p) load_row(ra[p], rsrcA, (base + p) * rowA);
 #pragma unroll
@@ -343,6 +399,8 @@
     split_store(0, 0, ra);
     split_store(0, 1, rb);
     load_chunk(1);
+    int e_next = 0;
+    if constexpr (G) e_next = entries[2 < n_chunks ? 2 : n_chunks - 1];
     asm volatile("s_waitcnt lgkmcnt(0)" ::: "memory");
     __builtin_amdgcn_s_barrier();
     asm volatile("" ::: "memory");
@@ -389,7 +447,7 @@
         x6_retire<0>(fa[2]);
         x6_retire<0>(fa[3]);
         const unsigned live_mask = rc + 1 < n_chunks ? 0xffffffffu : 0u;
-        const int nbase = (rc + 2 < n_chunks ? rc + 2 : n_chunks - 1) * kTnRows;
+        const int nbase = G ? e_next * kTnRows : (rc + 2 < n_chunks ? rc + 2 : n_chunks - 1) * kTnRows;
         char* const dst = my_slot + (buf ^ 1) * kX6BufBytes;
         unsigned pw[2][3][8];
         float t0 = 0.f, t1 = 0.f;
@@ -442,8 +500,13 @@
             constexpr int kX1 = 26;
             if constexpr (k < kX1) slice(ic<0>{}, ic<k>{});
             else slice(ic<1>{}, ic<k - kX1>{});
+            if constexpr (G && k == 2 * kX1) live_fetch(e_next, entries + (rc + 3 < n_chunks ? rc + 3 : n_chunks - 1));
             if constexpr (k == 59) {
-                asm volatile("s_waitcnt lgkmcnt(0)" ::: "memory");
+                if constexpr (G) {
+                    live_landed(e_next);
+                } else {
+                    asm volatile("s_waitcnt lgkmcnt(0)" ::: "memory");
+                }
                 __builtin_amdgcn_s_barrier();
                 asm volatile("" ::: "memory");
                 issue_first_row(a_base + (buf ^ 1) * kX6BufBytes, b_base + (buf ^ 1) * kX6BufBytes);
@@ -470,7 +533,13 @@
     extern __shared__ __attribute__((aligned(16))) char x6_smem[];
     const int item = __builtin_amdgcn_readfirstlane((int)blockIdx.z / b.splits);
     const int split = __builtin_amdgcn_readfirstlane((int)blockIdx.z - item * b.splits);
-    gemm_tn_x6_item(b.it[item], split, x6_smem);
+    gemm_tn_x6_item<false>(b.it[item], split, x6_smem);
+}
+__global__ __launch_bounds__(256) void gemm_tn_x6_live_kernel(TNBatchG b) {
+    extern __shared__ __attribute__((aligned(16))) char x6_smem[];
+    const int item = __builtin_amdgcn_readfirstlane((int)blockIdx.z / b.b.splits);
+    const int split = __builtin_amdgcn_readfirstlane((int)blockIdx.z - item * b.b.splits);
+    gemm_tn_x6_item<true>(b.b.it[item], split, x6_smem, b.live, b.b.splits);
 }
 
 __global__ __launch_bounds__(256) void reduce_batch_kernel(ReduceBatch b) {
@@ -511,15 +580,37 @@
     IDN_HIP_CHECK(hipGetLastError());
     return IDN_OK;
 }
-struct DwShape { int N, K, rows_per_chunk, max_splits; int (*launch)(const TNArgs&, int, hipStream_t); };
-constexpr DwShape kX6Shape = {256, 256, kTnRows, kMaxSplits, nullptr};
+template <int NTW, int KTW, int NB, int R>
+static int launch_tn_live(const TNArgs& g, const int* live, int splits, hipStream_t s) {
+    constexpr size_t lds = (size_t)NB * R * (size_t)(64 * NTW + 64 * KTW) * 4;
+    static LaunchSetup setup;
+    int num_cu = 0;
+    if (int e = setup.get([]() -> int {
+            IDN_HIP_CHECK(hipFuncSetAttribute(reinterpret_cast<const void*>(&gemm_tn_kernel<NTW, KTW, NB, R, true>),
+                                              hipFuncAttributeMaxDynamicSharedMemorySize, (int)lds));
+            return IDN_OK;
+        }, &num_cu))
+        return e;
+    hipLaunchKernelGGL((gemm_tn_kernel<NTW, KTW, NB, R, true>), dim3(g.N / (64 * NTW), g.K / (64 * KTW), splits), dim3(256), lds, s, TNArgsG{g, live});
+    IDN_HIP_CHECK(hipGetLastError());
+    return IDN_OK;
+}
+struct DwShape {
+    int N, K, rows_per_chunk, max_splits;
+    int (*launch)(const TNArgs&, int, hipStream_t);
+    int (*launch_live)(const TNArgs&, const int*, int, hipStream_t);
+};
+constexpr DwShape kX6Shape = {256, 256, kTnRows, kMaxSplits, nullptr, nullptr};
 constexpr DwShape kF32Shapes[] = {
-    {256, 256, kTnRows, kMaxSplits, &launch_tn<4, 4, kTnBufs>},
-    {256, 64, kTnRows4x1, kTnNarrowSplits, &launch_tn<4, 1, kTnNarrowBufs, kTnRows4x1>},
-    {128, 256, kTnRows, kMaxSplits, &launch_tn<2, 4, kTnBufs>},
-    {128, 64, kTnRowsThin, kTnNarrowSplits, &launch_tn<2, 1, kTnNarrowBufs, kTnRowsThin>},
-    {128, 128, kTnRows, kMaxSplits, &launch_tn<2, 2, kTnBufs>},
-    {64, 128, kTnRowsThin, kTnNarrowSplits, &launch_tn<1, 2, kTnNarrowBufs, kTnRowsThin>},
+    {256, 256, kTnRows, kMaxSplits, &launch_tn<4, 4, kTnBufs>, nullptr},
+    {256, 64, kTnRows4x1, kTnNarrowSplits, &launch_tn<4, 1, kTnNarrowBufs, kTnRows4x1>,
+     &launch_tn_live<4, 1, kTnNarrowBufs, kTnRows4x1>},
+    {128, 256, kTnRows, kMaxSplits, &launch_tn<2, 4, kTnBufs>, nullptr},
+    {128, 64, kTnRowsThin, kTnNarrowSplits, &launch_tn<2, 1, kTnNarrowBufs, kTnRowsThin>,
+     &launch_tn_live<2, 1, kTnNarrowBufs, kTnRowsThin>},
+    {128, 128, kTnRows, kMaxSplits, &launch_tn<2, 2, kTnBufs>, nullptr},
+    {64, 128, kTnRowsThin, kTnNarrowSplits, &launch_tn<1, 2, kTnNarrowBufs, kTnRowsThin>,
+     &launch_tn_live<1, 2, kTnNarrowBufs, kTnRowsThin>},
 };
 static_assert(kTnNarrowSplits <= kMaxSplits, "the pools hold kMaxSplits splits of every product of a pass (dw_gemm.h)");
 
@@ -527,6 +618,7 @@
     static LaunchSetup st;
     return st.get([]() -> int {
         IDN_HIP_CHECK(hipFuncSetAttribute(reinterpret_cast<const void*>(&gemm_tn_x6_kernel), hipFuncAttributeMaxDynamicSharedMemorySize, kX6Lds));
+        IDN_HIP_CHECK(hipFuncSetAttribute(reinterpret_cast<const void*>(&gemm_tn_x6_live_kernel), hipFuncAttributeMaxDynamicSharedMemorySize, kX6Lds));
         return IDN_OK;
     }, cus);
 }
@@ -540,6 +632,12 @@
     if (!sh) return fail(IDN_EUNSUPPORTED, "gemm_tn: no instantiation for %d x %d", N, K);
     const bool queued = sh->launch == nullptr;
     if (B2 && !queued) return fail(IDN_EINVAL, "gemm_tn: a split B needs the 256 x 256 bf16-piece kernel");
+    if (live) {
+        if (!queued && !sh->launch_live) return fail(IDN_EUNSUPPORTED, "gemm_tn: %d x %d on the fp32 pipe takes no live-chunk list", N, K);
+        const int64_t ld_max = lda > ldb ? lda : ldb;
+        if (P * ld_max * 4 + ((int64_t)1 << 31) > (int64_t)0xffffffffLL)
+            return fail(IDN_EUNSUPPORTED, "gemm_tn: %lld rows of %lld floats are beyond a live-chunk list's 32-bit offsets", (long long)P, (long long)ld_max);
+    }
     if (P % sh->rows_per_chunk) return fail(IDN_EINVAL, "gemm_tn: %lld rows are not a multiple of the %d-row chunk", (long long)P, sh->rows_per_chunk);
     const long chunks = P / sh->rows_per_chunk;
     int splits = sh->max_splits;
@@ -570,7 +668,7 @@
         x6.it[x6.n++] = g;
     } else {
         ProfScope prof(s, P, IDN_PROF_DW_GEMM);
-        if (int e = sh->launch(g, splits, s)) return e;
+        if (int e = live ? sh->launch_live(g, live, splits, s) : sh->launch(g, splits, s)) return e;
     }
     *h = DwProduct{g.part, g.cpart, splits, N, K, cps};
     part_next += part_floats, part_left -= part_floats;
@@ -592,7 +690,8 @@
 int DwPass::finish() {
     if (x6.n) {
         ProfScope prof(s, P * x6.n, IDN_PROF_DW_GEMM_X6);
-        hipLaunchKernelGGL(gemm_tn_x6_kernel, dim3(1, 1, x6.splits * x6.n), dim3(256), kX6Lds, s, x6);
+        if (live) hipLaunchKernelGGL(gemm_tn_x6_live_kernel, dim3(1, 1, x6.splits * x6.n), dim3(256), kX6Lds, s, TNBatchG{x6, live});
+        else hipLaunchKernelGGL(gemm_tn_x6_kernel, dim3(1, 1, x6.splits * x6.n), dim3(256), kX6Lds, s, x6);
     }
     IDN_HIP_CHECK(hipGetLastError());
     if (red.n) hipLaunchKernelGGL(reduce_batch_kernel, dim3(red_blocks), dim3(256), 0, s, red);
@@ -620,7 +719,7 @@
 }
 
 size_t dw_products_workspace_bytes() { return al256(kPartPoolFloats * 4) + al256(kCpartPoolFloats * 4); }
-int launch_dw_products(int64_t rows, int pipe, int x6_items, idn_dw_product* pr, int n, void* ws, size_t ws_bytes, hipStream_t s) {
+int launch_dw_products(int64_t rows, int pipe, int x6_items, idn_dw_product* pr, int n, const int* live, void* ws, size_t ws_bytes, hipStream_t s) {
     if (!pr) return fail(IDN_EINVAL, "dw_products: NULL pointer");
     if (n < 1 || n > IDN_DW_MAX_PRODUCTS) return fail(IDN_EINVAL, "dw_products: %d products outside [1, %d]", n, IDN_DW_MAX_PRODUCTS);
     if (pipe != kPipeX6 && pipe != kPipeF32) return fail(IDN_EINVAL, "dw_products: pipe %d", pipe);
@@ -637,6 +736,14 @@
         bool known = x6;
         for (const DwShape& sh : kF32Shapes) known = known || (sh.N == t.N && sh.K == t.K);
         if (!known) return fail(IDN_EUNSUPPORTED, "dw_products: product %d: no instantiation for %d x %d", i, t.N, t.K);
+        if (live) {
+            bool gathered = x6;
+            for (const DwShape& sh : kF32Shapes) gathered = gathered || (sh.N == t.N && sh.K == t.K && sh.launch_live && !(t.N == 256 && t.K == 256));
+            if (!gathered) return fail(IDN_EUNSUPPORTED, "dw_products: product %d: %d x %d on the fp32 pipe takes no live-chunk list", i, t.N, t.K);
+            const int64_t ld_max = t.ld_delta > t.ld_acts ? t.ld_delta : t.ld_acts;
+            if (rows * ld_max * 4 + ((int64_t)1 << 31) > (int64_t)0xffffffffLL)
+                return fail(IDN_EUNSUPPORTED, "dw_products: product %d: %lld rows of %lld floats are beyond a live-chunk list's 32-bit offsets", i, (long long)rows, (long long)ld_max);
+        }
         const int b_cols = t.acts2 ? 128 : t.K;
         if (t.ld_delta < t.N || t.ld_acts < b_cols) return fail(IDN_EINVAL, "dw_products: product %d: row pitch %d / %d < %d / %d", i, t.ld_delta, t.ld_acts, t.N, b_cols);
         if (t.ld_delta % 4 || t.ld_acts % 4 || ((uintptr_t)t.delta | (uintptr_t)t.acts | (uintptr_t)t.acts2) % 16)
@@ -673,7 +780,7 @@
         return fail(IDN_EWORKSPACE, "dw_products workspace %zu < %zu", ws_bytes, dw_products_workspace_bytes());
     float* part = reinterpret_cast<float*>(ws);
     float* cpart = reinterpret_cast<float*>(reinterpret_cast<char*>(ws) + al256(kPartPoolFloats * 4));
-    DwPass q(part, kPartPoolFloats, cpart, kCpartPoolFloats, rows, pipe, x6_items, s);
+    DwPass q(part, kPartPoolFloats, cpart, kCpartPoolFloats, rows, pipe, x6_items, s, live);
     for (int i = 0; i < n; ++i) {
         idn_dw_product& t = pr[i];
         DwProduct h;
diff --git a/ideal-nerf_amd/csrc/idn_internal.h b/ideal-nerf_amd/csrc/idn_internal.h
--- a/ideal-nerf_amd/csrc/idn_internal.h
+++ b/ideal-nerf_amd/csrc/idn_internal.h
@@ -261,9 +261,11 @@
                        int* grid_out = nullptr);
 size_t bwd_stream_floats_x6();
 int launch_pack_bf16x6_bwd(const idn_facenerf_params& p, float* packed_bwd, hipStream_t s);
+constexpr int kLiveListPad = 8, kLiveListHeader = 8;
+inline size_t live_list_ints(int64_t p_pad) { return (size_t)kLiveListHeader + (size_t)(p_pad / 16); }
 int launch_delta_chain_x6(const float* packed_bwd, const float* acts, int64_t p_pad, const float* d_rgb, float* dv0,
                           float* dv2, float* dv1, float* const da[8], hipStream_t s, int max_grid = 0,
-                          int* grid_out = nullptr);
+                          int* grid_out = nullptr, const int* live = nullptr);
 size_t delta_chain_workspace_bytes();
 int launch_delta_chain_alone(const idn_facenerf_params& p, int pipe, const float* acts, int64_t p_pad, const float* d_rgb,
                              float* dv0, float* dv21, float* da, int max_blocks, int* blocks_out, void* ws, size_t ws_bytes,
@@ -273,7 +275,8 @@
 int launch_dw_gemm(const float* delta, int ld_delta, const float* acts, int ld_acts, int64_t rows, float* dW, float* db, int pipe,
                    void* ws, size_t ws_bytes, hipStream_t s);
 size_t dw_products_workspace_bytes();
-int launch_dw_products(int64_t rows, int pipe, int x6_items, idn_dw_product* products, int n, void* ws, size_t ws_bytes, hipStream_t s);
+int launch_dw_products(int64_t rows, int pipe, int x6_items, idn_dw_product* products, int n, const int* live, void* ws, size_t ws_bytes,
+                       hipStream_t s);
 
 size_t bwd_workspace_bytes(int64_t n_points);
 struct BwdCond {
@@ -290,10 +293,14 @@
     int S;
     const float *g_rgb, *g_fg, *g_lw, *g_acc;
     float* d_rays;
+    int live_chunks;
+    int64_t* chunk_counters;
     void* ws;
     size_t ws_bytes;
 };
 int launch_pass_bwd(const PassBwd& b, hipStream_t s);
+size_t live_chunks_workspace_bytes(int64_t p_pad);
+int launch_live_chunks_alone(const float* d_rgb, const float* dv0, int64_t p_pad, int* list, void* ws, size_t ws_bytes, hipStream_t s);
 struct CompBwdArgs {
     const float4* raw; const float* z; const float* rays; const float* bc;
     const float* g_rgb;
diff --git a/ideal-nerf_amd/csrc/mlp_f32_bwd.hip b/ideal-nerf_amd/csrc/mlp_f32_bwd.hip
--- a/ideal-nerf_amd/csrc/mlp_f32_bwd.hip
+++ b/ideal-nerf_amd/csrc/mlp_f32_bwd.hip
@@ -443,7 +443,15 @@
 
 constexpr int kDelta6Lds = kX6RingFrags * kFragBytes;
 
-__global__ __launch_bounds__(256, 1) void delta_chain_x6_kernel(DeltaArgs a) {
+struct DeltaArgsG {
+    DeltaArgs a;
+    const int* live;
+};
+__device__ __forceinline__ const DeltaArgs& delta_args(const DeltaArgs& a) { return a; }
+__device__ __forceinline__ const DeltaArgs& delta_args(const DeltaArgsG& a) { return a.a; }
+template <bool G = false>
+__global__ __launch_bounds__(256, 1) void delta_chain_x6_kernel(std::conditional_t<G, DeltaArgsG, DeltaArgs> ga) {
+    const DeltaArgs& a = delta_args(ga);
     extern __shared__ __attribute__((aligned(16))) char smem[];
     char* ring = smem;
     const int tid = threadIdx.x, lane = tid & 63;
@@ -455,11 +463,17 @@
     FragReader fr;
     fr.addr0 = (uint32_t)(uintptr_t)(__attribute__((address_space(3))) char*)ring + lane * 16;
     fr.addr1 = fr.addr0 + 64 * kFragBytes;
-    const long ntiles = a.p_pad >> 7;
+    const long ntiles = [&]() -> long {
+        if constexpr (G) return ga.live[1] >> 3;
+        else return a.p_pad >> 7;
+    }();
     f32x4 pref[3] = {{0.f, 0.f, 0.f, 0.f}, {0.f, 0.f, 0.f, 0.f}, {0.f, 0.f, 0.f, 0.f}};
 
     for (long tile = blockIdx.x; tile < ntiles; tile += gridDim.x) {
-        const long P = tile * 128 + wave * 32 + m;
+        const long P = [&]() -> long {
+            if constexpr (G) return 16 * (long)ga.live[kLiveListHeader + tile * 8 + wave * 2 + (m >> 4)] + (m & 15);
+            else return tile * 128 + wave * 32 + m;
+        }();
         const f32x4 drgb = *reinterpret_cast<const f32x4*>(a.d_rgb + P * 64);
         const float dsig = a.dv0[P * 256 + kSigmaChannel];
         f32x4 in_rgb[3], in_sig[3];
@@ -487,7 +501,10 @@
         f32x16 O[8];
         typedef uint32_t u32x4 __attribute__((ext_vector_type(4)));
         const u32x4* mbase = reinterpret_cast<const u32x4*>(a.acts + (size_t)kActCols * a.p_pad);
-        auto mask_load = [&](int id) { return mbase[mask_index(id, a.p_pad, tile * 4 + wave, lane)]; };
+        auto mask_load = [&](int id) {
+            if constexpr (G) return mbase[mask_index(id, a.p_pad, P >> 5, (int)(P & 31) + 32 * h)];
+            else return mbase[mask_index(id, a.p_pad, tile * 4 + wave, lane)];
+        };
         u32x4 mask_nxt = mask_load(10);
         auto tiles = [&](auto Q, auto S_) {
             constexpr int q = decltype(Q)::value, s = decltype(S_)::value;
@@ -529,13 +546,15 @@
 }
 
 int launch_delta_chain_x6(const float* packed_bwd, const float* acts, int64_t p_pad, const float* d_rgb, float* dv0,
-                          float* dv2, float* dv1, float* const da[8], hipStream_t s, int max_grid, int* grid_out) {
+                          float* dv2, float* dv1, float* const da[8], hipStream_t s, int max_grid, int* grid_out, const int* live) {
     if (p_pad <= 0) return IDN_OK;
     if (p_pad % 128) return fail(IDN_EINVAL, "delta chain: p_pad %lld is not a multiple of 128", (long long)p_pad);
     static LaunchSetup setup;
     int num_cu = 0;
     if (int e = setup.get([]() -> int {
-            IDN_HIP_CHECK(hipFuncSetAttribute(reinterpret_cast<const void*>(&x6::delta_chain_x6_kernel),
+            IDN_HIP_CHECK(hipFuncSetAttribute(reinterpret_cast<const void*>(&x6::delta_chain_x6_kernel<false>),
+                                              hipFuncAttributeMaxDynamicSharedMemorySize, x6::kDelta6Lds));
+            IDN_HIP_CHECK(hipFuncSetAttribute(reinterpret_cast<const void*>(&x6::delta_chain_x6_kernel<true>),
                                               hipFuncAttributeMaxDynamicSharedMemorySize, x6::kDelta6Lds));
             return IDN_OK;
         }, &num_cu))
@@ -545,7 +564,8 @@
     DeltaArgs a{packed_bwd, acts, (long)p_pad, d_rgb, dv0, dv2, dv1, {}};
     for (int l = 0; l < 8; ++l) a.da[l] = da[l];
     ProfScope prof(s, p_pad, IDN_PROF_DELTA_CHAIN_X6);
-    hipLaunchKernelGGL(x6::delta_chain_x6_kernel, dim3(grid), dim3(256), x6::kDelta6Lds, s, a);
+    if (live) hipLaunchKernelGGL(x6::delta_chain_x6_kernel<true>, dim3(grid), dim3(256), x6::kDelta6Lds, s, x6::DeltaArgsG{a, live});
+    else hipLaunchKernelGGL(x6::delta_chain_x6_kernel<false>, dim3(grid), dim3(256), x6::kDelta6Lds, s, a);
     IDN_HIP_CHECK(hipGetLastError());
     if (grid_out) *grid_out = grid;
     return IDN_OK;
diff --git a/ideal-nerf_amd/csrc/train.hip b/ideal-nerf_amd/csrc/train.hip
--- a/ideal-nerf_amd/csrc/train.hip
+++ b/ideal-nerf_amd/csrc/train.hip
@@ -223,8 +223,106 @@
 constexpr int kCondColsumBlocks = 512;
 static_assert(512 + (size_t)kCondColsumBlocks * 512 * 2 <= kCpartPoolFloats, "the conditioning-only column sums fit the cpart pool");
 
+constexpr int kLiveThreads = 256, kLiveWaves = kLiveThreads / 64;
+__global__ __launch_bounds__(kLiveThreads) void live_chunks_mark_kernel(const float* d_rgb, const float* dv0, int n_chunks,
+                                                                        unsigned long long* masks, int* counts) {
+    __shared__ int wave_count[kLiveWaves];
+    const int lane = threadIdx.x & 63, wave = threadIdx.x >> 6;
+    const long c = (long)blockIdx.x * kLiveThreads + threadIdx.x;
+    bool live = false;
+    if (c < n_chunks) {
+#pragma unroll
+        for (int r = 0; r < 16; ++r) {
+            const long p = c * 16 + r;
+            const f32x4 v = *reinterpret_cast<const f32x4*>(d_rgb + p * 64);
+            const float sg = dv0[p * 256 + kSigmaChannel];
+            live = live || !(v[0] == 0.0f) || !(v[1] == 0.0f) || !(v[2] == 0.0f) || !(sg == 0.0f);
+        }
+    }
+    const unsigned long long ballot = __ballot(live);
+    if (lane == 0) {
+        masks[(long)blockIdx.x * kLiveWaves + wave] = ballot;
+        wave_count[wave] = __popcll(ballot);
+    }
+    __syncthreads();
+    if (threadIdx.x == 0) {
+        int n = 0;
+        for (int w = 0; w < kLiveWaves; ++w) n += wave_count[w];
+        counts[blockIdx.x] = n;
+    }
+}
+__global__ __launch_bounds__(kLiveThreads) void live_chunks_write_kernel(const unsigned long long* masks, const int* counts, int n_blocks,
+                                                                         int n_chunks, int* list, unsigned long long* counters) {
+    __shared__ int red[2][kLiveWaves];
+    const int lane = threadIdx.x & 63, wave = threadIdx.x >> 6;
+    int before = 0, total = 0;
+    for (int i = threadIdx.x; i < n_blocks; i += kLiveThreads) {
+        const int n = counts[i];
+        total += n;
+        if (i < (int)blockIdx.x) before += n;
+    }
+#pragma unroll
+    for (int m = 32; m >= 1; m >>= 1) {
+        before += __shfl_xor(before, m, 64);
+        total += __shfl_xor(total, m, 64);
+    }
+    if (lane == 0) red[0][wave] = before, red[1][wave] = total;
+    __syncthreads();
+    before = total = 0;
+    for (int w = 0; w < kLiveWaves; ++w) before += red[0][w], total += red[1][w];
+    const int pad = (kLiveListPad - total % kLiveListPad) % kLiveListPad;
+    const long c = (long)blockIdx.x * kLiveThreads + threadIdx.x;
+    const unsigned long long* m = masks + (long)blockIdx.x * kLiveWaves;
+    int pos = before;
+    for (int w = 0; w < wave; ++w) pos += __popcll(m[w]);
+    const unsigned long long mine = m[wave];
+    pos += __popcll(mine & ((1ull << lane) - 1ull));
+    if (c < n_chunks) {
+        if (mine >> lane & 1ull) {
+            list[kLiveListHeader + pos] = (int)c;
+        } else {
+            const long dead_rank = c - pos;
+            if (dead_rank < pad) list[kLiveListHeader + total + dead_rank] = (int)c;
+        }
+    }
+    if (blockIdx.x == 0 && threadIdx.x == 0) {
+        list[0] = total;
+        list[1] = total + pad;
+        if (counters) {
+            atomicAdd(counters + 0, (unsigned long long)total);
+            atomicAdd(counters + 1, (unsigned long long)n_chunks);
+        }
+    }
+}
+static size_t live_scratch_ints(int64_t p_pad) {
+    const size_t blocks = (size_t)((p_pad / 16 + kLiveThreads - 1) / kLiveThreads);
+    return 2 * kLiveWaves * blocks + blocks;
+}
+static int launch_live_chunks(const float* d_rgb, const float* dv0, int64_t p_pad, int* list, int* scratch, unsigned long long* counters,
+                              hipStream_t s) {
+    const int n_chunks = (int)(p_pad / 16), n_blocks = (n_chunks + kLiveThreads - 1) / kLiveThreads;
+    unsigned long long* masks = reinterpret_cast<unsigned long long*>(scratch);
+    int* counts = scratch + 2 * kLiveWaves * n_blocks;
+    hipLaunchKernelGGL(live_chunks_mark_kernel, dim3(n_blocks), dim3(kLiveThreads), 0, s, d_rgb, dv0, n_chunks, masks, counts);
+    IDN_HIP_CHECK(hipGetLastError());
+    hipLaunchKernelGGL(live_chunks_write_kernel, dim3(n_blocks), dim3(kLiveThreads), 0, s, (const unsigned long long*)masks, (const int*)counts,
+                       n_blocks, n_chunks, list, counters);
+    IDN_HIP_CHECK(hipGetLastError());
+    return IDN_OK;
+}
+size_t live_chunks_workspace_bytes(int64_t p_pad) { return al256(live_scratch_ints(p_pad) * 4); }
+int launch_live_chunks_alone(const float* d_rgb, const float* dv0, int64_t p_pad, int* list, void* ws, size_t ws_bytes, hipStream_t s) {
+    if (!d_rgb || !dv0 || !list) return fail(IDN_EINVAL, "live_chunks: NULL pointer");
+    if (p_pad <= 0 || p_pad % 128) return fail(IDN_EINVAL, "live_chunks: p_pad %lld is not a positive multiple of 128", (long long)p_pad);
+    if (p_pad > (int64_t)1 << 24) return fail(IDN_EUNSUPPORTED, "live_chunks: p_pad %lld exceeds 2^24", (long long)p_pad);
+    if (((uintptr_t)d_rgb | (uintptr_t)ws) & 15) return fail(IDN_EINVAL, "live_chunks: operands are not 16-byte aligned");
+    if (!ws || ws_bytes < live_chunks_workspace_bytes(p_pad)) return fail(IDN_EWORKSPACE, "live_chunks workspace %zu < %zu", ws_bytes, live_chunks_workspace_bytes(p_pad));
+    return launch_live_chunks(d_rgb, dv0, p_pad, list, static_cast<int*>(ws), nullptr, s);
+}
+
 struct BwdWs {
     float *dA[8], *dV[2], *dV0, *dRGB, *part, *cpart, *wbwd;
+    int *live, *live_scratch;
     size_t bytes;
 };
 static BwdWs carve_bwd(char* base, int64_t p_pad) {
@@ -243,6 +341,8 @@
     w.part = take(kPartPoolFloats);
     w.cpart = take(kCpartPoolFloats);
     w.wbwd = take(bwd_stream_floats_x6());
+    w.live = reinterpret_cast<int*>(take(live_list_ints(p_pad)));
+    w.live_scratch = reinterpret_cast<int*>(take(live_scratch_ints(p_pad)));
     w.bytes = off;
     return w;
 }
@@ -261,7 +361,7 @@
 }
 
 static int bwd_tail(const idn_facenerf_params& p, const idn_facenerf_grads* grads, const BwdCond& cond, const float* acts, int64_t P,
-                    int64_t Pp, const BwdWs& w, hipStream_t s) {
+                    int64_t Pp, const BwdWs& w, hipStream_t s, const int* live_chain = nullptr, const int* live_dw = nullptr) {
     const int C = p.dim_aud + p.dim_expr + p.dim_latent;
     const int PC = pts_ch_of(p), VC = views_ch_of(p);
     const int ld0 = PC + C, ld5 = PC + C + IDN_W, ldv = IDN_W + VC + p.dim_expr;
@@ -272,7 +372,7 @@
     const int pipe = backward_pipe();
     if (pipe == kPipeX6) {
         TRY(launch_pack_bf16x6_bwd(p, w.wbwd, s));
-        TRY(launch_delta_chain_x6(w.wbwd, acts, Pp, w.dRGB, w.dV0, w.dV[0], w.dV[1], w.dA, s));
+        TRY(launch_delta_chain_x6(w.wbwd, acts, Pp, w.dRGB, w.dV0, w.dV[0], w.dV[1], w.dA, s, 0, nullptr, live_chain));
     } else {
         TRY(launch_pack_f32_bwd(p, w.wbwd, s));
         TRY(launch_delta_chain(w.wbwd, acts, Pp, w.dRGB, w.dV0, w.dV[0], w.dV[1], w.dA, s));
@@ -308,7 +408,7 @@
         return IDN_OK;
     }
     const idn_facenerf_grads& gr = *grads;
-    DwPass q(w.part, kPartPoolFloats, w.cpart, kCpartPoolFloats, Pp, pipe, kX6ItemsPerPass, s);
+    DwPass q(w.part, kPartPoolFloats, w.cpart, kCpartPoolFloats, Pp, pipe, kX6ItemsPerPass, s, live_dw);
     DwProduct h;
     TRY(q.product(w.dRGB, 64, 64, v_l(3), 128, 128, true, &h));
     TRY(q.take_colsum(h, 0, 3, gr.rgb_b));
@@ -401,7 +501,10 @@
                       w.dRGB, 64, w.dV0 + kSigmaChannel, 256, (long)n_rays, S, d_rays ? d_rays + 6 : nullptr, IDN_RAY_FLOATS};
         if (int e = launch_composite_bwd(a, s)) return e;
     }
-    if (int e = bwd_tail(p, b.grads, b.cond, b.acts, P, Pp, w, s)) return e;
+    const bool live_plan = b.live_chunks && b.grads && backward_pipe() == kPipeX6 && Pp * 1024 < ((int64_t)1 << 31);
+    if (live_plan)
+        if (int e = launch_live_chunks(w.dRGB, w.dV0, Pp, w.live, w.live_scratch, reinterpret_cast<unsigned long long*>(b.chunk_counters), s)) return e;
+    if (int e = bwd_tail(p, b.grads, b.cond, b.acts, P, Pp, w, s, live_plan && !d_rays ? w.live : nullptr, live_plan ? w.live : nullptr)) return e;
     if (d_rays) {
         float* d_x = w.dA[1];
         static_assert(IDN_PTS_CH + IDN_VIEWS_CH <= 256, "the input-row gradient fits a delta matrix");
diff --git a/ideal-nerf_amd/ops.py b/ideal-nerf_amd/ops.py
--- a/ideal-nerf_amd/ops.py
+++ b/ideal-nerf_amd/ops.py
@@ -222,21 +222,34 @@
     return raw, acts
 
 
+LIVE_CHUNKS_DEFAULT = (os.environ.get("IDN_LIVE_CHUNKS", "1") or "1").strip() != "0"
+
+
 def _pass_bwd(p, grads, aud, expr, latent, acts, raw, z, rays, bc, g_rgb, g_fg, g_lw, g_acc, d_aud, d_latent, d_views0_bias=None,
-              d_rays=None, with_rays=False, d_expr=None, ex=False):
+              d_rays=None, with_rays=False, d_expr=None, ex=False, live_chunks=None, chunk_counters=None):
     lib = _lib.load()
     if grads is None:
         grads = {}
+    live = LIVE_CHUNKS_DEFAULT if live_chunks is None else bool(live_chunks)
+    if chunk_counters is not None:
+        _shape(chunk_counters, "chunk_counters", 2)
     n, S = z.shape
     for t, name, shape in ((raw, "raw", (n, S, 4)), (rays, "rays", (n, RAY_FLOATS)), (bc, "bc_rgb", (n, 3)),
                            (g_rgb, "g_rgb_map", (n, 3)), (g_fg, "g_rgb_fg", (n, 3)), (g_lw, "g_last_weight", (n,)),
                            (g_acc, "g_acc", (n,)), (d_rays, "d_rays", (n, RAY_FLOATS)), (d_expr, "d_expr", (p.dim_expr,))):
         _shape(t, name, *shape)
     tensors = (aud, expr, latent, acts, raw, z, rays, bc, g_rgb, g_fg, g_lw, g_acc, d_aud, d_latent)
-    with _Launch(*tensors, d_rays, d_expr, d_views0_bias if ex else None, *grads.values()) as L:
+    with _Launch(*tensors, d_rays, d_expr, d_views0_bias if ex else None, chunk_counters, *grads.values()) as L:
         ws = _workspace(lib.idealnerf_pass_bwd_workspace_bytes(n, S), z.device, L.stream)
         ptrs = [_ptr(t) for t in tensors]
-        if ex:
+        if not live or chunk_counters is not None:
+            if ex:
+                _shape(d_views0_bias, "d_views0_bias", W_HID // 2)
+            extra = _lib.PassBwdExtra(_ptr(d_expr, "d_expr"), _ptr(d_rays, "d_rays"), _ptr(d_views0_bias if ex else None, "d_views0_bias"))
+            opts = _lib.PassBwdOpts(int(live), _ptr(chunk_counters, "chunk_counters", torch.int64))
+            check(lib.idealnerf_pass_bwd_opts(C.byref(p), C.byref(grads_struct(grads)) if grads else None, *ptrs[:8], n, S, *ptrs[8:],
+                                              C.byref(extra), C.byref(opts), ws.data_ptr(), ws.numel(), L.stream))
+        elif ex:
             _shape(d_views0_bias, "d_views0_bias", W_HID // 2)
             extra = _lib.PassBwdExtra(_ptr(d_expr, "d_expr"), _ptr(d_rays, "d_rays"), _ptr(d_views0_bias, "d_views0_bias"))
             check(lib.idealnerf_pass_bwd_ex(C.byref(p), C.byref(grads_struct(grads)) if grads else None, *ptrs[:8], n, S, *ptrs[8:],
@@ -251,8 +264,10 @@
     return grads
 
 
-def pass_bwd(p, grads, aud, expr, latent, acts, raw, z, rays, bc, g_rgb, g_fg, g_lw, g_acc, d_aud, d_latent):
-    return _pass_bwd(p, grads, aud, expr, latent, acts, raw, z, rays, bc, g_rgb, g_fg, g_lw, g_acc, d_aud, d_latent)
+def pass_bwd(p, grads, aud, expr, latent, acts, raw, z, rays, bc, g_rgb, g_fg, g_lw, g_acc, d_aud, d_latent, live_chunks=None,
+             chunk_counters=None):
+    return _pass_bwd(p, grads, aud, expr, latent, acts, raw, z, rays, bc, g_rgb, g_fg, g_lw, g_acc, d_aud, d_latent,
+                     live_chunks=live_chunks, chunk_counters=chunk_counters)
 
 
 def pass_bwd_rays(p, grads, aud, expr, latent, acts, raw, z, rays, bc, g_rgb, g_fg, g_lw, g_acc, d_aud, d_latent, d_rays):
@@ -494,9 +509,31 @@
 _dw_products_ws = {}
 
 
-def dw_products(rows, products, pipe=0, x6_items=1):
+def live_chunks(d_rgb, dv0):
+    lib = _lib.load()
+    _shape(d_rgb, "d_rgb", None, 64)
+    p_pad = d_rgb.shape[0]
+    _shape(dv0, "dv0", p_pad, 256)
+    if p_pad <= 0 or p_pad % 128:
+        raise IdealNerfError(f"live_chunks: p_pad {p_pad} is not a positive multiple of 128")
+    with _Launch(d_rgb, dv0) as L:
+        out = torch.zeros(lib.idealnerf_live_list_ints(p_pad), dtype=torch.int32, device=L.device)
+        ws = torch.zeros(lib.idealnerf_live_chunks_workspace_bytes(p_pad), dtype=torch.uint8, device=L.device)
+        check(lib.idealnerf_live_chunks(_ptr(d_rgb, "d_rgb"), _ptr(dv0, "dv0"), p_pad, out.data_ptr(), ws.data_ptr(), ws.numel(), L.stream))
+    return out
+
+
+def dw_products(rows, products, pipe=0, x6_items=1, live=None):
     lib = _lib.load()
     E = IdealNerfError
+    if live is not None:
+        _shape(live, "live", 8 + rows // 16)
+        head = [int(v) for v in live[:2].tolist()]
+        if not 0 <= head[0] <= head[1] <= rows // 16 or head[1] % 8 or head[1] - head[0] >= 8:
+            raise E(f"dw_products: live list counts {head} for {rows // 16} chunks")
+        body = live[8:8 + head[1]]
+        if head[1] and (int(body.min()) < 0 or int(body.max()) >= rows // 16):
+            raise E(f"dw_products: live list entries outside [0, {rows // 16})")
     if not 1 <= len(products) <= _lib.DW_MAX_PRODUCTS:
         raise E(f"dw_products: {len(products)} products outside [1, {_lib.DW_MAX_PRODUCTS}]")
     if pipe not in (0, 1):
@@ -550,7 +587,7 @@
                 raise E(f"dw_products: product {i} column-sum take {j} does not fit out {list(out.shape)}")
             tensors.append(out)
         tensors += [t["delta"], t["acts"], t.get("acts2")]
-    with _Launch(*tensors) as L:
+    with _Launch(*tensors, live) as L:
         recs = (_lib.DwProduct * len(products))()
         for r, t in zip(recs, products):
             r.delta, r.ld_delta, r.N = _ptr(t["delta"], "delta") + 4 * int(t.get("delta_col0", 0)), t["delta"].shape[1], int(t["N"])
@@ -568,7 +605,11 @@
         ws = _dw_products_ws.get(key)
         if ws is None:
             ws = _dw_products_ws[key] = torch.zeros(nbytes, dtype=torch.uint8, device=L.device)
-        check(lib.idealnerf_dw_products(rows, int(pipe), int(x6_items), recs, len(products), ws.data_ptr(), ws.numel(), L.stream))
+        if live is not None:
+            check(lib.idealnerf_dw_products_live(rows, int(pipe), int(x6_items), recs, len(products), _ptr(live, "live", torch.int32),
+                                                 ws.data_ptr(), ws.numel(), L.stream))
+        else:
+            check(lib.idealnerf_dw_products(rows, int(pipe), int(x6_items), recs, len(products), ws.data_ptr(), ws.numel(), L.stream))
         return [(r.splits, r.chunks_per_split) for r in recs]
 
 
diff --git a/include/idealnerf.h b/include/idealnerf.h
--- a/include/idealnerf.h
+++ b/include/idealnerf.h
@@ -235,6 +235,21 @@
                           float* d_latent, const idn_pass_bwd_extra* extra, void* workspace, size_t workspace_bytes,
                           void* stream);
 
+typedef struct idn_pass_bwd_opts {
+    int live_chunks;
+    int64_t* chunk_counters;
+} idn_pass_bwd_opts;
+int idealnerf_pass_bwd_opts(const idn_facenerf_params* p, const idn_facenerf_grads* grads, const float* aud,
+                            const float* expr, const float* latent, const float* acts, const float* raw, const float* z,
+                            const float* rays, const float* bc_rgb, int64_t n_rays, int n_samples, const float* g_rgb_map,
+                            const float* g_rgb_fg, const float* g_last_weight, const float* g_acc, float* d_aud,
+                            float* d_latent, const idn_pass_bwd_extra* extra, const idn_pass_bwd_opts* opts, void* workspace,
+                            size_t workspace_bytes, void* stream);
+size_t idealnerf_live_list_ints(int64_t p_pad);
+size_t idealnerf_live_chunks_workspace_bytes(int64_t p_pad);
+int idealnerf_live_chunks(const float* d_rgb, const float* dv0, int64_t p_pad, int* list, void* workspace,
+                          size_t workspace_bytes, void* stream);
+
 int idealnerf_facenerf_train_fwd(const float* packed, const float* folded, int precision, const float* x, int64_t n,
                                  float* out, float* acts, void* stream);
 int idealnerf_facenerf_train_fwd_ch(const float* packed, const float* folded, int precision, const float* x, int pts_ch,
@@ -281,6 +296,8 @@
 size_t idealnerf_dw_products_workspace_bytes(void);
 int idealnerf_dw_products(int64_t rows, int pipe, int x6_items, idn_dw_product* products, int n, void* workspace,
                           size_t workspace_bytes, void* stream);
+int idealnerf_dw_products_live(int64_t rows, int pipe, int x6_items, idn_dw_product* products, int n, const int* live,
+                               void* workspace, size_t workspace_bytes, void* stream);
 
 size_t idealnerf_delta_chain_workspace_bytes(void);
 int idealnerf_delta_chain(const idn_facenerf_params* p, int pipe, const float* acts, int64_t p_pad, const float* d_rgb,
```

Result: no change. 132.9 million (median of 5 runs) (+0.1%).
